# huzi96/gaussian-pcloud-render

Measured on AMD Instinct MI355X. Metric: rendered frames/sec at 1080p (fwd+bwd), THuman-800K, higher is better.
Workload: dtype f32

## Files before the change

### gaussian-pcloud-render_amd/csrc/api.hip

```cpp
#include <algorithm>
#include <cstdarg>
#include <cstdio>
#include <cstring>
#include <string>
#include <vector>

#include "common.hpp"
#include <atomic>
#include <map>
#include <mutex>

namespace gsr {

static thread_local char g_err[512] = "";

static int fail(int code, const char* fmt, ...)
{
    va_list ap;
    va_start(ap, fmt);
    vsnprintf(g_err, sizeof(g_err), fmt, ap);
    va_end(ap);
    return code;
}

int check_launch(const Launch& L, const char* what)
{
    hipError_t e = hipGetLastError();
    if (e == hipSuccess && L.debug) e = hipStreamSynchronize(L.stream);
    if (e != hipSuccess) return fail(GSR_ERR_HIP, "[gsr] %s: %s", what, hipGetErrorString(e));
    return GSR_OK;
}

struct ProfEntry {
    const char* name;
    int a, b;
};
struct ProfTables {
    std::vector<hipEvent_t> pool;
    size_t used = 0;
    std::vector<ProfEntry> rec;
    int event()
    {
        if (used == pool.size()) {
            hipEvent_t e;
            if (hipEventCreateWithFlags(&e, hipEventDisableSystemFence) != hipSuccess) (void)hipEventCreate(&e);
            pool.push_back(e);
        }
        return (int)used++;
    }
};
static std::atomic<int> g_prof_on{0};
static std::mutex g_prof_mu;
static std::map<hipStream_t, ProfTables> g_prof;

struct ProfScope {
    hipStream_t s;
    bool on;
    ProfEntry e;
    ProfScope(const char* name, hipStream_t stream) : s(stream), on(false)
    {
        const int mode = g_prof_on;
        on = mode == 1 || (mode == 2 && strncmp(name, "render_", 7) == 0);
        if (!on) return;
        e.name = name;
        hipEvent_t ea;
        {
            std::lock_guard<std::mutex> lk(g_prof_mu);
            ProfTables& t = g_prof[s];
            e.a = t.event();
            e.b = t.event();
            ea = t.pool[e.a];
        }
        (void)hipEventRecord(ea, s);
    }
    ~ProfScope()
    {
        if (!on) return;
        std::lock_guard<std::mutex> lk(g_prof_mu);
        ProfTables& t = g_prof[s];
        (void)hipEventRecord(t.pool[e.b], s);
        t.rec.push_back(e);
    }
};

constexpr int MAX_VIEWS = 256;
struct HostLanding {
    uint64_t* pinned = nullptr;
    uint64_t* mapped = nullptr;
    hipEvent_t ev = nullptr;
};
static thread_local std::map<int, HostLanding> t_lands;
static int landing(HostLanding** out)
{
    int dev = 0;
    if (hipGetDevice(&dev) != hipSuccess) return fail(GSR_ERR_HIP, "[gsr] hipGetDevice: %s", hipGetErrorString(hipGetLastError()));
    HostLanding& h = t_lands[dev];
    if (!h.pinned) {
        if (hipHostMalloc((void**)&h.pinned, MAX_VIEWS * 4 * sizeof(uint64_t), hipHostMallocMapped | hipHostMallocCoherent) != hipSuccess ||
            hipHostGetDevicePointer((void**)&h.mapped, h.pinned, 0) != hipSuccess ||
            hipEventCreateWithFlags(&h.ev, hipEventDisableTiming) != hipSuccess) {
            h.pinned = nullptr;
            return fail(GSR_ERR_HIP, "[gsr] pinned host buffer: %s", hipGetErrorString(hipGetLastError()));
        }
    }
    *out = &h;
    return GSR_OK;
}

static thread_local std::vector<int64_t> t_list_pairs;

static std::atomic<long long> g_d2h_count{0};

static std::atomic<int> g_tickets{[] { const char* e = getenv("GSR_TICKETS"); return e && atoi(e) == 0 ? 0 : 1; }()};
int block_tickets(int set)
{
    if (set >= 0) g_tickets = set != 0;
    return g_tickets;
}

static int tile_count(const gsr_params* p) { return ((p->W + TILE_X - 1) / TILE_X) * ((p->H + TILE_Y - 1) / TILE_Y); }

static int check_params(const gsr_params* p, int V = 1)
{
    if (!p) return fail(GSR_ERR_INVALID, "[gsr] params is NULL");
    if (p->P < 0 || p->W <= 0 || p->H <= 0) return fail(GSR_ERR_INVALID, "[gsr] bad sizes P=%d W=%d H=%d", p->P, p->W, p->H);
    if (V < 1 || V > MAX_VIEWS) return fail(GSR_ERR_INVALID, "[gsr] view count %d outside 1..%d", V, MAX_VIEWS);
    if (p->P == 0) return GSR_OK;
    if (!p->means3D || !p->opacities || !p->bg || !p->viewmatrix || !p->projmatrix || !p->campos)
        return fail(GSR_ERR_INVALID, "[gsr] a required input pointer is NULL");
    if ((p->shs == nullptr) == (p->colors_precomp == nullptr))
        return fail(GSR_ERR_INVALID, "Please provide excatly one of either SHs or precomputed colors!");
    if (((p->scales == nullptr || p->rotations == nullptr) && p->cov3D_precomp == nullptr) ||
        ((p->scales != nullptr || p->rotations != nullptr) && p->cov3D_precomp != nullptr))
        return fail(GSR_ERR_INVALID, "Please provide exactly one of either scale/rotation pair or precomputed 3D covariance!");
    if (p->shs) {
        if (p->D < 0 || p->D > 3) return fail(GSR_ERR_INVALID, "[gsr] SH degree %d outside 0..3", p->D);
        if ((p->D + 1) * (p->D + 1) > p->M) return fail(GSR_ERR_INVALID, "[gsr] SH degree %d needs %d coefficients, M=%d", p->D, (p->D + 1) * (p->D + 1), p->M);
    }
    const int64_t gx = (p->W + TILE_X - 1) / TILE_X, gy = (p->H + TILE_Y - 1) / TILE_Y;
    if (gx > 65535 || gy > 65535) return fail(GSR_ERR_INVALID, "[gsr] image too large for 16-bit tile coordinates");
    if (gx * gy > (1ll << BWD_TILE_BITS) || (gx * gy / 8 + 1) * 64 * V > 0x7FFFFFFFll)
        return fail(GSR_ERR_INVALID, "[gsr] %lld tiles x %d views: too many for one launch", (long long)(gx * gy), V);
    return GSR_OK;
}

static int tile_bits(int T) { return (int)higher_msb((uint32_t)T); }
static int sorted_buffer(int T) { return ((tile_bits(T) + RADIX_BITS - 1) / RADIX_BITS) & 1; }

static inline void* align256(void* p) { return (void*)(((uintptr_t)p + 255) & ~(uintptr_t)255); }

static int make_batch(const gsr_params* p, int V, void* geom, size_t geom_bytes, void* image, size_t image_bytes, void* binning,
                      size_t binning_bytes, bool with_grad, Batch& B)
{
    B.V = V;
    const size_t G = geom_view(nullptr, p->P).bytes, I = image_view(nullptr, p->W, p->H).bytes;
    const size_t GR = with_grad ? grad_rec_bytes(p->P) : 0;
    if (!geom || geom_bytes < (size_t)V * (G + GR) + 256)
        return fail(GSR_ERR_CAPACITY, "[gsr] geom arena too small (%zu < %zu%s)", geom_bytes, (size_t)V * (G + GR) + 256,
                    with_grad ? ", need_backward" : "");
    if (!image || image_bytes < (size_t)V * I + 256)
        return fail(GSR_ERR_CAPACITY, "[gsr] image arena too small (%zu < %zu)", image_bytes, (size_t)V * I + 256);
    B.g = geom_view(align256(geom), p->P);
    B.g_stride = G;
    B.grad_rec = with_grad ? reinterpret_cast<float*>(reinterpret_cast<char*>(align256(geom)) + (size_t)V * G) : nullptr;
    B.gr_stride = GR;
    B.iv = image_view(align256(image), p->W, p->H);
    B.iv_stride = I;
    if (binning) {
        if (binning_bytes < 256 + 256 * (size_t)V) return fail(GSR_ERR_CAPACITY, "[gsr] binning arena too small");
        const size_t per_view = ((binning_bytes - 256) / (size_t)V) / 256 * 256;
        const int64_t cap = bin_capacity_from_bytes(per_view);
        if (cap < 1) return fail(GSR_ERR_CAPACITY, "[gsr] binning arena too small (%zu bytes for %d views)", binning_bytes, V);
        B.b = bin_view(align256(binning), cap > 0xFFFFFFFFll ? 0xFFFFFFFFll : cap);
        B.b_stride = per_view;
    } else {
        B.b = bin_view(nullptr, 1);
        B.b.cap = 0;
        B.b_stride = 0;
    }
    return GSR_OK;
}

struct FrameRecord {
    int kind = 0;
    int need_backward = 0;
    int nx = 0, layout = 0;
    int V = 0, P = 0, W = 0, H = 0;
    const void* xstate = nullptr;
    size_t xstate_bytes = 0;
    int fwd_need_backward = -1;
    int64_t list_pairs = -1;
    FrameRecord() = default;
    FrameRecord(int kind_, const gsr_params* p, int V_) : kind(kind_), need_backward(p->need_backward != 0), V(V_), P(p->P), W(p->W), H(p->H) {}
};
static std::mutex g_frames_mu;
static std::map<const void*, FrameRecord> g_frames;
static void note_frame(const void* geom, const FrameRecord& r)
{
    std::lock_guard<std::mutex> lk(g_frames_mu);
    if (g_frames.size() > 4096 && !g_frames.count(geom)) g_frames.clear();
    g_frames[geom] = r;
}
static bool find_frame(const void* geom, FrameRecord& r)
{
    std::lock_guard<std::mutex> lk(g_frames_mu);
    const auto it = g_frames.find(geom);
    if (it == g_frames.end()) return false;
    r = it->second;
    return true;
}
static size_t xstate_view_bytes(int W, int H, int64_t cap, int nx) { return align_up(xstate_view(nullptr, W, H, cap, nx).bytes, 256); }

static int memset_views(hipStream_t s, void* base, size_t stride, size_t bytes, int V)
{
    if (bytes == 0) return GSR_OK;
    hipError_t e = V == 1 ? hipMemsetAsync(base, 0, bytes, s) : hipMemset2DAsync(base, stride, 0, bytes, (size_t)V, s);
    return e == hipSuccess ? GSR_OK : fail(GSR_ERR_HIP, "[gsr] memset failed: %s", hipGetErrorString(e));
}

static int forward_impl(const gsr_params* p, int V, void* geom, size_t geom_bytes, void* image, size_t image_bytes, void* binning,
                        size_t binning_bytes, int* radii, float* out_color, int64_t* num_rendered, int mode, hipStream_t stream,
                        const ExtraChannels* X = nullptr)
{
    if (int e = check_params(p, V)) return e;
    if (!num_rendered) return fail(GSR_ERR_INVALID, "[gsr] num_rendered is NULL");
    for (int v = 0; v < V; v++) num_rendered[v] = 0;
    if (p->P == 0) return GSR_OK;
    if (mode != 1 && !radii) return fail(GSR_ERR_INVALID, "[gsr] radii is NULL");
    if (mode != 2 && !out_color) return fail(GSR_ERR_INVALID, "[gsr] out_color is NULL");
    if (mode != 2 && !binning) return fail(GSR_ERR_INVALID, "[gsr] binning arena is NULL");
    Batch B;
    if (int e = make_batch(p, V, geom, geom_bytes, image, image_bytes, mode == 2 ? nullptr : binning, binning_bytes,
                           p->need_backward != 0, B))
        return e;
    ExtraChannels Xs;
    const void* xraw = X != nullptr ? (const void*)X->state.accum : nullptr;
    if (X != nullptr && X->state.accum != nullptr) {
        Xs = *X;
        const size_t need = (size_t)V * xstate_view_bytes(p->W, p->H, B.b.cap, X->nx) + 256;
        if (X->state.bytes < need)
            return fail(GSR_ERR_CAPACITY, "[gsr] extra-state block too small (%zu < %zu: V * gsr_extra_state_bytes(W, H, n, nx) for a binning "
                        "arena of V * gsr_binning_bytes(n))", X->state.bytes, need);
        Xs.state = xstate_view(align256(const_cast<float*>(X->state.accum)), p->W, p->H, B.b.cap, X->nx);
        Xs.state_stride = xstate_view_bytes(p->W, p->H, B.b.cap, X->nx);
        if (!p->need_backward) Xs.state = XStateView{nullptr, nullptr, 0};
        X = &Xs;
    }
    {
        FrameRecord r(X ? 1 : 0, p, V);
        r.fwd_need_backward = r.need_backward;
        if (X) {
            r.nx = X->nx;
            r.layout = X->values_hi ? 2 : X->view_stride ? 1 : 0;
            if (X->state.accum) { r.xstate = xraw; r.xstate_bytes = X->state.bytes; }
        }
        note_frame(geom, r);
    }
    HostLanding* landp = nullptr;
    if (int e = landing(&landp)) return e;
    HostLanding& t_land = *landp;
    const Launch L{stream, p->debug};
    const int T = tile_count(p);
    const int gridx = (p->W + TILE_X - 1) / TILE_X;
    const bool key16 = tile_keys16(T);
    memset(t_land.pinned, 0, (size_t)V * 4 * sizeof(uint64_t));

    if (mode == 1) {
        if (int e = memset_views(L.stream, B.g.zero_begin, B.g_stride, B.g.zero_bytes, V)) return e;
        if (int e = memset_views(L.stream, B.iv.zero_begin, B.iv_stride, B.iv.zero_bytes, V)) return e;
    } else {
        if (p->prefiltered)
            if (int e = memset_views(L.stream, B.g.counters, B.g_stride, 8 * sizeof(uint64_t), V)) return e;
        {
            ProfScope ps("preprocess", L.stream);
            if (int e = launch_preprocess(L, *p, B, radii)) return e;
        }
        {
            ProfScope ps("depth_sort", L.stream);
            SortJob job{{B.g.dkey[0], B.g.dkey[1]}, {B.g.dval[0], B.g.dval[1]}, B.g.hist, B.g.totals, B.g_stride, nullptr, 0, p->P, V};
            job.blk_minmax = B.g.blk_minmax;
            job.sortctl = B.g.sortctl;
            job.small_blocks = div_up(p->P, RS_TILE) * V < 4096;
            int res = 0;
            if (int e = launch_radix_sort_pairs(L, job, true, 32, &res)) return e;
        }
    }
    const auto rest = [&]() -> int {
        {
            ProfScope ps("duplicate", L.stream);
            if (int e = launch_duplicate(L, p->P, B, gridx, key16, t_land.mapped)) return e;
        }
        {
            g_d2h_count++;
            const hipError_t e = hipEventRecord(t_land.ev, L.stream);
            if (e != hipSuccess) return fail(GSR_ERR_HIP, "[gsr] num_rendered read-back: %s", hipGetErrorString(e));
        }
        if (mode != 2) {
            const int res = sorted_buffer(T);
            {
                ProfScope ps("tile_sort", L.stream);
                SortJob job{{B.b.key[0], B.b.key[1]}, {B.b.val[0], B.b.val[1]}, B.b.hist, B.b.totals, B.b_stride,
                            B.g.counters + CNT_NUM_RENDERED, B.g_stride, B.b.cap, V};
                int r2 = 0;
                if (int e = launch_radix_sort_pairs(L, job, false, tile_bits(T), &r2, key16)) return e;
            }
            {
                ProfScope ps("tile_ranges", L.stream);
                if (int e = launch_tile_ranges(L, B, B.b.key[res], T, key16)) return e;
                if (int e = launch_tile_order(L, B, T)) return e;
            }
            {
                ProfScope ps("render_forward", L.stream);
                if (int e = launch_render_forward(L, *p, B, B.b.val[res], out_color, p->need_backward != 0, X)) return e;
            }
        }
        return GSR_OK;
    };
    if (int e = rest()) {
        (void)hipStreamSynchronize(L.stream);
        return e;
    }
    if (hipEventSynchronize(t_land.ev) != hipSuccess)
        return fail(GSR_ERR_HIP, "[gsr] num_rendered read-back failed: %s", hipGetErrorString(hipGetLastError()));
    bool retry = false;
    t_list_pairs.assign((size_t)V, 0);
    for (int v = 0; v < V; v++) {
        const uint64_t R = t_land.pinned[4 * v + LAND_NUM_REFERENCE], Lp = t_land.pinned[4 * v + CNT_NUM_RENDERED];
        if (t_land.pinned[4 * v + CNT_STALL])
            return fail(GSR_ERR_HIP, "[gsr] pair emission: a workgroup's pair count never arrived (view %d)", v);
        if (p->prefiltered && t_land.pinned[4 * v + CNT_TRAP])
            return fail(GSR_ERR_TRAP, "Point is filtered although prefiltered is set. This shouldn't happen!");
        if (R > 0x7FFFFFFFull)
            return fail(GSR_ERR_CAPACITY, "[gsr] num_rendered = %llu tile pairs does not fit the reference's int (scales too large?)",
                        (unsigned long long)R);
        num_rendered[v] = (int64_t)R;
        t_list_pairs[(size_t)v] = (int64_t)Lp;
        if (mode != 2 && (int64_t)Lp > B.b.cap) retry = true;
    }
    {
        FrameRecord r;
        if (find_frame(geom, r)) {
            r.list_pairs = *std::max_element(t_list_pairs.begin(), t_list_pairs.end());
            note_frame(geom, r);
        }
    }
    if (retry) {
        fail(GSR_RETRY, "[gsr] binning arena holds %lld pairs per view, the frame needs more (num_rendered is enough; gsr_last_list_pairs is exact): repeat with resume = 1",
             (long long)B.b.cap);
        return GSR_RETRY;
    }
    return GSR_OK;
}

}

using namespace gsr;

extern "C" {

size_t gsr_geom_bytes(int P) { return geom_view(nullptr, P).bytes + grad_rec_bytes(P) + 256; }
size_t gsr_geom_bytes_inference(int P) { return geom_view(nullptr, P).bytes + 256; }
size_t gsr_image_bytes(int W, int H) { return image_view(nullptr, W, H).bytes + 256; }
size_t gsr_binning_bytes(int64_t R) { return bin_view(nullptr, R).bytes + 256; }

int gsr_forward_batch(const gsr_params* p, int V, void* geom, size_t geom_bytes, void* image, size_t image_bytes, void* binning,
                      size_t binning_bytes, int* radii, float* out_color, int64_t* num_rendered, int resume, gsr_stream_t stream)
{
    return forward_impl(p, V, geom, geom_bytes, image, image_bytes, binning, binning_bytes, radii, out_color, num_rendered,
                        resume ? 1 : 0, (hipStream_t)stream);
}

static int extra_channels(const gsr_params* p, int nx, int extra_per_view, const float* extra, const float* extra_view_scale,
                          const float* bg_extra, float* out_extra, ExtraChannels& X)
{
    if (!p) return fail(GSR_ERR_INVALID, "[gsr] params is NULL");
    if (nx != 4 && nx != 8) return fail(GSR_ERR_INVALID, "[gsr] extra channels come in 4 or 8 (got %d): pad with zeros", nx);
    if (!extra || !bg_extra || !out_extra) return fail(GSR_ERR_INVALID, "[gsr] an extra-channel pointer is NULL");
    if (extra_per_view < 0 || extra_per_view > 2 || (extra_per_view == 2 && nx != 8))
        return fail(GSR_ERR_INVALID, "[gsr] extra_per_view is 0, 1 or (with 8 channels) 2");
    X = ExtraChannels{nx, extra, extra_view_scale, bg_extra, out_extra, extra_per_view == 1 ? (size_t)p->P * (size_t)nx : (size_t)0};
    if (extra_per_view == 2) {
        X.values_hi = extra + (size_t)p->P * 4;
        X.hi_view_stride = (size_t)p->P * 4;
    }
    return GSR_OK;
}

int gsr_forward_batch_channels(const gsr_params* p, int V, void* geom, size_t geom_bytes, void* image, size_t image_bytes,
                               void* binning, size_t binning_bytes, int* radii, float* out_color, int64_t* num_rendered, int resume,
                               int nx, int extra_per_view, const float* extra, const float* extra_view_scale, const float* bg_extra,
                               float* out_extra, gsr_stream_t stream)
{
    ExtraChannels X;
    if (int e = extra_channels(p, nx, extra_per_view, extra, extra_view_scale, bg_extra, out_extra, X)) return e;
    return forward_impl(p, V, geom, geom_bytes, image, image_bytes, binning, binning_bytes, radii, out_color, num_rendered,
                        resume ? 1 : 0, (hipStream_t)stream, &X);
}

size_t gsr_extra_state_bytes(int W, int H, int64_t num_rendered, int nx)
{
    if (W <= 0 || H <= 0 || (nx != 4 && nx != 8)) return 0;
    return xstate_view_bytes(W, H, bin_capacity_from_bytes(bin_view(nullptr, num_rendered).bytes), nx);
}

int gsr_forward_batch_channels_train(const gsr_params* p, int V, void* geom, size_t geom_bytes, void* image, size_t image_bytes,
                                     void* binning, size_t binning_bytes, int* radii, float* out_color, int64_t* num_rendered,
                                     int resume, int nx, int extra_per_view, const float* extra, const float* extra_view_scale,
                                     const float* bg_extra, float* out_extra, void* extra_state, size_t extra_state_bytes,
                                     gsr_stream_t stream)
{
    ExtraChannels X;
    if (int e = extra_channels(p, nx, extra_per_view, extra, extra_view_scale, bg_extra, out_extra, X)) return e;
    if (!extra_state) return fail(GSR_ERR_INVALID, "[gsr] extra_state is NULL");
    X.state = XStateView{reinterpret_cast<float*>(extra_state), nullptr, extra_state_bytes};
    return forward_impl(p, V, geom, geom_bytes, image, image_bytes, binning, binning_bytes, radii, out_color, num_rendered,
                        resume ? 1 : 0, (hipStream_t)stream, &X);
}

int gsr_forward_stage1(const gsr_params* p, void* geom, size_t geom_bytes, void* image, size_t image_bytes, int* radii,
                       int64_t* num_rendered_out, gsr_stream_t stream)
{
    if (!num_rendered_out) return fail(GSR_ERR_INVALID, "[gsr] num_rendered_out is NULL");
    return forward_impl(p, 1, geom, geom_bytes, image, image_bytes, nullptr, 0, radii, nullptr, num_rendered_out, 2, (hipStream_t)stream);
}

int gsr_forward_stage2(const gsr_params* p, void* geom, size_t geom_bytes, void* binning, size_t binning_bytes, void* image,
                       size_t image_bytes, int64_t R, float* out_color, gsr_stream_t stream)
{
    if (R < 0 || R > 0x7FFFFFFFll) return fail(GSR_ERR_INVALID, "[gsr] num_rendered out of range");
    if (p && p->P > 0 && (!binning || binning_bytes < gsr_binning_bytes(R)))
        return fail(GSR_ERR_CAPACITY, "[gsr] binning arena too small (%zu < %zu)", binning_bytes, gsr_binning_bytes(R));
    int64_t got = 0;
    const int rc = forward_impl(p, 1, geom, geom_bytes, image, image_bytes, binning, binning_bytes, nullptr, out_color, &got, 1,
                                (hipStream_t)stream);
    if (rc == GSR_OK && p && p->P > 0 && got != R) return fail(GSR_ERR_INVALID, "[gsr] stage 2 found %lld pairs, stage 1 reported %lld", (long long)got, (long long)R);
    return rc;
}

int gsr_forward_recolor(const gsr_params* p, int V, int colors_per_view, void* geom, size_t geom_bytes, const void* binning,
                        size_t binning_bytes, void* image, size_t image_bytes, float* out_color, gsr_stream_t stream)
{
    if (!p) return fail(GSR_ERR_INVALID, "[gsr] params is NULL");
    if (V < 1 || V > MAX_VIEWS) return fail(GSR_ERR_INVALID, "[gsr] view count %d outside 1..%d", V, MAX_VIEWS);
    if (p->P <= 0) return GSR_OK;
    if ((p->shs == nullptr) == (p->colors_precomp == nullptr))
        return fail(GSR_ERR_INVALID, "Please provide excatly one of either SHs or precomputed colors!");
    if (p->shs && (!p->means3D || !p->campos || p->D < 0 || p->D > 3 || (p->D + 1) * (p->D + 1) > p->M))
        return fail(GSR_ERR_INVALID, "[gsr] recolor: bad SH arguments");
    if (!out_color || !p->bg || !binning) return fail(GSR_ERR_INVALID, "[gsr] recolor: NULL pointer");
    Batch B;
    if (int e = make_batch(p, V, geom, geom_bytes, image, image_bytes, const_cast<void*>(binning), binning_bytes, false, B)) return e;
    {
        FrameRecord prev, r(2, p, V);
        if (find_frame(geom, prev)) {
            r.fwd_need_backward = prev.fwd_need_backward;
            r.list_pairs = prev.list_pairs;
        }
        note_frame(geom, r);
    }
    const Launch L{(hipStream_t)stream, p->debug};
    const int res = sorted_buffer(tile_count(p));
    {
        ProfScope ps("recolor", L.stream);
        if (int e = launch_recolor(L, *p, B, (colors_per_view && p->colors_precomp) ? (size_t)p->P * 3 : 0)) return e;
        if (int e = memset_views(L.stream, B.iv.tile_need, B.iv_stride, (size_t)tile_count(p) * sizeof(uint32_t), V)) return e;
    }
    {
        ProfScope ps("render_forward", L.stream);
        if (int e = launch_render_forward(L, *p, B, B.b.val[res], out_color, p->need_backward != 0)) return e;
    }
    return GSR_OK;
}

static size_t det_view_bytes(int W, int H, int64_t pairs)
{
    const int T = ((W + TILE_X - 1) / TILE_X) * ((H + TILE_Y - 1) / TILE_Y);
    return align_up(det_view(nullptr, T, pairs).bytes, 256);
}

size_t gsr_backward_det_bytes(int V, int P, int W, int H, int64_t pairs)
{
    (void)P;
    if (V < 1 || W <= 0 || H <= 0) return 0;
    if (pairs > 0xFFFFFFFFll) pairs = 0xFFFFFFFFll;
    return (size_t)V * det_view_bytes(W, H, pairs) + 256;
}

struct BwdGrads {
    const float* dL_dpix;
    float *dL_dmean2D, *dL_dopacity, *dL_dcolor, *dL_dmean3D, *dL_dcov3D, *dL_dsh, *dL_dscale, *dL_drot;
};
struct BwdDet { void* scratch; size_t bytes; };
struct BwdExtra {
    ExtraChannels X;
    ExtraGrads XG;
    int layout;
    const void* state;
    size_t state_bytes;
};

static int check_bwd_pointers(const gsr_params* p, const int* radii, const void* binning, const BwdGrads& G)
{
    if (!radii || !G.dL_dpix || !G.dL_dmean2D || !G.dL_dopacity || !G.dL_dcolor || !G.dL_dmean3D || !G.dL_dcov3D)
        return fail(GSR_ERR_INVALID, "[gsr] a required backward pointer is NULL");
    if (p->shs && !G.dL_dsh) return fail(GSR_ERR_INVALID, "[gsr] dL_dsh is NULL");
    if (p->scales && (!G.dL_dscale || !G.dL_drot)) return fail(GSR_ERR_INVALID, "[gsr] dL_dscale/dL_drot is NULL");
    if (p->scales && ((uintptr_t)G.dL_drot & 15u)) return fail(GSR_ERR_INVALID, "[gsr] dL_drot must be 16-byte aligned (it is written one float4 per Gaussian)");
    if (!binning) return fail(GSR_ERR_INVALID, "[gsr] binning arena is NULL");
    return GSR_OK;
}

static int check_bwd_frame(const void* geom, const gsr_params* p, int V, const BwdExtra* x, int64_t* list_pairs)
{
    FrameRecord r;
    *list_pairs = -1;
    if (!find_frame(geom, r))
        return x ? fail(GSR_ERR_INVALID, "[gsr] backward_channels: no forward on this geometry arena (run gsr_forward_batch_channels_train first)")
                 : GSR_OK;
    *list_pairs = r.list_pairs;
    const bool same = r.V == V && r.P == p->P && r.W == p->W && r.H == p->H;
    if (x) {
        if (r.kind == 2)
            return fail(GSR_ERR_INVALID, "[gsr] backward_channels after gsr_forward_recolor is not supported: the recolor replaced the saves "
                        "of the channels forward (run gsr_forward_batch_channels_train again)");
        if (r.kind != 1 || !r.need_backward || r.xstate == nullptr)
            return fail(GSR_ERR_INVALID, "[gsr] backward_channels: the forward on this arena saved no extra channels (it needs "
                        "gsr_forward_batch_channels_train with need_backward = 1)");
        if (r.nx != x->X.nx || r.layout != x->layout)
            return fail(GSR_ERR_INVALID, "[gsr] backward_channels: nx = %d, extra_per_view = %d, but the forward had nx = %d, extra_per_view = %d",
                        x->X.nx, x->layout, r.nx, r.layout);
        if (!same) return fail(GSR_ERR_INVALID, "[gsr] backward_channels: views / sizes differ from the forward's");
        if (r.xstate != x->state || x->state_bytes < r.xstate_bytes)
            return fail(GSR_ERR_INVALID, "[gsr] backward_channels: extra_state is not the block the forward saved into");
        return GSR_OK;
    }
    if (!r.need_backward)
        return fail(GSR_ERR_INVALID, "[gsr] backward: the last %s on this geometry arena had need_backward = 0 and saved nothing for "
                    "it", r.kind == 2 ? "gsr_forward_recolor" : "forward");
    if (r.fwd_need_backward == 0)
        return fail(GSR_ERR_INVALID, "[gsr] backward: the recolor's forward on this geometry arena had need_backward = 0 (a "
                    "need_backward recolor needs the arenas of a need_backward forward)");
    if (!same)
        return fail(GSR_ERR_INVALID, "[gsr] backward: V = %d, P = %d, %d x %d, but the last forward or recolor on this geometry "
                    "arena had V = %d, P = %d, %d x %d", V, p->P, p->W, p->H, r.V, r.P, r.W, r.H);
    return GSR_OK;
}

static int backward_impl(const gsr_params* p, int V, const int* radii, const void* geom, size_t geom_bytes, const void* binning,
                         size_t binning_bytes, const void* image, size_t image_bytes, const BwdGrads& G, const BwdDet* det, BwdExtra* x,
                         gsr_stream_t stream)
{
    if (det && x) return fail(GSR_ERR_INVALID, "[gsr] backward: no deterministic backward of the extra channels");
    if (int e = check_params(p, V)) return e;
    if (p->P == 0) return GSR_OK;
    int64_t list_pairs = -1;
    if (!x)
        if (int e = check_bwd_pointers(p, radii, binning, G)) return e;
    if (int e = check_bwd_frame(geom, p, V, x, &list_pairs)) return e;
    if (x)
        if (int e = check_bwd_pointers(p, radii, binning, G)) return e;
    Batch B;
    if (int e = make_batch(p, V, const_cast<void*>(geom), geom_bytes, const_cast<void*>(image), image_bytes,
                           const_cast<void*>(binning), binning_bytes, true, B))
        return e;
    const Launch L{(hipStream_t)stream, p->debug};
    const int T = tile_count(p), res = sorted_buffer(T);
    DetView D{};
    size_t d_stride = 0;
    if (det) {
        int64_t n = list_pairs >= 0 ? list_pairs : B.b.cap;
        if (n > B.b.cap) n = B.b.cap;
        if (n < 1) n = 1;
        const size_t need = gsr_backward_det_bytes(V, p->P, p->W, p->H, n);
        if (!det->scratch || det->bytes < need)
            return fail(GSR_ERR_CAPACITY, "[gsr] backward_det: scratch block too small (%zu < %zu = gsr_backward_det_bytes(%d, %d, %d, %d, %lld): "
                        "the forward's lists hold up to %lld pairs per view)", det->bytes, need, V, p->P, p->W, p->H, (long long)n,
                        (long long)n);
        D = det_view(align256(det->scratch), T, n);
        d_stride = det_view_bytes(p->W, p->H, n);
    }
    if (x) {
        const int nx = x->X.nx;
        x->X.state = xstate_view(align256(const_cast<void*>(x->state)), p->W, p->H, B.b.cap, nx);
        x->X.state_stride = xstate_view_bytes(p->W, p->H, B.b.cap, nx);
        if (x->state_bytes < (size_t)V * x->X.state_stride + 256)
            return fail(GSR_ERR_CAPACITY, "[gsr] extra-state block too small for this binning arena");
    }
    {
        ProfScope ps("bwd_items", L.stream);
        const size_t n_out = !x ? 0 : (size_t)p->P * (x->layout == 0 ? x->X.nx : x->layout == 1 ? V * x->X.nx : (1 + V) * 4);
        if (x && hipMemsetAsync(x->XG.grad, 0, n_out * sizeof(float), L.stream) != hipSuccess)
            return fail(GSR_ERR_HIP, "[gsr] memset failed: %s", hipGetErrorString(hipGetLastError()));
        if (int e = launch_bwd_items(L, B, T, p->P)) return e;
    }
    int dres = 0;
    if (det) {
        {
            ProfScope ps("det_prepare", L.stream);
            if (int e = launch_det_prepare(L, B, D, d_stride, B.b.val[res], T)) return e;
        }
        {
            ProfScope ps("det_sort", L.stream);
            if (int e = launch_det_sort(L, B, D, d_stride, p->P, &dres)) return e;
        }
    }
    {
        ProfScope ps("render_backward", L.stream);
        const RenderBwdDet d{D.part, D.flags, D.slot_base, d_stride, (uint32_t)D.cap};
        if (int e = launch_render_backward(L, *p, B, B.b.val[res], G.dL_dpix, x ? &x->X : nullptr, x ? &x->XG : nullptr, det ? &d : nullptr))
            return e;
    }
    if (det) {
        ProfScope ps("det_reduce", L.stream);
        if (int e = launch_det_reduce(L, B, D, d_stride, dres)) return e;
    }
    {
        ProfScope ps("preprocess_backward", L.stream);
        if (int e = launch_preprocess_backward(L, *p, B, radii, G.dL_dmean2D, G.dL_dopacity, G.dL_dcolor, G.dL_dmean3D, G.dL_dcov3D,
                                               G.dL_dsh, G.dL_dscale, G.dL_drot))
            return e;
    }
    return GSR_OK;
}

int gsr_backward_batch(const gsr_params* p, int V, const int* radii, const void* geom, size_t geom_bytes, const void* binning,
                       size_t binning_bytes, const void* image, size_t image_bytes, const float* dL_dpix, float* dL_dmean2D,
                       float* dL_dopacity, float* dL_dcolor, float* dL_dmean3D, float* dL_dcov3D, float* dL_dsh, float* dL_dscale,
                       float* dL_drot, gsr_stream_t stream)
{
    const BwdGrads G{dL_dpix, dL_dmean2D, dL_dopacity, dL_dcolor, dL_dmean3D, dL_dcov3D, dL_dsh, dL_dscale, dL_drot};
    return backward_impl(p, V, radii, geom, geom_bytes, binning, binning_bytes, image, image_bytes, G, nullptr, nullptr, stream);
}

int gsr_backward_batch_det(const gsr_params* p, int V, const int* radii, const void* geom, size_t geom_bytes, const void* binning,
                           size_t binning_bytes, const void* image, size_t image_bytes, const float* dL_dpix, float* dL_dmean2D,
                           float* dL_dopacity, float* dL_dcolor, float* dL_dmean3D, float* dL_dcov3D, float* dL_dsh, float* dL_dscale,
                           float* dL_drot, void* det_scratch, size_t det_scratch_bytes, gsr_stream_t stream)
{
    const BwdGrads G{dL_dpix, dL_dmean2D, dL_dopacity, dL_dcolor, dL_dmean3D, dL_dcov3D, dL_dsh, dL_dscale, dL_drot};
    const BwdDet det{det_scratch, det_scratch_bytes};
    return backward_impl(p, V, radii, geom, geom_bytes, binning, binning_bytes, image, image_bytes, G, &det, nullptr, stream);
}

int gsr_backward_batch_channels(const gsr_params* p, int V, const int* radii, const void* geom, size_t geom_bytes, const void* binning,
                                size_t binning_bytes, const void* image, size_t image_bytes, const float* dL_dpix, float* dL_dmean2D,
                                float* dL_dopacity, float* dL_dcolor, float* dL_dmean3D, float* dL_dcov3D, float* dL_dsh,
                                float* dL_dscale, float* dL_drot, int nx, int extra_per_view, const float* extra,
                                const float* extra_view_scale, const float* bg_extra, const void* extra_state, size_t extra_state_bytes,
                                const float* dL_dextra, float* dL_dextra_values, gsr_stream_t stream)
{
    BwdExtra x{{}, {}, extra_per_view, extra_state, extra_state_bytes};
    if (int e = extra_channels(p, nx, extra_per_view, extra, extra_view_scale, bg_extra, dL_dextra_values, x.X)) return e;
    if (!dL_dextra || !extra_state) return fail(GSR_ERR_INVALID, "[gsr] dL_dextra / extra_state is NULL");
    x.XG = ExtraGrads{dL_dextra, dL_dextra_values, extra_per_view == 2 ? dL_dextra_values + (size_t)p->P * 4 : nullptr};
    const BwdGrads G{dL_dpix, dL_dmean2D, dL_dopacity, dL_dcolor, dL_dmean3D, dL_dcov3D, dL_dsh, dL_dscale, dL_drot};
    return backward_impl(p, V, radii, geom, geom_bytes, binning, binning_bytes, image, image_bytes, G, nullptr, &x, stream);
}

int gsr_backward(const gsr_params* p, const int* radii, int64_t R, const void* geom, size_t geom_bytes, const void* binning,
                 size_t binning_bytes, const void* image, size_t image_bytes, const float* dL_dpix, float* dL_dmean2D,
                 float* dL_dopacity, float* dL_dcolor, float* dL_dmean3D, float* dL_dcov3D, float* dL_dsh,
                 float* dL_dscale, float* dL_drot, gsr_stream_t stream)
{
    (void)R;
    return gsr_backward_batch(p, 1, radii, geom, geom_bytes, binning, binning_bytes, image, image_bytes, dL_dpix, dL_dmean2D,
                              dL_dopacity, dL_dcolor, dL_dmean3D, dL_dcov3D, dL_dsh, dL_dscale, dL_drot, stream);
}

int gsr_mark_visible(int P, const float* means3D, const float* viewmatrix, const float* projmatrix, uint8_t* present,
                     gsr_stream_t stream)
{
    (void)projmatrix;
    if (P < 0) return fail(GSR_ERR_INVALID, "[gsr] P < 0");
    if (P == 0) return GSR_OK;
    if (!means3D || !viewmatrix || !present) return fail(GSR_ERR_INVALID, "[gsr] NULL pointer");
    const Launch L{(hipStream_t)stream, 0};
    return launch_mark_visible(L, P, means3D, viewmatrix, present);
}

namespace {
__global__ void k_clock_probe(unsigned long long* out, int iters)
{
    const unsigned long long s0 = clock64(), w0 = wall_clock64();
    float x = (float)threadIdx.x * 1e-3f;
    for (int i = 0; i < iters; i++) {
#pragma unroll
        for (int k = 0; k < 64; k++) x = __builtin_fmaf(x, 0.999f, 1e-3f);
    }
    const unsigned long long s1 = clock64(), w1 = wall_clock64();
    if (threadIdx.x == 0) {
        out[0] = s1 - s0;
        out[1] = w1 - w0;
    }
    if (x == 12345.678f) out[1] = 0;
}
__global__ void k_query(int what, int64_t n, const Splat* __restrict__ sp, const uint8_t* __restrict__ clamped,
                        const uint32_t* __restrict__ k, int key16, const uint32_t* __restrict__ v, void* __restrict__ dst)
{
    const int64_t i = (int64_t)blockIdx.x * 256 + threadIdx.x;
    if (i >= n) return;
    float* d = (float*)dst;
    switch (what) {
    case GSR_Q_DEPTHS: d[i] = sp[i].q2.y; break;
    case GSR_Q_MEANS2D: d[2 * i] = sp[i].q0.x; d[2 * i + 1] = sp[i].q0.y; break;
    case GSR_Q_CONIC_OPACITY:
        d[4 * i] = sp[i].q0.z; d[4 * i + 1] = sp[i].q0.w; d[4 * i + 2] = sp[i].q1.x; d[4 * i + 3] = sp[i].q1.y;
        break;
    case GSR_Q_RGB: d[3 * i] = sp[i].q1.z; d[3 * i + 1] = sp[i].q1.w; d[3 * i + 2] = sp[i].q2.x; break;
    case GSR_Q_POINT_LIST_KEYS:
        ((uint64_t*)dst)[i] = ((uint64_t)(key16 ? (uint32_t)((const uint16_t*)k)[i] : k[i]) << 32) | (uint64_t)__float_as_uint(sp[v[i]].q2.y);
        break;
    case GSR_Q_LIST_PAIRS: {
        const uint64_t* c = (const uint64_t*)k;
        if (i == 0) { ((uint64_t*)dst)[0] = c[CNT_NUM_RENDERED]; ((uint64_t*)dst)[1] = c[CNT_NUM_REFERENCE]; }
        break;
    }
    case GSR_Q_DEPTH_SORT: {
        uint32_t* o = (uint32_t*)dst;
        if (i == 0) { o[0] = k[SORTCTL_BASE]; o[1] = k[SORTCTL_BITS]; o[2] = depth_sort_passes(k[SORTCTL_BITS]); o[3] = 0u; }
        break;
    }
    case GSR_Q_CLAMPED: {
        uint8_t* c = (uint8_t*)dst;
        c[3 * i] = clamped[i] & 1; c[3 * i + 1] = (clamped[i] >> 1) & 1; c[3 * i + 2] = (clamped[i] >> 2) & 1;
        break;
    }
    default: break;
    }
}
}

int gsr_query(const gsr_params* p, int what, const void* geom, const void* binning, size_t binning_bytes, const void* image,
              int64_t R, void* dst, size_t dst_bytes, gsr_stream_t stream)
{
    if (!p || !dst) return fail(GSR_ERR_INVALID, "[gsr] query: NULL");
    hipStream_t s = (hipStream_t)stream;
    const int P = p->P, T = tile_count(p);
    const int64_t N = (int64_t)p->W * p->H;
    const GeomView g = geom_view(align256(const_cast<void*>(geom)), P);
    if (binning && binning_bytes < 512) return fail(GSR_ERR_CAPACITY, "[gsr] query: binning arena too small");
    const int64_t cap = binning ? bin_capacity_from_bytes(((binning_bytes - 256)) / 256 * 256) : 0;
    if (binning && R > cap && (what == GSR_Q_POINT_LIST || what == GSR_Q_POINT_LIST_KEYS))
        return fail(GSR_ERR_CAPACITY, "[gsr] query: arena holds %lld pairs, asked for %lld (the lists hold GSR_Q_LIST_PAIRS pairs)", (long long)cap, (long long)R);
    const BinView b = bin_view(align256(const_cast<void*>(binning)), cap > 0 ? cap : 1);
    const ImageView iv = image_view(align256(const_cast<void*>(image)), p->W, p->H);
    const int res = sorted_buffer(T);
    int64_t n = 0;
    size_t bytes = 0;
    const void* src = nullptr;
    switch (what) {
    case GSR_Q_DEPTHS: n = P; bytes = (size_t)P * 4; break;
    case GSR_Q_MEANS2D: n = P; bytes = (size_t)P * 8; break;
    case GSR_Q_CONIC_OPACITY: n = P; bytes = (size_t)P * 16; break;
    case GSR_Q_RGB: n = P; bytes = (size_t)P * 12; break;
    case GSR_Q_CLAMPED: n = P; bytes = (size_t)P * 3; break;
    case GSR_Q_POINT_LIST_KEYS: n = R; bytes = (size_t)R * 8; break;
    case GSR_Q_TILES_TOUCHED: src = g.tiles_touched; bytes = (size_t)P * 4; break;
    case GSR_Q_POINT_LIST: src = b.val[res]; bytes = (size_t)R * 4; break;
    case GSR_Q_RANGES: src = iv.ranges; bytes = (size_t)T * 8; break;
    case GSR_Q_FINAL_T: src = iv.final_T; bytes = (size_t)N * 4; break;
    case GSR_Q_N_CONTRIB: src = iv.n_contrib; bytes = (size_t)N * 4; break;
    case GSR_Q_TILE_NEED: src = iv.tile_need; bytes = (size_t)T * 4; break;
    case GSR_Q_DEPTH_SORT: n = 1; bytes = 16; break;
    case GSR_Q_LIST_PAIRS: n = 1; bytes = 16; break;
    default: return fail(GSR_ERR_INVALID, "[gsr] query: unknown item %d", what);
    }
    if (dst_bytes < bytes) return fail(GSR_ERR_CAPACITY, "[gsr] query %d: destination too small", what);
    if (bytes == 0) return GSR_OK;
    if (src) {
        if (hipMemcpyAsync(dst, src, bytes, hipMemcpyDeviceToDevice, s) != hipSuccess) return fail(GSR_ERR_HIP, "[gsr] query copy failed");
    } else {
        hipLaunchKernelGGL(k_query, dim3((unsigned)div_up(n, 256)), dim3(256), 0, s, what, n, g.splat, g.clamped,
                           what == GSR_Q_DEPTH_SORT ? (const uint32_t*)g.sortctl
                           : what == GSR_Q_LIST_PAIRS ? (const uint32_t*)g.counters : (const uint32_t*)b.key[res],
                           (int)tile_keys16(T), b.val[res], dst);
        if (hipGetLastError() != hipSuccess) return fail(GSR_ERR_HIP, "[gsr] query kernel failed");
    }
    return GSR_OK;
}

int gsr_selftest(gsr_stream_t stream)
{
    hipStream_t s = (hipStream_t)stream;
    float* d = nullptr;
    if (hipMalloc(&d, 256 * sizeof(float)) != hipSuccess) return fail(GSR_ERR_HIP, "[gsr] selftest: hipMalloc failed");
    const int rm = selftest_mm(s, d);
    (void)hipFree(d);
    if (rm != 0) return fail(GSR_ERR_HIP, "[gsr] selftest: matrix-core pixel contraction wrong at check %d", rm);
    const int rd = selftest_det_reduce(s);
    if (rd != 0) return fail(GSR_ERR_HIP, "[gsr] selftest: ordered reduction of the deterministic backward differs from the host sum at check %d", rd);

    const int64_t n = 100003;
    std::vector<uint32_t> hk(n), hv(n), order(n);
    uint32_t x = 12345u;
    for (int64_t i = 0; i < n; i++) {
        x = x * 1664525u + 1013904223u;
        hk[i] = (x >> 8) % 3001u;
        hv[i] = (uint32_t)i;
        order[i] = (uint32_t)i;
    }
    std::stable_sort(order.begin(), order.end(), [&](uint32_t a, uint32_t b) { return hk[a] < hk[b]; });
    uint32_t *k0, *k1, *v0, *v1, *hist, *tot;
    const size_t nb = (size_t)sort_hist_stride(n);
    if (hipMalloc(&k0, n * 4) != hipSuccess || hipMalloc(&k1, n * 4) != hipSuccess || hipMalloc(&v0, n * 4) != hipSuccess ||
        hipMalloc(&v1, n * 4) != hipSuccess || hipMalloc(&hist, RADIX * nb * 4) != hipSuccess || hipMalloc(&tot, RADIX * 4) != hipSuccess)
        return fail(GSR_ERR_HIP, "[gsr] selftest: hipMalloc failed");
    (void)hipMemcpyAsync(k0, hk.data(), n * 4, hipMemcpyHostToDevice, s);
    uint32_t* key[2] = {k0, k1};
    uint32_t* val[2] = {v0, v1};
    int res = 0;
    const Launch L{s, 1};
    const SortJob job{{k0, k1}, {v0, v1}, hist, tot, 0, nullptr, 0, n, 1};
    int rc = launch_radix_sort_pairs(L, job, true, 12, &res);
    std::vector<uint32_t> gk(n), gv(n);
    if (rc == 0) {
        (void)hipMemcpyAsync(gk.data(), key[res], n * 4, hipMemcpyDeviceToHost, s);
        (void)hipMemcpyAsync(gv.data(), val[res], n * 4, hipMemcpyDeviceToHost, s);
        if (hipStreamSynchronize(s) != hipSuccess) rc = GSR_ERR_HIP;
    }
    (void)hipFree(k0); (void)hipFree(k1); (void)hipFree(v0); (void)hipFree(v1); (void)hipFree(hist); (void)hipFree(tot);
    if (rc != 0) return rc;
    for (int64_t i = 0; i < n; i++)
        if (gv[i] != order[i] || gk[i] != hk[order[i]]) return fail(GSR_ERR_HIP, "[gsr] selftest: radix sort differs from std::stable_sort at %lld", (long long)i);
    return GSR_OK;
}

int gsr_clock_probe_launch(void* dst16, int iters, gsr_stream_t stream)
{
    if (!dst16 || iters < 1) return fail(GSR_ERR_INVALID, "[gsr] clock probe: bad argument");
    hipLaunchKernelGGL(k_clock_probe, dim3(1), dim3(64), 0, (hipStream_t)stream, (unsigned long long*)dst16, iters);
    if (hipGetLastError() != hipSuccess) return fail(GSR_ERR_HIP, "[gsr] clock probe launch failed");
    return GSR_OK;
}

int gsr_wall_clock_khz(void)
{
    int dev = 0, khz = 0;
    if (hipGetDevice(&dev) != hipSuccess || hipDeviceGetAttribute(&khz, hipDeviceAttributeWallClockRate, dev) != hipSuccess) return 0;
    return khz;
}

void gsr_set_profiling(int on)
{
    std::lock_guard<std::mutex> lk(g_prof_mu);
    g_prof_on = on < 0 ? 0 : on > 2 ? 1 : on;
    for (auto& kv : g_prof) { kv.second.rec.clear(); kv.second.used = 0; }
}

int gsr_get_profile(const char** names, float* ms, int cap)
{
    std::lock_guard<std::mutex> lk(g_prof_mu);
    int n = 0;
    for (auto& kv : g_prof) {
        ProfTables& t = kv.second;
        for (auto& e : t.rec) {
            if (n >= cap) break;
            (void)hipEventSynchronize(t.pool[e.b]);
            float d = 0;
            (void)hipEventElapsedTime(&d, t.pool[e.a], t.pool[e.b]);
            names[n] = e.name;
            ms[n] = d;
            n++;
        }
        t.rec.clear();
        t.used = 0;
    }
    return n;
}

#ifdef GSR_STATS
__attribute__((visibility("default"))) int gsr_debug_bwd_stats(unsigned long long* out8, int reset) { return gsr::debug_bwd_stats(out8, reset); }
__attribute__((visibility("default"))) int gsr_debug_scatter_times(unsigned long long* out8, int reset) { return gsr::debug_scatter_times(out8, reset); }
__attribute__((visibility("default"))) int gsr_debug_fwd_times(unsigned long long* out8, int reset) { return gsr::debug_fwd_times(out8, reset); }
__attribute__((visibility("default"))) int gsr_debug_fwd_records(unsigned* out, int n) { return gsr::debug_fwd_records(out, n); }
__attribute__((visibility("default"))) int gsr_debug_bwd_times(unsigned long long* out8, int reset) { return gsr::debug_bwd_times(out8, reset); }
__attribute__((visibility("default"))) int gsr_debug_bwd_records(unsigned* out, int n) { return gsr::debug_bwd_records(out, n); }
__attribute__((visibility("default"))) int gsr_debug_dup_times(unsigned long long* out8, int reset) { return gsr::debug_dup_times(out8, reset); }
#endif

long long gsr_d2h_count(void) { return gsr::g_d2h_count.load(); }
int gsr_set_forward_half_views(int views) { return gsr::forward_half_views(views); }
int gsr_set_backward_moments(int mode) { return gsr::backward_subquadrant_moments(mode); }

int gsr_last_list_pairs(int64_t* out, int V)
{
    if (!out || V < 0) return fail(GSR_ERR_INVALID, "[gsr] gsr_last_list_pairs: bad argument");
    for (int v = 0; v < V; v++) out[v] = (size_t)v < gsr::t_list_pairs.size() ? gsr::t_list_pairs[(size_t)v] : 0;
    return GSR_OK;
}

const char* gsr_last_error(void) { return gsr::g_err; }
const char* gsr_version(void) { return "gsr-hip 0.3 (gfx950)"; }

}
```

### gaussian-pcloud-render_amd/csrc/binning.hip

```cpp
#include "common.hpp"
#include "tile_cull.hpp"

namespace gsr {

__device__ __forceinline__ uint64_t agent_load(const uint64_t* p)
{
    return __hip_atomic_load(p, __ATOMIC_RELAXED, __HIP_MEMORY_SCOPE_AGENT);
}
__device__ __forceinline__ void agent_store(uint64_t* p, uint64_t v)
{
    __hip_atomic_store(p, v, __ATOMIC_RELAXED, __HIP_MEMORY_SCOPE_AGENT);
}

#ifdef GSR_STATS
constexpr int DUP_REC = 65536;
__device__ unsigned g_dup_rec[DUP_REC][4];
#define DUP_T(var) const unsigned long long var = wall_clock64()
#define DUP_ADD(i, v) do { if (threadIdx.x == 0) { const unsigned r_ = blockIdx.y * gridDim.x + s_ticket; if (r_ < DUP_REC) g_dup_rec[r_][i] = (unsigned)(v); } } while (0)
int debug_dup_times(unsigned long long* out8, int reset)
{
    static unsigned host[DUP_REC][4];
    if (hipMemcpyFromSymbol(host, HIP_SYMBOL(g_dup_rec), sizeof(host)) != hipSuccess) return -1;
    for (int i = 0; i < 8; i++) out8[i] = 0;
    for (int r = 0; r < DUP_REC; r++) {
        if (host[r][0] == 0 && host[r][1] == 0) continue;
        for (int i = 0; i < 4; i++) out8[i] += host[r][i];
        out8[4]++;
    }
    if (reset) {
        for (int r = 0; r < DUP_REC; r++) for (int i = 0; i < 4; i++) host[r][i] = 0;
        if (hipMemcpyToSymbol(HIP_SYMBOL(g_dup_rec), host, sizeof(host)) != hipSuccess) return -1;
    }
    return 0;
}
#else
#define DUP_T(var) do { } while (0)
#define DUP_ADD(i, v) do { } while (0)
#endif

struct DupArgs {
    int P;
    uint32_t gridx;
    const uint32_t* order[2];
    const uint32_t* sortctl;
    const Splat* splat;
    uint64_t* dup_status;
    uint64_t* counters;
    size_t g_stride;
    void* keys;
    uint32_t* vals;
    size_t b_stride;
    int64_t cap;
    uint64_t* host_land;
    int tickets;
};

template <typename KeyT>
__global__ __launch_bounds__(DUP_THREADS) void k_duplicate(DupArgs a)
{
    __shared__ uint32_t s_off[4][64];
    __shared__ uint32_t s_id[4][64];
    __shared__ uint2 s_rect[4][64];
    __shared__ uint32_t s_sp2[4][64];
    __shared__ uint2 s_pre[4][64];
    __shared__ uint32_t s_flag[4][64];
    __shared__ uint64_t s_wave[4];
    __shared__ uint64_t s_ref[4];
    __shared__ uint64_t s_base;
    __shared__ uint32_t s_ticket;
    const uint32_t view = blockIdx.y;
    const uint32_t lane = threadIdx.x & 63, w = threadIdx.x >> 6;
    uint64_t* status = at_view(a.dup_status, a.g_stride, view);
    const uint32_t nblk = gridDim.x;
    DUP_T(t0);
    if (threadIdx.x == 0) s_ticket = a.tickets ? (uint32_t)atomicAdd((unsigned long long*)&status[DUP_COPIES * nblk], 1ull) : blockIdx.x;
    __syncthreads();
    DUP_T(t1);
    DUP_ADD(0, t1 - t0);
    const uint32_t blk = s_ticket;
    const uint32_t npass = depth_sort_passes(at_view(a.sortctl, a.g_stride, view)[SORTCTL_BITS]);
    const uint32_t* order = at_view((npass & 1u) ? a.order[1] : a.order[0], a.g_stride, view);
    const Splat* splat = at_view(a.splat, a.g_stride, view);

    uint32_t cnt[DUP_G], id[DUP_G], sp2[DUP_G];
    uint2 rc[DUP_G];
    uint64_t ref_cnt = 0;
    const int slot0 = (int)(blk * DUP_BLOCK + w * (64 * DUP_G) + lane);
#pragma unroll
    for (int g = 0; g < DUP_G; g++) {
        const int slot = slot0 + g * 64;
        id[g] = slot < a.P ? order[slot] : 0u;
    }
#pragma unroll
    for (int g = 0; g < DUP_G; g++) {
        cnt[g] = 0;
        rc[g] = make_uint2(0, 0);
        sp2[g] = 0;
        if (slot0 + g * 64 < a.P) {
            const float4 q3 = splat[id[g]].q3;
            const uint32_t w3 = __float_as_uint(q3.w);
            rc[g] = make_uint2(__float_as_uint(q3.x), __float_as_uint(q3.y));
            sp2[g] = __float_as_uint(q3.z);
            if (w3 & SPANS_FLAG) {
                const uint32_t a4 = (rc[g].y >> 4) & 0x0F0F0F0Fu, b4 = (sp2[g] >> 4) & 0x0F0F0F0Fu;
                const uint32_t pa = a4 * 0x01010101u;
                const uint32_t pb = b4 * 0x01010101u + (pa >> 24) * 0x01010101u;
                cnt[g] = pb >> 24;
                id[g] |= SPANS_FLAG;
            } else {
                cnt[g] = sp2[g];
            }
            ref_cnt += w3 & ~SPANS_FLAG;
        }
    }
    uint64_t excl[DUP_G];
    uint64_t run = 0;
#pragma unroll
    for (int g = 0; g < DUP_G; g++) {
        uint64_t inc64 = cnt[g];
#pragma unroll
        for (int d = 1; d < 64; d <<= 1) {
            const uint64_t n = (uint64_t)__shfl_up((unsigned long long)inc64, d, 64);
            if (lane >= (uint32_t)d) inc64 += n;
        }
        excl[g] = run + inc64 - cnt[g];
        run += (uint64_t)__shfl((unsigned long long)inc64, 63, 64);
    }
#pragma unroll
    for (int d = 32; d >= 1; d >>= 1) ref_cnt += (uint64_t)__shfl_xor((unsigned long long)ref_cnt, d, 64);
    if (lane == 63) { s_wave[w] = run; s_ref[w] = ref_cnt; }
    __syncthreads();
    uint64_t wave_base = 0;
#pragma unroll
    for (int i = 0; i < 4; i++)
        if ((uint32_t)i < w) wave_base += s_wave[i];
    const uint64_t block_total = s_wave[0] + s_wave[1] + s_wave[2] + s_wave[3];
    const uint64_t block_ref = s_ref[0] + s_ref[1] + s_ref[2] + s_ref[3];
    const uint64_t sat = 0xFFFFFFFEull;
    const uint64_t word = ((block_total < sat ? block_total : sat) + 1ull) | ((block_ref < 0xFFFFFFFFull ? block_ref : 0xFFFFFFFFull) << 32);
    if (threadIdx.x < DUP_COPIES) agent_store(&status[threadIdx.x * nblk + blk], word);
    DUP_T(t2);
    DUP_ADD(1, t2 - t1);
    uint64_t part = 0, part_ref = 0;
    constexpr uint32_t LB = 4;
    const uint64_t* mine = status + (size_t)(blk % DUP_COPIES) * nblk;
    for (uint32_t b0 = threadIdx.x; b0 < blk; b0 += DUP_THREADS * LB) {
        uint64_t v[LB];
#pragma unroll
        for (uint32_t k = 0; k < LB; k++) {
            const uint32_t b = b0 + k * DUP_THREADS;
            v[k] = b < blk ? agent_load(&mine[b]) : 1ull;
        }
#pragma unroll
        for (uint32_t k = 0; k < LB; k++) {
            uint32_t spins = 0;
            while ((uint32_t)v[k] == 0u) {
                v[k] = agent_load(&mine[b0 + k * DUP_THREADS]);
                if ((uint32_t)v[k] == 0u && ++spins > (1u << 24)) {
                    at_view(a.counters, a.g_stride, view)[CNT_STALL] = 1;
                    a.host_land[4 * view + CNT_STALL] = 1;
                    v[k] = 1;
                }
            }
            part += (v[k] & 0xFFFFFFFFull) - 1;
            part_ref += v[k] >> 32;
        }
    }
#pragma unroll
    for (int d = 32; d >= 1; d >>= 1) {
        part += (uint64_t)__shfl_xor((unsigned long long)part, d, 64);
        part_ref += (uint64_t)__shfl_xor((unsigned long long)part_ref, d, 64);
    }
    __syncthreads();
    if (lane == 0) { s_wave[w] = part; s_ref[w] = part_ref; }
    __syncthreads();
    if (threadIdx.x == 0) {
        const uint64_t base = s_wave[0] + s_wave[1] + s_wave[2] + s_wave[3];
        s_base = base;
        if (blk == nblk - 1) {
            uint64_t* cnt = at_view(a.counters, a.g_stride, view);
            const uint64_t ref_total = s_ref[0] + s_ref[1] + s_ref[2] + s_ref[3] + block_ref;
            cnt[CNT_NUM_RENDERED] = base + block_total;
            cnt[CNT_NUM_REFERENCE] = ref_total;
            a.host_land[4 * view + CNT_NUM_RENDERED] = base + block_total;
            a.host_land[4 * view + CNT_TRAP] = cnt[CNT_TRAP];
            a.host_land[4 * view + LAND_NUM_REFERENCE] = ref_total;
            __threadfence_system();
        }
    }
    __syncthreads();
    DUP_T(t3);
    DUP_ADD(2, t3 - t2);
    if (a.keys == nullptr) return;
    KeyT* keys = at_view((KeyT*)a.keys, a.b_stride, view);
    uint32_t* vals = at_view(a.vals, a.b_stride, view);
    const uint64_t wave_off = s_base + wave_base;

#pragma unroll 1
    for (int g = 0; g < DUP_G; g++) {
        uint32_t cnt_g = cnt[0], id_g = id[0], sp2_g = sp2[0];
        uint2 rc_g = rc[0];
        uint64_t ex_g = excl[0];
#pragma unroll
        for (int k = 1; k < DUP_G; k++)
            if (g == k) { cnt_g = cnt[k]; id_g = id[k]; rc_g = rc[k]; ex_g = excl[k]; sp2_g = sp2[k]; }
        const uint64_t off64 = wave_off + ex_g;
        const uint64_t grp_begin64 = (uint64_t)__shfl((unsigned long long)off64, 0, 64);
        const uint64_t grp_end64 = (uint64_t)__shfl((unsigned long long)(off64 + cnt_g), 63, 64);
        if (grp_begin64 >= (uint64_t)a.cap) break;
        const uint32_t grp_begin = (uint32_t)grp_begin64;
        const uint32_t grp_end = grp_end64 < (uint64_t)a.cap ? (uint32_t)grp_end64 : (uint32_t)a.cap;
        const uint64_t nzb = __ballot(cnt_g != 0);
        const uint32_t n_nz = (uint32_t)__popcll(nzb);
        const uint32_t jslot = __builtin_amdgcn_mbcnt_hi((uint32_t)(nzb >> 32), __builtin_amdgcn_mbcnt_lo((uint32_t)nzb, 0u));
        __builtin_amdgcn_wave_barrier();
        if (cnt_g != 0) {
            s_off[w][jslot] = (uint32_t)(off64 - grp_begin64);
            s_id[w][jslot] = id_g;
            s_rect[w][jslot] = rc_g;
            s_sp2[w][jslot] = sp2_g;
            if (id_g & SPANS_FLAG) {
                const uint32_t a4 = (rc_g.y >> 4) & 0x0F0F0F0Fu, b4 = (sp2_g >> 4) & 0x0F0F0F0Fu;
                const uint32_t pa = a4 * 0x01010101u;
                s_pre[w][jslot] = make_uint2(pa, b4 * 0x01010101u + (pa >> 24) * 0x01010101u);
            }
        }
        __builtin_amdgcn_wave_barrier();
        const uint32_t my_start = lane < n_nz ? s_off[w][lane] : 0xFFFFFFFFu;
        const uint32_t range = grp_end - grp_begin;
        uint32_t before = 0;
        for (uint32_t c = 0; c < range; c += 64) {
            s_flag[w][lane] = 0u;
            const uint32_t d = my_start - c;
            if (d < 64u) s_flag[w][d] = 1u;
            __builtin_amdgcn_wave_barrier();
            const uint32_t mine = s_flag[w][lane];
            const uint64_t starts = __ballot(mine != 0u);
            const uint32_t owner = before + mine - 1u +
                                   __builtin_amdgcn_mbcnt_hi((uint32_t)(starts >> 32), __builtin_amdgcn_mbcnt_lo((uint32_t)starts, 0u));
            before += (uint32_t)__popcll(starts);
            __builtin_amdgcn_wave_barrier();
            const uint32_t rel = c + lane;
            if (rel < range) {
                const uint2 r = s_rect[w][owner];
                const uint32_t oid = s_id[w][owner];
                const uint32_t minx = r.x & 0xFFFFu, miny = r.x >> 16;
                const uint32_t t = rel - s_off[w][owner];
                uint32_t row, col;
                if (oid & SPANS_FLAG) {
                    const uint2 pre = s_pre[w][owner];
                    const uint32_t tt = (127u - t) * 0x01010101u;
                    const uint32_t xa = (pre.x + tt) & 0x80808080u, xb = (pre.y + tt) & 0x80808080u;
                    row = 8u - (uint32_t)__popc(xa) - (uint32_t)__popc(xb);
                    const uint32_t rp = row - 1u;
                    const uint32_t before = row == 0u ? 0u : (((rp < 4u ? pre.x : pre.y) >> (8u * (rp & 3u))) & 0xFFu);
                    const uint32_t byte = ((row < 4u ? r.y : s_sp2[w][owner]) >> (8u * (row & 3u))) & 0xFFu;
                    col = (byte & 15u) + (t - before);
                } else {
                    const uint32_t width = (r.y & 0xFFFFu) - minx;
                    row = t / width;
                    col = t - row * width;
                }
                const uint32_t p = grp_begin + rel;
                keys[p] = (KeyT)((miny + row) * a.gridx + (minx + col));
                vals[p] = oid & ~SPANS_FLAG;
            }
        }
    }
#ifdef GSR_STATS
    if (w == 0) { DUP_T(t4); DUP_ADD(3, t4 - t3); }
#endif
}

int launch_duplicate(const Launch& L, int P, const Batch& B, int gridx, bool key16, uint64_t* host_land)
{
    DupArgs a;
    a.P = P;
    a.gridx = (uint32_t)gridx;
    a.order[0] = B.g.dval[0];
    a.order[1] = B.g.dval[1];
    a.sortctl = B.g.sortctl;
    a.splat = B.g.splat;
    a.dup_status = B.g.dup_status;
    a.counters = B.g.counters;
    a.g_stride = B.g_stride;
    a.keys = B.b.key[0];
    a.vals = B.b.val[0];
    a.b_stride = B.b_stride;
    a.cap = B.b.key[0] ? B.b.cap : 0;
    a.host_land = host_land;
    a.tickets = block_tickets(-1);
    const dim3 grid((unsigned)div_up(P, DUP_BLOCK), B.V);
    if (key16)
        hipLaunchKernelGGL(k_duplicate<uint16_t>, grid, dim3(DUP_THREADS), 0, L.stream, a);
    else
        hipLaunchKernelGGL(k_duplicate<uint32_t>, grid, dim3(DUP_THREADS), 0, L.stream, a);
    return check_launch(L, "duplicate");
}

constexpr int RANGE_SAMPLE = 4096;
constexpr int RANGE_MAX_SAMPLES = 8192;

template <typename KeyT>
__device__ __forceinline__ uint32_t lower_bound_keys(const KeyT* __restrict__ keys, uint32_t n, const uint32_t* __restrict__ samples,
                                                     uint32_t ns, uint32_t t)
{
    uint32_t lo = 0, hi = n;
    if (ns != 0) {
        uint32_t a = 0, b = ns;
        while (a < b) {
            const uint32_t m = (a + b) >> 1;
            if (samples[m] < t) a = m + 1; else b = m;
        }
        if (a == 0) return 0;
        lo = (a - 1) * RANGE_SAMPLE + 1;
        hi = a < ns ? a * RANGE_SAMPLE : n;
    }
    while (lo < hi) {
        const uint32_t m = (lo + hi) >> 1;
        if ((uint32_t)keys[m] < t) lo = m + 1; else hi = m;
    }
    return lo;
}

constexpr int RANGE_TILES_PER_WG = 255;
template <typename KeyT>
__global__ __launch_bounds__(256) void k_tile_ranges(const uint64_t* __restrict__ counters, size_t g_stride, int64_t cap,
                                                     const KeyT* __restrict__ keys, size_t b_stride, uint2* __restrict__ ranges,
                                                     size_t iv_stride, int T)
{
    __shared__ uint32_t samples[RANGE_MAX_SAMPLES];
    __shared__ uint32_t bound[256];
    const uint32_t view = blockIdx.y;
    const uint64_t n64 = at_view(counters, g_stride, view)[CNT_NUM_RENDERED];
    const uint32_t n = (uint32_t)(n64 < (uint64_t)cap ? n64 : (uint64_t)cap);
    keys = at_view(keys, b_stride, view);
    ranges = at_view(ranges, iv_stride, view);
    uint32_t ns = (n + RANGE_SAMPLE - 1) / RANGE_SAMPLE;
    if (ns > RANGE_MAX_SAMPLES) ns = 0;
    for (uint32_t j = threadIdx.x; j < ns; j += 256) samples[j] = (uint32_t)keys[(size_t)j * RANGE_SAMPLE];
    __syncthreads();
    const int t = blockIdx.x * RANGE_TILES_PER_WG + threadIdx.x;
    bound[threadIdx.x] = (t < T && n != 0) ? lower_bound_keys(keys, n, samples, ns, (uint32_t)t) : n;
    __syncthreads();
    if (threadIdx.x >= RANGE_TILES_PER_WG || t >= T) return;
    const uint32_t first = bound[threadIdx.x], last = bound[threadIdx.x + 1];
    ranges[t] = first < last ? make_uint2(first, last) : make_uint2(0u, 0u);
}

int launch_tile_ranges(const Launch& L, const Batch& B, const uint32_t* sorted_keys, int T, bool key16)
{
    const dim3 grid((unsigned)div_up(T, RANGE_TILES_PER_WG), B.V);
    if (key16)
        hipLaunchKernelGGL(k_tile_ranges<uint16_t>, grid, dim3(256), 0, L.stream, B.g.counters, B.g_stride, B.b.cap,
                           (const uint16_t*)sorted_keys, B.b_stride, B.iv.ranges, B.iv_stride, T);
    else
        hipLaunchKernelGGL(k_tile_ranges<uint32_t>, grid, dim3(256), 0, L.stream, B.g.counters, B.g_stride, B.b.cap, sorted_keys,
                           B.b_stride, B.iv.ranges, B.iv_stride, T);
    return check_launch(L, "tile_ranges");
}

constexpr int ORD_BUCKETS = 128;

__device__ __forceinline__ uint32_t work_bucket(uint32_t len)
{
    if (len == 0) return ORD_BUCKETS - 1;
    const uint32_t msb = 31u - (uint32_t)__builtin_clz(len);
    const uint32_t frac = msb >= 2 ? (len >> (msb - 2)) & 3u : 0u;
    const uint32_t rank = msb * 4u + frac;
    return (ORD_BUCKETS - 2) - (rank < ORD_BUCKETS - 2 ? rank : ORD_BUCKETS - 2);
}

__device__ __forceinline__ uint32_t work_estimate(uint32_t len, float knee, float expo)
{
    if (knee <= 0.f || (float)len <= knee) return len;
    return (uint32_t)(knee * __builtin_amdgcn_exp2f(expo * __builtin_amdgcn_logf(knee / (float)len)));
}

__global__ __launch_bounds__(1024) void k_tile_order(int T, const uint2* __restrict__ ranges, uint32_t* __restrict__ tile_order,
                                                     size_t iv_stride, float knee, float expo)
{
    ranges = at_view(ranges, iv_stride, blockIdx.x);
    tile_order = at_view(tile_order, iv_stride, blockIdx.x);
    __shared__ uint32_t cnt[ORD_BUCKETS];
    __shared__ uint32_t cur[ORD_BUCKETS];
    const uint32_t lane = threadIdx.x & 63;
    const uint64_t lt_mask = (1ull << lane) - 1ull;
    if (threadIdx.x < ORD_BUCKETS) cnt[threadIdx.x] = 0;
    __syncthreads();
    const int T_pad = (T + 1023) / 1024 * 1024;
    for (int pass = 0; pass < 2; pass++) {
        for (int t = threadIdx.x; t < T_pad; t += 1024) {
            const bool ok = t < T;
            uint32_t b = 0;
            if (ok) b = work_bucket(work_estimate(ranges[t].y - ranges[t].x, knee, expo));
            const bool empty = ok && b == ORD_BUCKETS - 1;
            const uint64_t em = __ballot(empty);
            uint32_t slot = 0;
            if (pass == 0) {
                if (empty) { if ((em & lt_mask) == 0) atomicAdd(&cnt[b], (uint32_t)__popcll(em)); }
                else if (ok) atomicAdd(&cnt[b], 1u);
            } else {
                uint32_t basev = 0;
                const int leader = em ? (int)__builtin_ctzll(em) : 0;
                if (empty && (int)lane == leader) basev = atomicAdd(&cur[b], (uint32_t)__popcll(em));
                basev = __shfl(basev, leader, 64);
                if (empty) slot = basev + (uint32_t)__popcll(em & lt_mask);
                else if (ok) slot = atomicAdd(&cur[b], 1u);
                if (ok) tile_order[slot] = (uint32_t)t;
            }
        }
        __syncthreads();
        if (pass == 0) {
            if (threadIdx.x < 64) {
                const uint32_t a0 = cnt[2 * lane], a1 = cnt[2 * lane + 1];
                uint32_t inc = a0 + a1;
#pragma unroll
                for (int d = 1; d < 64; d <<= 1) {
                    const uint32_t n = __shfl_up(inc, d, 64);
                    if (lane >= (uint32_t)d) inc += n;
                }
                cur[2 * lane] = inc - a0 - a1;
                cur[2 * lane + 1] = inc - a1;
            }
            __syncthreads();
        }
    }
}

static void order_params(float& knee, float& expo)
{
    static const float k = [] { const char* e = getenv("GSR_ORDER_KNEE"); return e ? (float)atof(e) : 2048.f; }();
    static const float x = [] { const char* e = getenv("GSR_ORDER_EXP"); return e ? (float)atof(e) : 0.3f; }();
    knee = k;
    expo = x;
}

int launch_tile_order(const Launch& L, const Batch& B, int T)
{
    float knee, expo;
    order_params(knee, expo);
    hipLaunchKernelGGL(k_tile_order, dim3(B.V), dim3(1024), 0, L.stream, T, B.iv.ranges, B.iv.tile_order, B.iv_stride, knee, expo);
    return check_launch(L, "tile_order");
}

constexpr int BWD_CLEAR_BLOCKS = 64;
__global__ __launch_bounds__(1024) void k_bwd_items(int T, int chunk_shift, const uint32_t* __restrict__ need, uint32_t* __restrict__ items,
                                                    uint32_t* __restrict__ count, size_t iv_stride, const uint64_t* __restrict__ counters,
                                                    size_t g_stride, float* __restrict__ grad_rec, size_t gr_stride, size_t gr_bytes)
{
    if (blockIdx.y != 0) {
        if (at_view(counters, g_stride, blockIdx.x)[CNT_BWD_DIRTY] == 0) return;
        zero_region(reinterpret_cast<char*>(at_view(grad_rec, gr_stride, blockIdx.x)), gr_bytes,
                    (size_t)(blockIdx.y - 1) * 1024 + threadIdx.x, (size_t)BWD_CLEAR_BLOCKS * 1024);
        return;
    }
    need = at_view(need, iv_stride, blockIdx.x);
    items = at_view(items, iv_stride, blockIdx.x);
    count = at_view(count, iv_stride, blockIdx.x);
    if (threadIdx.x < 8) count[BWD_QUEUE_WORD + threadIdx.x] = 0;
    __shared__ uint32_t cnt[ORD_BUCKETS];
    __shared__ uint32_t cur[ORD_BUCKETS];
    const uint32_t lane = threadIdx.x & 63;
    if (threadIdx.x < ORD_BUCKETS) cnt[threadIdx.x] = 0;
    __syncthreads();
    const uint32_t full_bucket = work_bucket(1u << chunk_shift);
    for (int pass = 0; pass < 2; pass++) {
        for (int t = threadIdx.x; t < T; t += 1024) {
            const uint32_t n = need[t];
            if (n == 0) continue;
            uint32_t n_full = n >> chunk_shift;
            if (n_full > BWD_MAX_CHUNKS - 1) n_full = BWD_MAX_CHUNKS - 1;
            const uint32_t rest = n - (n_full << chunk_shift);
            if (pass == 0) {
                if (n_full) atomicAdd(&cnt[full_bucket], n_full);
                if (rest) atomicAdd(&cnt[work_bucket(rest)], 1u);
            } else {
                if (n_full) {
                    const uint32_t slot = atomicAdd(&cur[full_bucket], n_full);
                    for (uint32_t c = 0; c < n_full; c++) items[slot + c] = (uint32_t)t | (c << BWD_TILE_BITS);
                }
                if (rest) items[atomicAdd(&cur[work_bucket(rest)], 1u)] = (uint32_t)t | (n_full << BWD_TILE_BITS);
            }
        }
        __syncthreads();
        if (pass == 0) {
            if (threadIdx.x < 64) {
                const uint32_t a0 = cnt[2 * lane], a1 = cnt[2 * lane + 1];
                uint32_t inc = a0 + a1;
#pragma unroll
                for (int d = 1; d < 64; d <<= 1) {
                    const uint32_t n = __shfl_up(inc, d, 64);
                    if (lane >= (uint32_t)d) inc += n;
                }
                cur[2 * lane] = inc - a0 - a1;
                cur[2 * lane + 1] = inc - a1;
                if (lane == 63) count[0] = inc;
            }
            __syncthreads();
        }
    }
}

int launch_bwd_items(const Launch& L, const Batch& B, int T, int P)
{
    hipLaunchKernelGGL(k_bwd_items, dim3(B.V, 1 + BWD_CLEAR_BLOCKS), dim3(1024), 0, L.stream, T, B.chunk_shift(), B.iv.tile_need, B.iv.bwd_items,
                       B.iv.bwd_count, B.iv_stride, B.g.counters, B.g_stride, B.grad_rec, B.gr_stride, grad_rec_bytes(P));
    return check_launch(L, "bwd_items");
}

}
```

### gaussian-pcloud-render_amd/csrc/common.hpp

```cpp
#pragma once
#include <hip/hip_runtime.h>
#include <stdint.h>

#include <type_traits>

#include "../../include/gsr.h"

#if defined(__HIP_DEVICE_COMPILE__) && !defined(__gfx950__)
#error "libgsr_hip is written for gfx950 (MI355X) only: build with --offload-arch=gfx950"
#endif

namespace gsr {

constexpr int TILE_X = 16;
constexpr int TILE_Y = 16;
constexpr int TILE_PIX = TILE_X * TILE_Y;

constexpr int RS_THREADS = 256;
constexpr int RS_WAVES = RS_THREADS / 64;
#ifndef GSR_RS_ITEMS
#define GSR_RS_ITEMS 16
#endif
constexpr int RS_ITEMS = GSR_RS_ITEMS;
constexpr int RS_TILE = RS_THREADS * RS_ITEMS;
constexpr int RADIX_BITS = 8;
constexpr int RADIX = 1 << RADIX_BITS;

constexpr int RS_ITEMS_SMALL = 8;
constexpr int RS_TILE_SMALL = RS_THREADS * RS_ITEMS_SMALL;
inline int sort_hist_stride(int64_t n, int tile = RS_TILE) { return (int)(((n + tile - 1) / tile + 15) / 16 * 16); }

constexpr int DUP_THREADS = 256;
#ifndef GSR_DUP_G
#define GSR_DUP_G 4
#endif
constexpr int DUP_G = GSR_DUP_G;
constexpr int DUP_BLOCK = DUP_THREADS * DUP_G;
#ifndef GSR_DUP_COPIES
#define GSR_DUP_COPIES 8
#endif
constexpr int DUP_COPIES = GSR_DUP_COPIES;

inline size_t align_up(size_t v, size_t a) { return (v + a - 1) / a * a; }
inline int64_t div_up(int64_t a, int64_t b) { return (a + b - 1) / b; }

template <typename T>
__host__ __device__ __forceinline__ T* at_view(T* p, size_t stride_bytes, uint32_t view)
{
    using B = typename std::conditional<std::is_const<T>::value, const char, char>::type;
    return (T*)((B*)p + stride_bytes * view);
}

struct __attribute__((aligned(64))) Splat {
    float4 q0, q1, q2, q3;
};

constexpr int GRAD_REC_WORDS = 16;
inline size_t grad_rec_bytes(int P) { return ((size_t)(P > 0 ? P : 1) * GRAD_REC_WORDS * sizeof(float) + 255) / 256 * 256; }

constexpr int CNT_NUM_RENDERED = 0;
constexpr int CNT_TRAP = 1;
constexpr int CNT_STALL = 2;
constexpr int CNT_NUM_REFERENCE = 4;
constexpr int LAND_NUM_REFERENCE = 3;
constexpr int CNT_BWD_DIRTY = 3;

struct GeomView {
    Splat* splat;
    uint32_t* tiles_touched;
    uint8_t* clamped;
    uint32_t* dkey[2];
    uint32_t* dval[2];
    uint32_t* hist;
    uint32_t* totals;
    uint32_t* blk_minmax;
    uint32_t* sortctl;
    uint64_t* dup_status;
    uint64_t* counters;
    char* zero_begin;
    size_t zero_bytes;
    size_t bytes;
};

constexpr int BWD_CHUNK_SHIFT_MIN = 9;
#ifndef GSR_CHUNK_V
#define GSR_CHUNK_V 2
#endif
__host__ __device__ inline int bwd_chunk_shift(int V) { return V >= GSR_CHUNK_V ? 10 : 9; }
constexpr int BWD_MAX_CHUNKS = 32;
constexpr int BWD_QUEUE_WORD = 8;
constexpr int BWD_TILE_BITS = 27;

struct BinView {
    uint32_t* key[2];
    uint32_t* val[2];
    uint32_t* hist;
    uint32_t* totals;
    float4* ckpt;
    int64_t cap;
    size_t bytes;
};

struct ImageView {
    uint32_t* tile_need;
    uint32_t* bwd_count;
    uint2* ranges;
    float* final_T;
    uint32_t* n_contrib;
    uint32_t* tile_order;
    float* accum;
    uint32_t* bwd_items;
    char* zero_begin;
    size_t zero_bytes;
    size_t bytes;
};

template <typename T>
inline void carve(char*& cur, T*& ptr, size_t count)
{
    ptr = reinterpret_cast<T*>(cur);
    cur += align_up(count * sizeof(T), 256);
}

inline GeomView geom_view(void* base, int P)
{
    GeomView g;
    char* cur = reinterpret_cast<char*>(base);
    const size_t p = (size_t)(P > 0 ? P : 1);
    const size_t nblk = (size_t)sort_hist_stride((int64_t)p, RS_TILE_SMALL);
    carve(cur, g.splat, p);
    carve(cur, g.tiles_touched, p);
    carve(cur, g.clamped, p);
    carve(cur, g.dkey[0], p);
    carve(cur, g.dkey[1], p);
    carve(cur, g.dval[0], p);
    carve(cur, g.dval[1], p);
    carve(cur, g.hist, RADIX * nblk);
    carve(cur, g.totals, (size_t)RADIX);
    carve(cur, g.blk_minmax, 2 * nblk);
    carve(cur, g.sortctl, (size_t)4);
    g.zero_begin = cur;
    carve(cur, g.dup_status, (size_t)DUP_COPIES * (size_t)div_up((int64_t)p, DUP_BLOCK) + 1);
    g.zero_bytes = (size_t)(cur - g.zero_begin);
    carve(cur, g.counters, (size_t)8);
    g.bytes = (size_t)(cur - reinterpret_cast<char*>(base));
    return g;
}

inline BinView bin_view(void* base, int64_t cap)
{
    BinView b;
    char* cur = reinterpret_cast<char*>(base);
    const size_t r = (size_t)(cap > 0 ? cap : 1);
    const size_t nblk = (size_t)sort_hist_stride((int64_t)r);
    carve(cur, b.key[0], r);
    carve(cur, b.key[1], r);
    carve(cur, b.val[0], r);
    carve(cur, b.val[1], r);
    carve(cur, b.hist, RADIX * nblk);
    carve(cur, b.totals, (size_t)RADIX);
    carve(cur, b.ckpt, ((r >> BWD_CHUNK_SHIFT_MIN) + 2) * 256);
    b.cap = (int64_t)r;
    b.bytes = (size_t)(cur - reinterpret_cast<char*>(base));
    return b;
}

inline int64_t bin_capacity_from_bytes(size_t bytes)
{
    if (bin_view(nullptr, 1).bytes > bytes) return 0;
    int64_t lo = 1, hi = (int64_t)(bytes / 16) + 1;
    while (lo < hi) {
        const int64_t mid = lo + (hi - lo + 1) / 2;
        if (bin_view(nullptr, mid).bytes <= bytes) lo = mid; else hi = mid - 1;
    }
    return lo;
}

struct XStateView {
    float* accum;
    float4* ckpt;
    size_t bytes;
};
inline XStateView xstate_view(void* base, int W, int H, int64_t cap, int nx)
{
    XStateView x;
    char* cur = reinterpret_cast<char*>(base);
    const size_t N = (size_t)W * (size_t)H, r = (size_t)(cap > 0 ? cap : 1);
    carve(cur, x.accum, (size_t)nx * (N ? N : 1));
    carve(cur, x.ckpt, ((r >> BWD_CHUNK_SHIFT_MIN) + 2) * (size_t)(nx / 4) * 256);
    x.bytes = (size_t)(cur - reinterpret_cast<char*>(base));
    return x;
}

inline ImageView image_view(void* base, int W, int H)
{
    ImageView v;
    char* cur = reinterpret_cast<char*>(base);
    const size_t N = (size_t)W * (size_t)H;
    const size_t T = (size_t)((W + TILE_X - 1) / TILE_X) * (size_t)((H + TILE_Y - 1) / TILE_Y);
    v.zero_begin = cur;
    carve(cur, v.tile_need, T ? T : 1);
    carve(cur, v.bwd_count, (size_t)16);
    v.zero_bytes = (size_t)(cur - v.zero_begin);
    carve(cur, v.ranges, T ? T : 1);
    carve(cur, v.final_T, N ? N : 1);
    carve(cur, v.n_contrib, N ? N : 1);
    carve(cur, v.tile_order, T ? T : 1);
    carve(cur, v.accum, 3 * (N ? N : 1));
    carve(cur, v.bwd_items, (size_t)BWD_MAX_CHUNKS * (T ? T : 1));
    v.bytes = (size_t)(cur - reinterpret_cast<char*>(base));
    return v;
}

inline uint32_t higher_msb(uint32_t n)
{
    uint32_t msb = sizeof(n) * 4;
    uint32_t step = msb;
    while (step > 1) {
        step /= 2;
        if (n >> msb) msb += step; else msb -= step;
    }
    if (n >> msb) msb++;
    return msb;
}

constexpr int DET_SLOT_WORDS = 16;
struct DetView {
    uint32_t* key[2];
    uint32_t* val[2];
    uint32_t* hist;
    uint32_t* totals;
    uint32_t* slot_base;
    uint64_t* count;
    uint32_t* flags;
    float* part;
    int64_t cap;
    size_t bytes;
};
inline DetView det_view(void* base, int T, int64_t cap)
{
    DetView d;
    char* cur = reinterpret_cast<char*>(base);
    const size_t r = (size_t)(cap > 0 ? cap : 1);
    carve(cur, d.key[0], r);
    carve(cur, d.key[1], r);
    carve(cur, d.val[0], r);
    carve(cur, d.val[1], r);
    carve(cur, d.hist, (size_t)RADIX * (size_t)sort_hist_stride((int64_t)r));
    carve(cur, d.totals, (size_t)RADIX);
    carve(cur, d.slot_base, (size_t)(T > 0 ? T : 1) + 1);
    carve(cur, d.count, (size_t)2);
    carve(cur, d.flags, r);
    carve(cur, d.part, r * 4 * DET_SLOT_WORDS);
    d.cap = (int64_t)r;
    d.bytes = (size_t)(cur - reinterpret_cast<char*>(base));
    return d;
}
struct RenderBwdDet {
    float* part;
    uint32_t* flags;
    const uint32_t* slot_base;
    size_t stride;
    uint32_t cap;
};

struct Launch {
    hipStream_t stream;
    int debug;
};

struct Batch {
    int V;
    int chunk_shift() const { return bwd_chunk_shift(V); }
    GeomView g;
    size_t g_stride;
    ImageView iv;
    size_t iv_stride;
    BinView b;
    size_t b_stride;
    float* grad_rec;
    size_t gr_stride;
};

int check_launch(const Launch& L, const char* what);

int launch_preprocess(const Launch& L, const gsr_params& p, const Batch& B, int* radii);
int launch_recolor(const Launch& L, const gsr_params& p, const Batch& B, size_t colors_view_stride);
int launch_mark_visible(const Launch& L, int P, const float* means3D, const float* view, uint8_t* present);
struct SortJob {
    uint32_t* key[2];
    uint32_t* val[2];
    uint32_t* hist;
    uint32_t* totals;
    size_t stride;
    const uint64_t* n_dev;
    size_t n_stride;
    int64_t cap;
    int V;
    uint32_t* blk_minmax = nullptr;
    uint32_t* sortctl = nullptr;
    bool small_blocks = false;
};
constexpr int SORTCTL_BASE = 0;
constexpr int SORTCTL_BITS = 1;
constexpr uint32_t CULLED_KEY = 0xFFFFFFFFu;
__host__ __device__ inline uint32_t depth_sort_passes(uint32_t bits) { return (bits + RADIX_BITS - 1) / RADIX_BITS; }
int launch_radix_sort_pairs(const Launch& L, const SortJob& job, bool iota_vals, int end_bit, int* result_buffer, bool key16 = false);
int block_tickets(int set);
inline bool tile_keys16(int T) { return T <= 65536; }
int launch_duplicate(const Launch& L, int P, const Batch& B, int gridx, bool key16, uint64_t* host_land);
int launch_tile_ranges(const Launch& L, const Batch& B, const uint32_t* sorted_keys, int T, bool key16);
int launch_tile_order(const Launch& L, const Batch& B, int T);
int launch_bwd_items(const Launch& L, const Batch& B, int T, int P);
struct ExtraChannels {
    int nx;
    const float* values;
    const float* view_scale;
    const float* bg;
    float* out;
    size_t view_stride;
    const float* values_hi = nullptr;
    size_t hi_view_stride = 0;
    XStateView state{nullptr, nullptr, 0};
    size_t state_stride = 0;
};
struct ExtraGrads {
    const float* dL_dextra;
    float* grad;
    float* grad_hi;
};
int launch_render_forward(const Launch& L, const gsr_params& p, const Batch& B, const uint32_t* point_list, float* out_color,
                          bool with_ckpt, const ExtraChannels* X = nullptr);
int launch_render_backward(const Launch& L, const gsr_params& p, const Batch& B, const uint32_t* point_list, const float* dL_dpix,
                           const ExtraChannels* X = nullptr, const ExtraGrads* XG = nullptr, const RenderBwdDet* D = nullptr);
int backward_subquadrant_moments(int set);
int forward_half_views(int set);
int selftest_mm(hipStream_t stream, float* d_scratch256);
int launch_det_prepare(const Launch& L, const Batch& B, const DetView& D, size_t d_stride, const uint32_t* point_list, int T);
int launch_det_sort(const Launch& L, const Batch& B, const DetView& D, size_t d_stride, int P, int* result_buffer);
int launch_det_reduce(const Launch& L, const Batch& B, const DetView& D, size_t d_stride, int sorted_buffer);
int selftest_det_reduce(hipStream_t stream);
#ifdef GSR_STATS
int debug_bwd_stats(unsigned long long* out8, int reset);
int debug_dup_times(unsigned long long* out8, int reset);
int debug_scatter_times(unsigned long long* out8, int reset);
int debug_fwd_times(unsigned long long* out8, int reset);
int debug_fwd_records(unsigned* out, int n);
int debug_bwd_times(unsigned long long* out8, int reset);
int debug_bwd_records(unsigned* out, int n);
#endif
int launch_preprocess_backward(const Launch& L, const gsr_params& p, const Batch& B, const int* radii, float* dL_dmean2D,
                               float* dL_dopacity, float* dL_dcolor, float* dL_dmean3D, float* dL_dcov3D, float* dL_dsh,
                               float* dL_dscale, float* dL_drot);

__device__ __forceinline__ void zero_region(char* p, size_t bytes, size_t gtid, size_t nthreads)
{
    uint4* q = reinterpret_cast<uint4*>(p);
    const size_t n = bytes / 16;
    for (size_t i = gtid; i < n; i += nthreads) q[i] = make_uint4(0u, 0u, 0u, 0u);
}

}
```

### gaussian-pcloud-render_amd/csrc/preprocess.hip

```cpp
#include "common.hpp"
#include "splat_math.hpp"
#include "tile_cull.hpp"

namespace gsr {

template <int deg>
__device__ __forceinline__ V3 sh_to_rgb_t(V3 pos, V3 campos, const float* sh, uint32_t* clamp_mask)
{
    V3 dir = pos - campos;
    const float len = sqrtf(dot3(dir, dir));
    dir = v3(dir.x / len, dir.y / len, dir.z / len);
#define SHV(k) v3(sh[3 * (k)], sh[3 * (k) + 1], sh[3 * (k) + 2])
    V3 result = kSH_C0 * SHV(0);
    if constexpr (deg > 0) {
        const float x = dir.x, y = dir.y, z = dir.z;
        result = ((result - (kSH_C1 * y) * SHV(1)) + (kSH_C1 * z) * SHV(2)) - (kSH_C1 * x) * SHV(3);
        if constexpr (deg > 1) {
            const float xx = x * x, yy = y * y, zz = z * z;
            const float xy = x * y, yz = y * z, xz = x * z;
            result = result + (kSH_C2[0] * xy) * SHV(4);
            result = result + (kSH_C2[1] * yz) * SHV(5);
            result = result + (kSH_C2[2] * (2.0f * zz - xx - yy)) * SHV(6);
            result = result + (kSH_C2[3] * xz) * SHV(7);
            result = result + (kSH_C2[4] * (xx - yy)) * SHV(8);
            if constexpr (deg > 2) {
                result = result + (kSH_C3[0] * y * (3.0f * xx - yy)) * SHV(9);
                result = result + (kSH_C3[1] * xy * z) * SHV(10);
                result = result + (kSH_C3[2] * y * (4.0f * zz - xx - yy)) * SHV(11);
                result = result + (kSH_C3[3] * z * (2.0f * zz - 3.0f * xx - 3.0f * yy)) * SHV(12);
                result = result + (kSH_C3[4] * x * (4.0f * zz - xx - yy)) * SHV(13);
                result = result + (kSH_C3[5] * z * (xx - yy)) * SHV(14);
                result = result + (kSH_C3[6] * x * (xx - 3.0f * yy)) * SHV(15);
            }
        }
    }
#undef SHV
    result.x += 0.5f;
    result.y += 0.5f;
    result.z += 0.5f;
    *clamp_mask = (result.x < 0 ? 1u : 0u) | (result.y < 0 ? 2u : 0u) | (result.z < 0 ? 4u : 0u);
    return v3(fmax_(result.x, 0.0f), fmax_(result.y, 0.0f), fmax_(result.z, 0.0f));
}

__device__ __forceinline__ V3 sh_to_rgb(int deg, V3 pos, V3 campos, const float* __restrict__ sh, uint32_t* clamp_mask)
{
    switch (deg) {
    case 0: return sh_to_rgb_t<0>(pos, campos, sh, clamp_mask);
    case 1: return sh_to_rgb_t<1>(pos, campos, sh, clamp_mask);
    case 2: return sh_to_rgb_t<2>(pos, campos, sh, clamp_mask);
    default: return sh_to_rgb_t<3>(pos, campos, sh, clamp_mask);
    }
}

__device__ __forceinline__ float ndc_to_pix(float v, int S) { return (float)((((double)v + 1.0) * (double)S - 1.0) * 0.5); }

__device__ __forceinline__ uint32_t clamp_tile(float f, uint32_t grid)
{
    int v = (int)f;
    v = v > 0 ? v : 0;
    return grid < (uint32_t)v ? grid : (uint32_t)v;
}

struct PreArgs {
    int P, D, M, W, H, V, vpt;
    float tanfovx, tanfovy, focal_x, focal_y, scale_modifier;
    int prefiltered, need_backward, reference_lists;
    uint32_t gridx, gridy;
    const float *means3D, *shs, *colors_precomp, *opacities, *scales, *rotations, *cov3D_precomp;
    const float *view, *proj, *campos;
    Splat* splat;
    uint32_t* tiles_touched;
    uint8_t* clamped;
    uint32_t* dkey;
    float* grad_rec;
    uint64_t* counters;
    char* g_zero;
    size_t g_zero_bytes, g_stride, gr_stride;
    char* iv_zero;
    size_t iv_zero_bytes, iv_stride;
    int* radii;
};

template <int DEG>
__global__ __launch_bounds__(256) void k_preprocess(PreArgs a)
{
    const int v_first = blockIdx.y * a.vpt, v_last = v_first + a.vpt < a.V ? v_first + a.vpt : a.V;
    const int idx_raw = blockIdx.x * 256 + threadIdx.x;
    {
        const size_t gtid = (size_t)blockIdx.x * 256 + threadIdx.x, nthr = (size_t)gridDim.x * 256;
        for (int vw = v_first; vw < v_last; vw++) {
            if (gtid == 0) {
                at_view(a.counters, a.g_stride, vw)[CNT_STALL] = 0;
                at_view(a.counters, a.g_stride, vw)[CNT_BWD_DIRTY] = 0;
            }
            zero_region(a.g_zero + a.g_stride * vw, a.g_zero_bytes, gtid, nthr);
            zero_region(a.iv_zero + a.iv_stride * vw, a.iv_zero_bytes, gtid, nthr);
        }
    }
    const bool valid = idx_raw < a.P;
    const int idx = valid ? idx_raw : a.P - 1;
    __shared__ float4 xpose[4][256];

    const V3 p_orig = v3(a.means3D[3 * idx], a.means3D[3 * idx + 1], a.means3D[3 * idx + 2]);
    float cov6[6];
    if (a.cov3D_precomp) {
#pragma unroll
        for (int i = 0; i < 6; i++) cov6[i] = a.cov3D_precomp[6 * (size_t)idx + i];
    } else {
        const V3 sc = v3(a.scales[3 * idx], a.scales[3 * idx + 1], a.scales[3 * idx + 2]);
        const float4 q = *reinterpret_cast<const float4*>(a.rotations + 4 * (size_t)idx);
        cov3d_from_scale_rot(sc, a.scale_modifier, q, cov6, nullptr);
    }
    const float opacity = a.opacities[idx];
    V3 rgb_pre = v3(0, 0, 0);
    constexpr int NSH = 3 * (DEG + 1) * (DEG + 1);
    float shv[NSH];
    if (a.colors_precomp) {
        rgb_pre = v3(a.colors_precomp[3 * idx], a.colors_precomp[3 * idx + 1], a.colors_precomp[3 * idx + 2]);
    } else {
        const float* shp = a.shs + (size_t)idx * a.M * 3;
#pragma unroll
        for (int i = 0; i < NSH; i++) shv[i] = shp[i];
    }

    for (int vw = v_first; vw < v_last; vw++) {
        float view[16], proj[16];
#pragma unroll
        for (int i = 0; i < 16; i++) {
            view[i] = a.view[16 * vw + i];
            proj[i] = a.proj[16 * vw + i];
        }

        int radius_out = 0;
        uint32_t tiles = 0, etiles = 0, key = 0xFFFFFFFFu, cmask = 0;
        uint2 rect = make_uint2(0, 0), spans = make_uint2(0, 0);
        bool spans_valid = false;
        Splat s;
        s.q0 = make_float4(0, 0, 0, 0);
        s.q1 = make_float4(0, 0, 0, 0);
        s.q2 = make_float4(0, 0, 0, 0);

        const V3 p_view = xform_point_4x3(p_orig, view);
        if (p_view.z <= 0.2f) {
            if (a.prefiltered && valid) at_view(a.counters, a.g_stride, vw)[CNT_TRAP] = 1;
        } else {
            const float hx = ((proj[0] * p_orig.x + proj[4] * p_orig.y) + proj[8] * p_orig.z) + proj[12];
            const float hy = ((proj[1] * p_orig.x + proj[5] * p_orig.y) + proj[9] * p_orig.z) + proj[13];
            const float hw = ((proj[3] * p_orig.x + proj[7] * p_orig.y) + proj[11] * p_orig.z) + proj[15];
            const float p_w = 1.0f / (hw + 0.0000001f);
            const float proj_x = hx * p_w, proj_y = hy * p_w;

            const Cov2D c = cov2d_project(p_orig, a.focal_x, a.focal_y, a.tanfovx, a.tanfovy, cov6, view);
            const float cov_x = c.cov.m[0][0] + 0.3f;
            const float cov_y = c.cov.m[0][1];
            const float cov_z = c.cov.m[1][1] + 0.3f;

            const float det = (cov_x * cov_z - cov_y * cov_y);
            if (det != 0.0f) {
                const float det_inv = 1.f / det;
                const float conic_x = cov_z * det_inv, conic_y = -cov_y * det_inv, conic_z = cov_x * det_inv;

                const float mid = 0.5f * (cov_x + cov_z);
                const float lambda1 = mid + sqrtf(fmax_(0.1f, mid * mid - det));
                const float lambda2 = mid - sqrtf(fmax_(0.1f, mid * mid - det));
                const float my_radius = ceilf(3.f * sqrtf(fmax_(lambda1, lambda2)));
                const float px = ndc_to_pix(proj_x, a.W), py = ndc_to_pix(proj_y, a.H);

                const float r = (float)(int)my_radius;
                const uint32_t minx = clamp_tile((px - r) / (float)TILE_X, a.gridx);
                const uint32_t miny = clamp_tile((py - r) / (float)TILE_Y, a.gridy);
                const uint32_t maxx = clamp_tile((((px + r) + (float)TILE_X) - 1.0f) / (float)TILE_X, a.gridx);
                const uint32_t maxy = clamp_tile((((py + r) + (float)TILE_Y) - 1.0f) / (float)TILE_Y, a.gridy);
                const uint32_t ntiles = (maxx - minx) * (maxy - miny);
                if (ntiles != 0) {
                    V3 rgb = rgb_pre;
                    if (!a.colors_precomp) {
                        const V3 cam = v3(a.campos[3 * vw], a.campos[3 * vw + 1], a.campos[3 * vw + 2]);
                        rgb = sh_to_rgb_t<DEG>(p_orig, cam, shv, &cmask);
                    }
                    radius_out = (int)my_radius;
                    tiles = ntiles;
                    key = __float_as_uint(p_view.z);
                    rect = make_uint2(minx | (miny << 16), maxx | (maxy << 16));
                    etiles = a.reference_lists ? ntiles
                                               : clip_rect_to_footprint(px, py, cov_x, cov_y, cov_z, det, conic_x, conic_y, conic_z,
#ifdef GSR_NO_SPANS
                                                                        opacity, r, rect, a.gridx, a.gridy);
#else
                                                                        opacity, r, rect, a.gridx, a.gridy, &spans, &spans_valid);
#endif
                    s.q0 = make_float4(px, py, conic_x, conic_y);
                    s.q1 = make_float4(conic_z, opacity, rgb.x, rgb.y);
                    s.q2 = make_float4(rgb.z, p_view.z, 0.f, 0.f);
                }
            }
        }

        if (valid) {
            a.radii[(size_t)vw * a.P + idx] = radius_out;
            at_view(a.tiles_touched, a.g_stride, vw)[idx] = tiles;
            at_view(a.dkey, a.g_stride, vw)[idx] = key;
        }
        const float4 q3 = spans_valid ? make_float4(__uint_as_float(rect.x), __uint_as_float(spans.x), __uint_as_float(spans.y),
                                                    __uint_as_float(tiles | SPANS_FLAG))
                                      : make_float4(__uint_as_float(rect.x), __uint_as_float(rect.y), __uint_as_float(etiles),
                                                    __uint_as_float(tiles));
        const int wave_first = idx_raw - (int)(threadIdx.x & 63);
        const bool full_wave = wave_first + 64 <= a.P;
        if (full_wave) {
            float4* mine = xpose[threadIdx.x >> 6] + 4 * (threadIdx.x & 63);
            mine[0] = s.q0; mine[1] = s.q1; mine[2] = s.q2; mine[3] = q3;
            __builtin_amdgcn_wave_barrier();
            const float4* rd = xpose[threadIdx.x >> 6] + (threadIdx.x & 63);
            float4* out = reinterpret_cast<float4*>(at_view(a.splat, a.g_stride, vw) + wave_first) + (threadIdx.x & 63);
            const float4 t0 = rd[0], t1 = rd[64], t2 = rd[128], t3 = rd[192];
            out[0] = t0; out[64] = t1; out[128] = t2; out[192] = t3;
            __builtin_amdgcn_wave_barrier();
        } else if (valid) {
            Splat* sp = at_view(a.splat, a.g_stride, vw) + idx;
            sp->q0 = s.q0;
            sp->q1 = s.q1;
            sp->q2 = s.q2;
            sp->q3 = q3;
        }
        if (a.need_backward && valid) {
            at_view(a.clamped, a.g_stride, vw)[idx] = (uint8_t)cmask;
            const float4 z = make_float4(0.f, 0.f, 0.f, 0.f);
            if (full_wave) {
                float4* recw = reinterpret_cast<float4*>(at_view(a.grad_rec, a.gr_stride, vw) + (size_t)wave_first * GRAD_REC_WORDS) + (threadIdx.x & 63);
                recw[0] = z; recw[64] = z; recw[128] = z; recw[192] = z;
            } else {
                float4* rec = reinterpret_cast<float4*>(at_view(a.grad_rec, a.gr_stride, vw) + (size_t)idx * GRAD_REC_WORDS);
                rec[0] = z; rec[1] = z; rec[2] = z; rec[3] = z;
            }
        }
    }
}

int launch_preprocess(const Launch& L, const gsr_params& p, const Batch& B, int* radii)
{
    const GeomView& g = B.g;
    PreArgs a;
    a.P = p.P; a.D = p.D; a.M = p.M; a.W = p.W; a.H = p.H;
    a.tanfovx = p.tanfovx; a.tanfovy = p.tanfovy;
    a.focal_y = p.H / (2.0f * p.tanfovy);
    a.focal_x = p.W / (2.0f * p.tanfovx);
    a.scale_modifier = p.scale_modifier;
    a.prefiltered = p.prefiltered;
    a.need_backward = p.need_backward;
    a.reference_lists = p.reference_lists;
    a.gridx = (uint32_t)((p.W + TILE_X - 1) / TILE_X);
    a.gridy = (uint32_t)((p.H + TILE_Y - 1) / TILE_Y);
    a.means3D = p.means3D; a.shs = p.shs; a.colors_precomp = p.colors_precomp; a.opacities = p.opacities;
    a.scales = p.scales; a.rotations = p.rotations; a.cov3D_precomp = p.cov3D_precomp;
    a.view = p.viewmatrix; a.proj = p.projmatrix; a.campos = p.campos;
    a.splat = g.splat; a.tiles_touched = g.tiles_touched; a.clamped = g.clamped;
    a.dkey = g.dkey[0]; a.radii = radii; a.counters = g.counters; a.grad_rec = B.grad_rec; a.gr_stride = B.gr_stride;
    a.g_zero = g.zero_begin; a.g_zero_bytes = g.zero_bytes; a.g_stride = B.g_stride;
    a.iv_zero = B.iv.zero_begin; a.iv_zero_bytes = B.iv.zero_bytes; a.iv_stride = B.iv_stride;
    const int blocks = (p.P + 255) / 256;
    a.V = B.V;
    a.vpt = 1;
    while (a.vpt < B.V && (int64_t)blocks * div_up(B.V, a.vpt * 2) >= 2048) a.vpt *= 2;
    if (a.vpt > B.V) a.vpt = B.V;
    const dim3 grid(blocks, (unsigned)div_up(B.V, a.vpt));
    switch (p.shs ? p.D : 0) {
    case 0: hipLaunchKernelGGL(k_preprocess<0>, grid, dim3(256), 0, L.stream, a); break;
    case 1: hipLaunchKernelGGL(k_preprocess<1>, grid, dim3(256), 0, L.stream, a); break;
    case 2: hipLaunchKernelGGL(k_preprocess<2>, grid, dim3(256), 0, L.stream, a); break;
    default: hipLaunchKernelGGL(k_preprocess<3>, grid, dim3(256), 0, L.stream, a); break;
    }
    return check_launch(L, "preprocess");
}

__global__ __launch_bounds__(256) void k_recolor(int P, int D, int M, const float* __restrict__ means3D,
                                                 const float* __restrict__ shs, const float* __restrict__ colors_precomp,
                                                 const float* __restrict__ campos, const uint32_t* __restrict__ tiles_touched,
                                                 Splat* __restrict__ splat, uint8_t* __restrict__ clamped, size_t g_stride,
                                                 size_t colors_view_stride)
{
    const uint32_t vw = blockIdx.y;
    if (colors_precomp) colors_precomp += colors_view_stride * vw;
    tiles_touched = at_view(tiles_touched, g_stride, vw);
    splat = at_view(splat, g_stride, vw);
    if (campos) campos += 3 * vw;
    const int idx = blockIdx.x * 256 + threadIdx.x;
    if (idx >= P || tiles_touched[idx] == 0) return;
    V3 rgb;
    uint32_t cmask = 0;
    if (colors_precomp) {
        rgb = v3(colors_precomp[3 * idx], colors_precomp[3 * idx + 1], colors_precomp[3 * idx + 2]);
    } else {
        const V3 pos = v3(means3D[3 * idx], means3D[3 * idx + 1], means3D[3 * idx + 2]);
        rgb = sh_to_rgb(D, pos, v3(campos[0], campos[1], campos[2]), shs + (size_t)idx * M * 3, &cmask);
    }
    float* rec = reinterpret_cast<float*>(splat + idx);
    rec[6] = rgb.x;
    rec[7] = rgb.y;
    rec[8] = rgb.z;
    if (clamped) at_view(clamped, g_stride, vw)[idx] = (uint8_t)cmask;
}

int launch_recolor(const Launch& L, const gsr_params& p, const Batch& B, size_t colors_view_stride)
{
    hipLaunchKernelGGL(k_recolor, dim3((p.P + 255) / 256, B.V), dim3(256), 0, L.stream, p.P, p.D, p.M, p.means3D, p.shs,
                       p.colors_precomp, p.campos, B.g.tiles_touched, B.g.splat, p.need_backward ? B.g.clamped : nullptr, B.g_stride,
                       colors_view_stride);
    return check_launch(L, "recolor");
}

__global__ __launch_bounds__(256) void k_mark_visible(int P, const float* __restrict__ means3D,
                                                      const float* __restrict__ view, uint8_t* __restrict__ present)
{
    const int idx = blockIdx.x * 256 + threadIdx.x;
    if (idx >= P) return;
    const V3 p = v3(means3D[3 * idx], means3D[3 * idx + 1], means3D[3 * idx + 2]);
    const float z = ((view[2] * p.x + view[6] * p.y) + view[10] * p.z) + view[14];
    present[idx] = !(z <= 0.2f);
}

int launch_mark_visible(const Launch& L, int P, const float* means3D, const float* view, uint8_t* present)
{
    hipLaunchKernelGGL(k_mark_visible, dim3((P + 255) / 256), dim3(256), 0, L.stream, P, means3D, view, present);
    return check_launch(L, "mark_visible");
}

}
```

### gaussian-pcloud-render_amd/csrc/sort.hip

```cpp
#include "common.hpp"

namespace gsr {

__device__ __forceinline__ uint32_t lane_id() { return __builtin_amdgcn_mbcnt_hi(~0u, __builtin_amdgcn_mbcnt_lo(~0u, 0u)); }

__device__ __forceinline__ uint32_t wave_inclusive_scan(uint32_t v, uint32_t lane)
{
#pragma unroll
    for (int d = 1; d < 64; d <<= 1) {
        const uint32_t n = __shfl_up(v, d, 64);
        if (lane >= (uint32_t)d) v += n;
    }
    return v;
}

__device__ __forceinline__ uint32_t block_exclusive_scan_256(uint32_t v, uint32_t* tmp, uint32_t* total)
{
    const uint32_t lane = threadIdx.x & 63, w = threadIdx.x >> 6;
    const uint32_t inc = wave_inclusive_scan(v, lane);
    if (lane == 63) tmp[w] = inc;
    __syncthreads();
    uint32_t base = 0;
#pragma unroll
    for (int i = 0; i < 4; i++)
        if ((uint32_t)i < w) base += tmp[i];
    if (total) *total = tmp[0] + tmp[1] + tmp[2] + tmp[3];
    __syncthreads();
    return base + inc - v;
}

struct SortView {
    size_t stride;
    const uint64_t* n_dev;
    size_t n_stride;
    int64_t cap;
    const uint32_t* ctl;
};
__device__ __forceinline__ bool pass_control(const SortView& sv, uint32_t view, int shift, uint32_t& base)
{
    base = 0u;
    if (sv.ctl == nullptr) return true;
    const uint32_t* c = at_view(sv.ctl, sv.stride, view);
    base = c[SORTCTL_BASE];
    return (uint32_t)shift < c[SORTCTL_BITS];
}
__device__ __forceinline__ int64_t view_count(const SortView& sv, uint32_t view)
{
    if (sv.n_dev == nullptr) return sv.cap;
    const uint64_t n = *at_view(sv.n_dev, sv.n_stride, view);
    return n < (uint64_t)sv.cap ? (int64_t)n : sv.cap;
}

constexpr int HIST_GROUP = 16;

template <typename KeyT, int RS_ITEMS>
__global__ __launch_bounds__(RS_THREADS) void k_radix_hist(const KeyT* __restrict__ keys, SortView sv, int shift,
                                                           uint32_t mask, uint32_t* __restrict__ hist, int nblk_pad,
                                                           uint32_t* __restrict__ minmax)
{
    constexpr int RS_TILE = RS_THREADS * RS_ITEMS;
    const uint32_t view = blockIdx.y;
    uint32_t kbase;
    if (!pass_control(sv, view, shift, kbase)) return;
    const int64_t n = view_count(sv, view);
    keys = at_view(keys, sv.stride, view);
    hist = at_view(hist, sv.stride, view);
    if (minmax) minmax = at_view(minmax, sv.stride, view);
    const uint32_t d = threadIdx.x;
    if ((int64_t)blockIdx.x * RS_TILE >= n) {
        if (d <= mask) hist[(size_t)d * nblk_pad + blockIdx.x] = 0;
        if (minmax && d == 0) { minmax[blockIdx.x] = 0xFFFFFFFFu; minmax[nblk_pad + blockIdx.x] = 0u; }
        return;
    }
    constexpr int HIST_COPIES = 4 * RS_WAVES;
    __shared__ __attribute__((aligned(16))) uint32_t h[HIST_COPIES][RADIX];
    __shared__ uint32_t s_min, s_max;
    for (int i = threadIdx.x; i < HIST_COPIES * RADIX / 4; i += RS_THREADS) reinterpret_cast<uint4*>(&h[0][0])[i] = make_uint4(0, 0, 0, 0);
    if (threadIdx.x == 0) { s_min = 0xFFFFFFFFu; s_max = 0u; }
    __syncthreads();
    uint32_t kmin = 0xFFFFFFFFu, kmax = 0u;
    const int64_t base = (int64_t)blockIdx.x * RS_TILE;
    const uint32_t w = (threadIdx.x >> 6) * 4u + (threadIdx.x & 3u);
    if (sizeof(KeyT) == 2 && RS_ITEMS % 8 == 0 && base + RS_TILE <= n) {
        const uint4* k4 = reinterpret_cast<const uint4*>(keys + base) + threadIdx.x * (RS_ITEMS / 8);
#pragma unroll
        for (int v = 0; v < RS_ITEMS / 8; v++) {
            const uint4 q = k4[v];
            const uint32_t wds[4] = {q.x, q.y, q.z, q.w};
#pragma unroll
            for (int j = 0; j < 4; j++) {
                atomicAdd(&h[w][((wds[j] & 0xFFFFu) >> shift) & mask], 1u);
                atomicAdd(&h[w][((wds[j] >> 16) >> shift) & mask], 1u);
            }
        }
    } else {
#pragma unroll
        for (int i = 0; i < RS_ITEMS; i++) {
            const int64_t idx = base + i * RS_THREADS + threadIdx.x;
            if (idx < n) {
                const uint32_t key = (uint32_t)keys[idx];
                atomicAdd(&h[w][((key - kbase) >> shift) & mask], 1u);
                if (key != CULLED_KEY) { kmin = key < kmin ? key : kmin; kmax = key > kmax ? key : kmax; }
            }
        }
    }
    if (minmax) {
#pragma unroll
        for (int dd = 32; dd >= 1; dd >>= 1) {
            const uint32_t a = __shfl_xor(kmin, dd, 64), b = __shfl_xor(kmax, dd, 64);
            kmin = a < kmin ? a : kmin;
            kmax = b > kmax ? b : kmax;
        }
        if ((threadIdx.x & 63) == 0) { atomicMin(&s_min, kmin); atomicMax(&s_max, kmax); }
    }
    __syncthreads();
    if (minmax && d == 0) { minmax[blockIdx.x] = s_min; minmax[nblk_pad + blockIdx.x] = s_max; }
    if (d <= mask) {
        uint32_t c = 0;
#pragma unroll
        for (int i = 0; i < HIST_COPIES; i++) c += h[i][d];
        hist[(size_t)d * nblk_pad + blockIdx.x] = c;
    }
}

__global__ __launch_bounds__(256) void k_radix_rowscan(uint32_t* __restrict__ hist, uint32_t* __restrict__ totals, int nblk_pad,
                                                       size_t stride, const uint32_t* __restrict__ ctl, int shift,
                                                       const uint32_t* __restrict__ minmax, uint32_t* __restrict__ ctl_out,
                                                       uint32_t nrows)
{
    __shared__ uint32_t tmp[4];
    if (blockIdx.x == nrows) {
        minmax = at_view(minmax, stride, blockIdx.y);
        uint32_t kmin = 0xFFFFFFFFu, kmax = 0u;
        for (int b = threadIdx.x; b < nblk_pad; b += 256) {
            const uint32_t a = minmax[b], c = minmax[nblk_pad + b];
            kmin = a < kmin ? a : kmin;
            kmax = c > kmax ? c : kmax;
        }
        __shared__ uint32_t s_min, s_max;
        if (threadIdx.x == 0) { s_min = 0xFFFFFFFFu; s_max = 0u; }
        __syncthreads();
        atomicMin(&s_min, kmin);
        atomicMax(&s_max, kmax);
        __syncthreads();
        if (threadIdx.x == 0) {
            uint32_t* c = at_view(ctl_out, stride, blockIdx.y);
            const uint32_t base = s_min <= s_max ? (s_min & ~(uint32_t)(RADIX - 1)) : 0u;
            const uint32_t span = s_min <= s_max ? s_max - base : 0u;
            const uint32_t bits = span ? 32u - (uint32_t)__builtin_clz(span) : 0u;
            c[SORTCTL_BASE] = base;
            c[SORTCTL_BITS] = bits < (uint32_t)RADIX_BITS ? (uint32_t)RADIX_BITS : bits;
        }
        return;
    }
    if (ctl != nullptr && (uint32_t)shift >= at_view(ctl, stride, blockIdx.y)[SORTCTL_BITS]) return;
    hist = at_view(hist, stride, blockIdx.y);
    totals = at_view(totals, stride, blockIdx.y);
    uint32_t* row = hist + (size_t)blockIdx.x * nblk_pad;
    uint32_t carry = 0;
    for (int b0 = 0; b0 < nblk_pad; b0 += 256) {
        const int b = b0 + threadIdx.x;
        const uint32_t v = b < nblk_pad ? row[b] : 0u;
        uint32_t tot;
        const uint32_t ex = block_exclusive_scan_256(v, tmp, &tot);
        if (b < nblk_pad) row[b] = carry + ex;
        carry += tot;
    }
    if (threadIdx.x == 0) totals[blockIdx.x] = carry;
}

#ifdef GSR_STATS
constexpr int SC_REC = 65536;
__device__ unsigned g_sc_rec[SC_REC][5];
#define SC_T(var) const unsigned long long var = wall_clock64()
#define SC_PUT(i, v) do { if (threadIdx.x == 0) { const unsigned r_ = blockIdx.y * gridDim.x + blockIdx.x; if (r_ < SC_REC) g_sc_rec[r_][i] = (unsigned)(v); } } while (0)
int debug_scatter_times(unsigned long long* out8, int reset)
{
    static unsigned host[SC_REC][5];
    if (hipMemcpyFromSymbol(host, HIP_SYMBOL(g_sc_rec), sizeof(host)) != hipSuccess) return -1;
    for (int i = 0; i < 8; i++) out8[i] = 0;
    for (int r = 0; r < SC_REC; r++) {
        if (host[r][1] == 0) continue;
        for (int i = 0; i < 5; i++) out8[i] += host[r][i];
        out8[5]++;
    }
    if (reset) {
        for (int r = 0; r < SC_REC; r++) for (int i = 0; i < 5; i++) host[r][i] = 0;
        if (hipMemcpyToSymbol(HIP_SYMBOL(g_sc_rec), host, sizeof(host)) != hipSuccess) return -1;
    }
    return 0;
}
#else
#define SC_T(var) do { } while (0)
#define SC_PUT(i, v) do { } while (0)
#endif

template <int BITS, typename KeyT, int RS_ITEMS>
__global__ __launch_bounds__(RS_THREADS) void k_radix_scatter(const KeyT* __restrict__ keys_in,
                                                              const uint32_t* __restrict__ vals_in,
                                                              KeyT* __restrict__ keys_out,
                                                              uint32_t* __restrict__ vals_out, SortView sv, int shift,
                                                              uint32_t mask, const uint32_t* __restrict__ hist,
                                                              const uint32_t* __restrict__ totals, int nblk_pad)
{
    constexpr int RS_TILE = RS_THREADS * RS_ITEMS;
    const uint32_t view = blockIdx.y;
    uint32_t kbase;
    if (!pass_control(sv, view, shift, kbase)) return;
    const int64_t n = view_count(sv, view);
    const uint32_t wg = blockIdx.x, xcd = wg & 7u, r = wg >> 3;
    const uint32_t blk = ((r / HIST_GROUP) * 8u + xcd) * HIST_GROUP + (r % HIST_GROUP);
    hist = at_view(hist, sv.stride, view);
    totals = at_view(totals, sv.stride, view);
    if ((int64_t)blk * RS_TILE >= n) return;
    keys_in = at_view(keys_in, sv.stride, view);
    if (vals_in) vals_in = at_view(vals_in, sv.stride, view);
    keys_out = at_view(keys_out, sv.stride, view);
    vals_out = at_view(vals_out, sv.stride, view);
    __shared__ uint32_t s_key[RS_TILE];
    __shared__ uint32_t s_val[RS_TILE];
    __shared__ uint32_t wave_cnt[RS_WAVES][RADIX];
    __shared__ uint32_t local_base[RADIX];
    __shared__ uint32_t global_base[RADIX];
    __shared__ uint32_t tmp[4];

    const uint32_t tid = threadIdx.x, lane = tid & 63, w = tid >> 6;
    const int64_t blk_base = (int64_t)blk * RS_TILE;
    const int64_t seg_base = blk_base + (int64_t)w * (RS_TILE / RS_WAVES);

    for (int i = lane; i < RADIX; i += 64) wave_cnt[w][i] = 0;
    SC_T(t0);

    const uint32_t tot_d = tid <= mask ? totals[tid] : 0u;
    const uint32_t hist_d = tid <= mask ? hist[(size_t)tid * nblk_pad + blk] : 0u;

    uint32_t k[RS_ITEMS], v[RS_ITEMS], rank[RS_ITEMS];
    const bool full = blk_base + RS_TILE <= n;
    {
        const KeyT* kp = keys_in + seg_base + lane;
        const uint32_t* vp = vals_in ? vals_in + seg_base + lane : nullptr;
        if (full) {
#pragma unroll
            for (int j = 0; j < RS_ITEMS; j++) k[j] = (uint32_t)kp[j * 64] - kbase;
            if (vp) {
#pragma unroll
                for (int j = 0; j < RS_ITEMS; j++) v[j] = vp[j * 64];
            } else {
#pragma unroll
                for (int j = 0; j < RS_ITEMS; j++) v[j] = (uint32_t)(seg_base + j * 64 + lane);
            }
        } else {
#pragma unroll
            for (int j = 0; j < RS_ITEMS; j++) {
                const int64_t idx = seg_base + j * 64 + lane;
                const bool ok = idx < n;
                k[j] = ok ? (uint32_t)kp[j * 64] - kbase : 0xFFFFFFFFu;
                v[j] = ok ? (vp ? vp[j * 64] : (uint32_t)idx) : 0u;
            }
        }
    }
    uint32_t gbase_d = block_exclusive_scan_256(tot_d, tmp, nullptr) + hist_d;
    __builtin_amdgcn_wave_barrier();
#ifdef GSR_STATS
    asm volatile("s_waitcnt vmcnt(0)" ::: "memory");
#endif
    SC_T(t1);
    SC_PUT(0, t1 - t0);

#pragma unroll
    for (int j = 0; j < RS_ITEMS; j++) {
        const bool ok = full || seg_base + j * 64 + lane < n;
        const uint32_t d = (k[j] >> shift) & mask;
        const uint64_t okb = full ? ~0ull : __ballot(ok);
        uint32_t plo = (uint32_t)okb, phi = (uint32_t)(okb >> 32);
#pragma unroll
        for (int b = 0; b < BITS; b++) {
            const uint32_t m = (uint32_t)__builtin_amdgcn_sbfe((int32_t)k[j], (uint32_t)(shift + b), 1u);
            const uint64_t bal = __ballot(m != 0u);
            plo = __builtin_amdgcn_bitop3_b32(plo, (uint32_t)bal, m, 0x90);
            phi = __builtin_amdgcn_bitop3_b32(phi, (uint32_t)(bal >> 32), m, 0x90);
        }
        const uint32_t before = wave_cnt[w][d];
        const uint32_t below = __builtin_amdgcn_mbcnt_hi(phi, __builtin_amdgcn_mbcnt_lo(plo, 0u));
        rank[j] = before + below;
        __builtin_amdgcn_wave_barrier();
        if (ok && below == 0) wave_cnt[w][d] = before + (uint32_t)__popc(plo) + (uint32_t)__popc(phi);
        __builtin_amdgcn_wave_barrier();
    }
    __syncthreads();
    SC_T(t2);
    SC_PUT(1, t2 - t1);

    {
        const uint32_t d = tid;
        uint32_t c[RS_WAVES], run = 0;
#pragma unroll
        for (int i = 0; i < RS_WAVES; i++) {
            c[i] = wave_cnt[i][d];
            wave_cnt[i][d] = run;
            run += c[i];
        }
        const uint32_t lbase = block_exclusive_scan_256(run, tmp, nullptr);
        local_base[d] = lbase;
        global_base[d] = gbase_d;
    }
    __syncthreads();
    SC_T(t3);
    SC_PUT(2, t3 - t2);

#pragma unroll
    for (int j = 0; j < RS_ITEMS; j++) {
        if (full || seg_base + j * 64 + lane < n) {
            const uint32_t d = (k[j] >> shift) & mask;
            const uint32_t pos = local_base[d] + wave_cnt[w][d] + rank[j];
            s_key[pos] = k[j];
            s_val[pos] = v[j];
        }
    }
    __syncthreads();
    SC_T(t4);
    SC_PUT(3, t4 - t3);

    const int64_t rem = n - blk_base;
    const uint32_t count = rem < RS_TILE ? (uint32_t)rem : (uint32_t)RS_TILE;
#pragma unroll
    for (int i = 0; i < RS_ITEMS; i++) {
        const uint32_t p = i * RS_THREADS + tid;
        if (p < count) {
            const uint32_t key = s_key[p];
            const uint32_t d = (key >> shift) & mask;
            const size_t g = (size_t)global_base[d] + (p - local_base[d]);
            keys_out[g] = (KeyT)(key + kbase);
            vals_out[g] = s_val[p];
        }
    }
#ifdef GSR_STATS
    { SC_T(t5); SC_PUT(4, t5 - t4); }
#endif
}

int launch_radix_sort_pairs(const Launch& L, const SortJob& job, bool iota_vals, int end_bit, int* result_buffer, bool key16)
{
    int cur = 0;
    if (job.cap > 0 && job.V > 0) {
        const bool small = job.small_blocks && !key16 && end_bit % RADIX_BITS == 0;
        const int tile = small ? RS_TILE_SMALL : RS_TILE;
        const int nblk = (int)div_up(job.cap, tile);
        const int nblk_pad = sort_hist_stride(job.cap, tile);
        SortView sv{job.stride, job.n_dev, job.n_stride, job.cap, nullptr};
        const dim3 grid_hist(nblk_pad, job.V);
        const dim3 grid((unsigned)div_up(nblk, 8 * HIST_GROUP) * 8 * HIST_GROUP, job.V);
        bool first = true;
        const int npass = (end_bit + RADIX_BITS - 1) / RADIX_BITS;
        int shift = 0;
        for (int pass = 0; pass < npass; pass++) {
            const int bits = (end_bit - shift + (npass - pass) - 1) / (npass - pass);
            const uint32_t mask = (1u << bits) - 1u;
            const bool make_ctl = job.sortctl != nullptr && pass == 0;
            sv.ctl = (job.sortctl != nullptr && pass > 0) ? job.sortctl : nullptr;
            uint32_t* minmax = make_ctl ? job.blk_minmax : nullptr;
            if (key16)
                hipLaunchKernelGGL((k_radix_hist<uint16_t, RS_ITEMS>), grid_hist, dim3(RS_THREADS), 0, L.stream, (const uint16_t*)job.key[cur], sv,
                                   shift, mask, job.hist, nblk_pad, minmax);
            else if (small)
                hipLaunchKernelGGL((k_radix_hist<uint32_t, RS_ITEMS_SMALL>), grid_hist, dim3(RS_THREADS), 0, L.stream, (const uint32_t*)job.key[cur], sv,
                                   shift, mask, job.hist, nblk_pad, minmax);
            else
                hipLaunchKernelGGL((k_radix_hist<uint32_t, RS_ITEMS>), grid_hist, dim3(RS_THREADS), 0, L.stream, (const uint32_t*)job.key[cur], sv,
                                   shift, mask, job.hist, nblk_pad, minmax);
            if (int e = check_launch(L, "radix_hist")) return e;
            hipLaunchKernelGGL(k_radix_rowscan, dim3(mask + 1u + (make_ctl ? 1u : 0u), job.V), dim3(256), 0, L.stream, job.hist,
                               job.totals, nblk_pad, job.stride, sv.ctl, shift, (const uint32_t*)minmax, job.sortctl, mask + 1u);
            if (int e = check_launch(L, "radix_rowscan")) return e;
            const uint32_t* vin = (first && iota_vals) ? (const uint32_t*)nullptr : (const uint32_t*)job.val[cur];
#define GSR_SCATTER(B)                                                                                                        \
    case B:                                                                                                                   \
        if (key16)                                                                                                            \
            hipLaunchKernelGGL((k_radix_scatter<B, uint16_t, RS_ITEMS>), grid, dim3(RS_THREADS), 0, L.stream,                 \
                               (const uint16_t*)job.key[cur], vin, (uint16_t*)job.key[cur ^ 1], job.val[cur ^ 1], sv, shift,  \
                               mask, job.hist, job.totals, nblk_pad);                                                         \
        else                                                                                                                  \
            hipLaunchKernelGGL((k_radix_scatter<B, uint32_t, RS_ITEMS>), grid, dim3(RS_THREADS), 0, L.stream,                 \
                               (const uint32_t*)job.key[cur], vin, job.key[cur ^ 1], job.val[cur ^ 1], sv, shift, mask,       \
                               job.hist, job.totals, nblk_pad);                                                               \
        break;
            if (small)
                hipLaunchKernelGGL((k_radix_scatter<RADIX_BITS, uint32_t, RS_ITEMS_SMALL>), grid, dim3(RS_THREADS), 0, L.stream,
                                   (const uint32_t*)job.key[cur], vin, job.key[cur ^ 1], job.val[cur ^ 1], sv, shift, mask, job.hist,
                                   job.totals, nblk_pad);
            else switch (bits) {
                GSR_SCATTER(1) GSR_SCATTER(2) GSR_SCATTER(3) GSR_SCATTER(4) GSR_SCATTER(5) GSR_SCATTER(6) GSR_SCATTER(7)
                GSR_SCATTER(8)
            }
#undef GSR_SCATTER
            if (int e = check_launch(L, "radix_scatter")) return e;
            cur ^= 1;
            first = false;
            shift += bits;
        }
    } else {
        cur = ((end_bit + RADIX_BITS - 1) / RADIX_BITS) & 1;
    }
    *result_buffer = cur;
    return GSR_OK;
}

}
```

### gaussian-pcloud-render_amd/diff_gaussian_rasterization/_native.py

```python
import ctypes as C
import os
import threading
import weakref as _weakref

import torch

_HERE = os.path.dirname(os.path.abspath(__file__))
LIB_PATH = os.environ.get("GSR_LIB") or os.path.join(_HERE, "libgsr_hip.so")

_fp = C.c_void_p


class GsrParams(C.Structure):
    _fields_ = [
        ("P", C.c_int), ("D", C.c_int), ("M", C.c_int), ("W", C.c_int), ("H", C.c_int),
        ("tanfovx", C.c_float), ("tanfovy", C.c_float), ("scale_modifier", C.c_float),
        ("prefiltered", C.c_int), ("debug", C.c_int), ("need_backward", C.c_int), ("reference_lists", C.c_int),
        ("bg", _fp), ("means3D", _fp), ("shs", _fp), ("colors_precomp", _fp), ("opacities", _fp),
        ("scales", _fp), ("rotations", _fp), ("cov3D_precomp", _fp),
        ("viewmatrix", _fp), ("projmatrix", _fp), ("campos", _fp),
    ]


GSR_RETRY = 1

Q = dict(DEPTHS=1, MEANS2D=2, CONIC_OPACITY=3, RGB=4, TILES_TOUCHED=5, POINT_LIST=6, POINT_LIST_KEYS=7, RANGES=8,
         FINAL_T=9, N_CONTRIB=10, CLAMPED=11, TILE_NEED=12, DEPTH_SORT=13, LIST_PAIRS=14)

_int, _i64, _size, _pp = C.c_int, C.c_int64, C.c_size_t, C.POINTER(GsrParams)
_ARENAS = [_fp, _size, _fp, _size, _fp, _size]
_FWD = [_pp, _int] + _ARENAS + [_fp, _fp, C.POINTER(_i64), _int]
_FWD_X = _FWD + [_int, _int, _fp, _fp, _fp, _fp]
_BWD = [_pp, _int, _fp] + _ARENAS + [_fp] * 9
_DECL = {
    "gsr_geom_bytes": (_size, [_int]),
    "gsr_geom_bytes_inference": (_size, [_int]),
    "gsr_image_bytes": (_size, [_int, _int]),
    "gsr_binning_bytes": (_size, [_i64]),
    "gsr_extra_state_bytes": (_size, [_int, _int, _i64, _int]),
    "gsr_backward_det_bytes": (_size, [_int, _int, _int, _int, _i64]),
    "gsr_forward_batch": (_int, _FWD + [_fp]),
    "gsr_forward_batch_channels": (_int, _FWD_X + [_fp]),
    "gsr_forward_batch_channels_train": (_int, _FWD_X + [_fp, _size, _fp]),
    "gsr_forward_stage1": (_int, [_pp, _fp, _size, _fp, _size, _fp, C.POINTER(_i64), _fp]),
    "gsr_forward_stage2": (_int, [_pp] + _ARENAS + [_i64, _fp, _fp]),
    "gsr_forward_recolor": (_int, [_pp, _int, _int] + _ARENAS + [_fp, _fp]),
    "gsr_backward_batch": (_int, _BWD + [_fp]),
    "gsr_backward_batch_det": (_int, _BWD + [_fp, _size, _fp]),
    "gsr_backward_batch_channels": (_int, _BWD + [_int, _int, _fp, _fp, _fp, _fp, _size, _fp, _fp, _fp]),
    "gsr_backward": (_int, [_pp, _fp, _i64] + _ARENAS + [_fp] * 9 + [_fp]),
    "gsr_mark_visible": (_int, [_int, _fp, _fp, _fp, _fp, _fp]),
    "gsr_query": (_int, [_pp, _int, _fp, _fp, _size, _fp, _i64, _fp, _size, _fp]),
    "gsr_set_profiling": (None, [_int]),
    "gsr_set_forward_half_views": (_int, [_int]),
    "gsr_set_backward_moments": (_int, [_int]),
    "gsr_get_profile": (_int, [C.POINTER(C.c_char_p), C.POINTER(C.c_float), _int]),
    "gsr_selftest": (_int, [_fp]),
    "gsr_d2h_count": (C.c_longlong, []),
    "gsr_clock_probe_launch": (_int, [_fp, _int, _fp]),
    "gsr_wall_clock_khz": (_int, []),
    "gsr_last_list_pairs": (_int, [C.POINTER(_i64), _int]),
}
_RESTYPE_ONLY = {"gsr_last_error": C.c_char_p, "gsr_version": C.c_char_p}
SYMBOLS = tuple(_DECL) + tuple(_RESTYPE_ONLY)


def _load():
    if not os.path.exists(LIB_PATH):
        raise ImportError(
            "diff_gaussian_rasterization: %s not found - build it with "
            "`python gaussian-pcloud-render_amd/build.py` (hipcc, gfx950). There is no CPU fallback." % LIB_PATH)
    lib = C.CDLL(LIB_PATH)
    for name, (restype, argtypes) in _DECL.items():
        getattr(lib, name).restype, getattr(lib, name).argtypes = restype, argtypes
    for name, restype in _RESTYPE_ONLY.items():
        getattr(lib, name).restype = restype
    return lib


lib = _load()


def _ptr(t):
    if t is None or t.numel() == 0:
        return None
    return t.data_ptr()


def _check(rc):
    if rc != 0:
        raise RuntimeError(lib.gsr_last_error().decode("utf-8", "replace"))


def _f32c(t, device, name):
    if t.numel() == 0:
        return t
    if t.dtype != torch.float32:
        raise RuntimeError("expected scalar type Float but found %s for %s" % (t.dtype, name))
    if t.device == device and t.is_contiguous():
        return t
    return t.to(device).contiguous()


_raw_stream = getattr(torch._C, "_cuda_getCurrentRawStream", None)


def _stream_handle(device):
    if _raw_stream is not None and device.index is not None:
        return _raw_stream(device.index)
    return torch.cuda.current_stream(device).cuda_stream


class _NoContext:
    def __enter__(self):
        return self

    def __exit__(self, *exc):
        return False

    @staticmethod
    def give(*tensors):
        return tensors[0] if len(tensors) == 1 else tensors


_NO_CONTEXT = _NoContext()


def _on_device(device):
    if device.index is None or device.index == torch.cuda.current_device():
        return _NO_CONTEXT
    return torch.cuda.device(device)


def _require_hip(device):
    if device.type != "cuda":
        raise RuntimeError(
            "diff_gaussian_rasterization (MI355X build) needs tensors on a HIP device (torch device 'cuda'); got %s. "
            "There is no CPU path." % device)


def _params(bg, means3D, colors, opacity, scales, rotations, scale_modifier, cov3D_precomp, viewmatrix, projmatrix,
            tan_fovx, tan_fovy, H, W, sh, degree, campos, prefiltered, debug, need_backward):
    device = means3D.device
    keep = (_f32c(bg, device, "bg"), _f32c(means3D, device, "means3D"), _f32c(sh, device, "sh"),
            _f32c(colors, device, "colors_precomp"), _f32c(opacity, device, "opacities"), _f32c(scales, device, "scales"),
            _f32c(rotations, device, "rotations"), _f32c(cov3D_precomp, device, "cov3D_precomp"),
            _f32c(viewmatrix, device, "viewmatrix"), _f32c(projmatrix, device, "projmatrix"), _f32c(campos, device, "campos"))
    M = int(sh.shape[1]) if sh.numel() != 0 and sh.shape[0] != 0 else 0
    p = GsrParams(means3D.shape[0], int(degree), M, int(W), int(H), float(tan_fovx), float(tan_fovy), float(scale_modifier),
                  int(bool(prefiltered)), int(bool(debug)), int(bool(need_backward)), int(reference_lists()),
                  *[_ptr(t) for t in keep])
    return p, keep


_REFERENCE_LISTS = [os.environ.get("GSR_REFERENCE_LISTS", "0") not in ("", "0")]
_TLS = threading.local()


def reference_lists():
    return getattr(_TLS, "reference_lists", _REFERENCE_LISTS[0])


def set_reference_lists(on):
    old = getattr(_TLS, "reference_lists", None)
    if on is None:
        if hasattr(_TLS, "reference_lists"):
            del _TLS.reference_lists
    else:
        _TLS.reference_lists = bool(on)
    return old


_DETERMINISTIC = [{"0": False, "1": True}.get(os.environ.get("GSR_DETERMINISTIC", "").strip())]
CALLS = dict(backward=0, backward_det=0)


def set_deterministic(flag):
    _DETERMINISTIC[0] = None if flag is None else bool(flag)


def get_deterministic():
    return _DETERMINISTIC[0]


def deterministic_active():
    f = _DETERMINISTIC[0]
    return bool(torch.are_deterministic_algorithms_enabled()) if f is None else f


def last_list_pairs(V):
    pairs = (C.c_int64 * V)()
    _check(lib.gsr_last_list_pairs(pairs, V))
    return int(max(pairs))


def det_scratch(V, P, W, H, pairs, binning_bytes, device):
    if pairs is None:
        pairs = max(1, int(binning_bytes) // max(1, V) // 16)
    return torch.empty((int(lib.gsr_backward_det_bytes(V, P, W, H, int(pairs))),), dtype=torch.uint8, device=device)


_CAP_HINT = {}
CAP_SLACK = 1.25


def _cap_key(device, P, W, H):
    return (device.index if device.index is not None else torch.cuda.current_device(), int(P), int(W), int(H))


def _note_counts(key, counts):
    old = _CAP_HINT.get(key, 0)
    _CAP_HINT[key] = max(max(counts), int(old * 0.98))


def reset_capacity_hints():
    _CAP_HINT.clear()


_ARENA_BYTES, _IMAGE_BYTES = {}, {}


def _arena_bytes(P, need_backward):
    k = (P, bool(need_backward))
    b = _ARENA_BYTES.get(k)
    if b is None:
        if len(_ARENA_BYTES) > 256:
            _ARENA_BYTES.clear()
        b = _ARENA_BYTES[k] = int(lib.gsr_geom_bytes(P) if need_backward else lib.gsr_geom_bytes_inference(P))
    return b


def _image_bytes(W, H):
    k = (W, H)
    b = _IMAGE_BYTES.get(k)
    if b is None:
        if len(_IMAGE_BYTES) > 256:
            _IMAGE_BYTES.clear()
        b = _IMAGE_BYTES[k] = int(lib.gsr_image_bytes(W, H))
    return b



if os.environ.get("GSR_SET_HW_QUEUES", "0") == "1" and not torch.cuda.is_initialized():
    os.environ.setdefault("GPU_MAX_HW_QUEUES", "8")

_OVERLAP_ON = os.environ.get("GSR_OVERLAP", "0") == "1"
_OVERLAP_STREAMS = int(os.environ.get("GSR_OVERLAP_STREAMS", "3"))
_OVERLAP_PRIORITY = int(os.environ.get("GSR_OVERLAP_PRIORITY", "-1"))
OVERLAP_MAX_VIEWS = 3
_OVERLAP = {}
OVERLAP_STATS = dict(calls=0, overlapped=0)


def set_overlap(on):
    global _OVERLAP_ON
    _OVERLAP_ON = bool(on)


class _OverlapState:
    def __init__(self, device, cur):
        self.streams = [torch.cuda.Stream(device=device, priority=_OVERLAP_PRIORITY) for _ in range(_OVERLAP_STREAMS)]
        self.turn = 0
        self.seen = {}
        self.seq = 0

    @staticmethod
    def _where(t):
        return (t.data_ptr(), t.storage_offset(), tuple(t.shape), tuple(t.stride()), t.dtype)

    def input_event(self, tensors, cur):
        self.seq += 1
        newest, missing = None, []
        for t in tensors:
            try:
                ver = t._version
            except RuntimeError:
                return self._now(cur, []), False
            rec = self.seen.get(id(t))
            if rec is not None and rec[0]() is t and rec[1] == ver and rec[4] == self._where(t):
                if newest is None or rec[3] > newest[3]:
                    newest = rec
            else:
                missing.append((t, ver))
        if missing or newest is None:
            return self._now(cur, missing), False
        return newest[2], True

    def _now(self, cur, missing):
        ev = torch.cuda.Event()
        ev.record(cur)
        if len(self.seen) > 512:
            self.seen = {k: r for k, r in self.seen.items() if r[0]() is not None}
            if len(self.seen) > 512:
                self.seen.clear()
        for t, ver in missing:
            self.seen[id(t)] = (_weakref.ref(t), ver, ev, self.seq, self._where(t))
        return ev

    def next_stream(self):
        self.turn = (self.turn + 1) % len(self.streams)
        return self.streams[self.turn]


class _OnSideStream:

    def __init__(self, device, tensors):
        self.device, self.active, self.out = device, False, []
        if device.type != "cuda":
            return
        self.cur = torch.cuda.current_stream(device)
        key = (device.index if device.index is not None else torch.cuda.current_device(), self.cur.cuda_stream)
        st = _OVERLAP.get(key)
        if st is None:
            st = _OVERLAP[key] = _OverlapState(device, self.cur)
        live = [t for t in tensors if isinstance(t, torch.Tensor) and t.numel() != 0 and t.device.type == "cuda"]
        ev, early = st.input_event(live, self.cur)
        OVERLAP_STATS["calls"] += 1
        OVERLAP_STATS["overlapped"] += int(early)
        self.side = st.next_stream()
        self.side.wait_event(ev)
        self.active = True

    def give(self, *tensors):
        self.out += [t for t in tensors if isinstance(t, torch.Tensor) and t.numel() != 0]
        return tensors[0] if len(tensors) == 1 else tensors

    def __enter__(self):
        if self.active:
            self.ctx = torch.cuda.stream(self.side)
            self.ctx.__enter__()
        return self

    def __exit__(self, *exc):
        if self.active:
            self.ctx.__exit__(*exc)
            done = torch.cuda.Event()
            done.record(self.side)
            self.cur.wait_event(done)
            for t in self.out:
                t.record_stream(self.cur)
        return False


def _extra_layout(extra, P, V, device):
    xv, xs, xb = extra
    if isinstance(xv, (tuple, list)):
        lo, hi = xv
        if tuple(lo.shape) != (P, 4) or tuple(hi.shape) != (V, P, 4):
            raise RuntimeError("split extra channels must have shapes (num_points, 4) and (num_views, num_points, 4)")
        xv = torch.cat([_f32c(lo, device, "extra").reshape(-1), _f32c(hi, device, "extra").reshape(-1)])
        x_per_view, nx = 2, 8
    else:
        x_per_view = int(xv.dim() == 3)
        nx = int(xv.shape[-1]) if xv.dim() in (2, 3) else -1
        if nx not in (4, 8) or xv.shape[-2] != P or (x_per_view and xv.shape[0] != V):
            raise RuntimeError("extra channels must have shape (num_points, 4 or 8) or (num_views, num_points, 4 or 8)")
    if xb.numel() != nx or (xs is not None and tuple(xs.shape) != (V, nx)):
        raise RuntimeError("bg_extra must have nx entries and view_scale shape (V, nx)")
    return nx, x_per_view, xv, xs, xb
# ... 422 lines not shown
```

### include/gsr.h

```cpp
#ifndef GSR_H
#define GSR_H

#include <stddef.h>
#include <stdint.h>

#ifdef __cplusplus
extern "C" {
#endif

#define GSR_OK 0
#define GSR_ERR_INVALID (-1)
#define GSR_ERR_HIP (-2)
#define GSR_ERR_CAPACITY (-3)
#define GSR_ERR_TRAP (-4)
#define GSR_RETRY 1

typedef void* gsr_stream_t;

typedef struct gsr_params {
    int P;
    int D;
    int M;
    int W, H;
    float tanfovx, tanfovy;
    float scale_modifier;
    int prefiltered;
    int debug;
    int need_backward;
    int reference_lists;
    const float* bg;
    const float* means3D;
    const float* shs;
    const float* colors_precomp;
    const float* opacities;
    const float* scales;
    const float* rotations;
    const float* cov3D_precomp;
    const float* viewmatrix;
    const float* projmatrix;
    const float* campos;
} gsr_params;

size_t gsr_geom_bytes(int P);
size_t gsr_geom_bytes_inference(int P);
size_t gsr_image_bytes(int W, int H);
size_t gsr_binning_bytes(int64_t num_rendered);

int gsr_forward_batch(const gsr_params* p, int V, void* geom, size_t geom_bytes, void* image, size_t image_bytes,
                      void* binning, size_t binning_bytes, int* radii, float* out_color, int64_t* num_rendered,
                      int resume, gsr_stream_t stream);

int gsr_forward_batch_channels(const gsr_params* p, int V, void* geom, size_t geom_bytes, void* image, size_t image_bytes,
                               void* binning, size_t binning_bytes, int* radii, float* out_color, int64_t* num_rendered, int resume,
                               int nx, int extra_per_view, const float* extra, const float* extra_view_scale, const float* bg_extra,
                               float* out_extra, gsr_stream_t stream);

size_t gsr_extra_state_bytes(int W, int H, int64_t num_rendered, int nx);
int gsr_forward_batch_channels_train(const gsr_params* p, int V, void* geom, size_t geom_bytes, void* image, size_t image_bytes,
                                     void* binning, size_t binning_bytes, int* radii, float* out_color, int64_t* num_rendered,
                                     int resume, int nx, int extra_per_view, const float* extra, const float* extra_view_scale,
                                     const float* bg_extra, float* out_extra, void* extra_state, size_t extra_state_bytes,
                                     gsr_stream_t stream);

int gsr_forward_stage1(const gsr_params* p, void* geom, size_t geom_bytes, void* image, size_t image_bytes,
                       int* radii, int64_t* num_rendered_out, gsr_stream_t stream);

int gsr_forward_stage2(const gsr_params* p, void* geom, size_t geom_bytes, void* binning, size_t binning_bytes,
                       void* image, size_t image_bytes, int64_t num_rendered, float* out_color, gsr_stream_t stream);

int gsr_forward_recolor(const gsr_params* p, int V, int colors_per_view, void* geom, size_t geom_bytes, const void* binning,
                        size_t binning_bytes, void* image, size_t image_bytes, float* out_color, gsr_stream_t stream);

int gsr_backward_batch(const gsr_params* p, int V, const int* radii, const void* geom, size_t geom_bytes, const void* binning,
                       size_t binning_bytes, const void* image, size_t image_bytes, const float* dL_dpix, float* dL_dmean2D,
                       float* dL_dopacity, float* dL_dcolor, float* dL_dmean3D, float* dL_dcov3D, float* dL_dsh,
                       float* dL_dscale, float* dL_drot, gsr_stream_t stream);

size_t gsr_backward_det_bytes(int V, int P, int W, int H, int64_t pairs);
int gsr_backward_batch_det(const gsr_params* p, int V, const int* radii, const void* geom, size_t geom_bytes, const void* binning,
                           size_t binning_bytes, const void* image, size_t image_bytes, const float* dL_dpix, float* dL_dmean2D,
                           float* dL_dopacity, float* dL_dcolor, float* dL_dmean3D, float* dL_dcov3D, float* dL_dsh,
                           float* dL_dscale, float* dL_drot, void* det_scratch, size_t det_scratch_bytes, gsr_stream_t stream);

int gsr_backward_batch_channels(const gsr_params* p, int V, const int* radii, const void* geom, size_t geom_bytes, const void* binning,
                                size_t binning_bytes, const void* image, size_t image_bytes, const float* dL_dpix, float* dL_dmean2D,
                                float* dL_dopacity, float* dL_dcolor, float* dL_dmean3D, float* dL_dcov3D, float* dL_dsh,
                                float* dL_dscale, float* dL_drot, int nx, int extra_per_view, const float* extra,
                                const float* extra_view_scale, const float* bg_extra, const void* extra_state, size_t extra_state_bytes,
                                const float* dL_dextra, float* dL_dextra_values, gsr_stream_t stream);

int gsr_backward(const gsr_params* p, const int* radii, int64_t num_rendered, const void* geom, size_t geom_bytes,
                 const void* binning, size_t binning_bytes, const void* image, size_t image_bytes,
                 const float* dL_dpix , float* dL_dmean2D, float* dL_dopacity,
                 float* dL_dcolor, float* dL_dmean3D, float* dL_dcov3D, float* dL_dsh, float* dL_dscale,
                 float* dL_drot, gsr_stream_t stream);

int gsr_last_list_pairs(int64_t* out, int V);

int gsr_mark_visible(int P, const float* means3D, const float* viewmatrix, const float* projmatrix,
                     uint8_t* present, gsr_stream_t stream);

#define GSR_Q_DEPTHS 1
#define GSR_Q_MEANS2D 2
#define GSR_Q_CONIC_OPACITY 3
#define GSR_Q_RGB 4
#define GSR_Q_TILES_TOUCHED 5
#define GSR_Q_POINT_LIST 6
#define GSR_Q_POINT_LIST_KEYS 7
#define GSR_Q_RANGES 8
#define GSR_Q_FINAL_T 9
#define GSR_Q_N_CONTRIB 10
#define GSR_Q_TILE_NEED 12
#define GSR_Q_CLAMPED 11
#define GSR_Q_LIST_PAIRS 14
#define GSR_Q_DEPTH_SORT 13
int gsr_query(const gsr_params* p, int what, const void* geom, const void* binning, size_t binning_bytes, const void* image,
              int64_t num_rendered, void* dst, size_t dst_bytes, gsr_stream_t stream);

void gsr_set_profiling(int on);
int gsr_get_profile(const char** names, float* ms, int cap);

int gsr_clock_probe_launch(void* dst16, int iters, gsr_stream_t stream);
int gsr_wall_clock_khz(void);

int gsr_selftest(gsr_stream_t stream);

long long gsr_d2h_count(void);

int gsr_set_forward_half_views(int views);

int gsr_set_backward_moments(int mode);

const char* gsr_last_error(void);
const char* gsr_version(void);

#ifdef __cplusplus
}
#endif
#endif
```

Before: 2132.

## Fuse tile-key pair emission with first radix pass via digit-counting duplicate

Replaces the single-pass decoupled-lookback duplicate kernel (ticketed blocks spinning on status words) with three steps. A count kernel builds per-block histograms of the low tile-key digit using LDS difference arrays. A rowscan produces pair offsets, totals and host landing values. The duplicate kernel then scatters pairs directly into first-radix-pass order, so the tile sort skips its first pass. This removes inter-block spin-waiting and one full sort pass, at the cost of an extra launch and a second read of splat rectangles.

```diff
diff --git a/gaussian-pcloud-render_amd/csrc/api.hip b/gaussian-pcloud-render_amd/csrc/api.hip
--- a/gaussian-pcloud-render_amd/csrc/api.hip
+++ b/gaussian-pcloud-render_amd/csrc/api.hip
@@ -110,13 +110,6 @@
 static thread_local std::vector<int64_t> t_list_pairs;
 
 static std::atomic<long long> g_d2h_count{0};
-
-static std::atomic<int> g_tickets{[] { const char* e = getenv("GSR_TICKETS"); return e && atoi(e) == 0 ? 0 : 1; }()};
-int block_tickets(int set)
-{
-    if (set >= 0) g_tickets = set != 0;
-    return g_tickets;
-}
 
 static int tile_count(const gsr_params* p) { return ((p->W + TILE_X - 1) / TILE_X) * ((p->H + TILE_Y - 1) / TILE_Y); }
 
@@ -144,7 +137,6 @@
     return GSR_OK;
 }
 
-static int tile_bits(int T) { return (int)higher_msb((uint32_t)T); }
 static int sorted_buffer(int T) { return ((tile_bits(T) + RADIX_BITS - 1) / RADIX_BITS) & 1; }
 
 static inline void* align256(void* p) { return (void*)(((uintptr_t)p + 255) & ~(uintptr_t)255); }
@@ -266,7 +258,6 @@
     memset(t_land.pinned, 0, (size_t)V * 4 * sizeof(uint64_t));
 
     if (mode == 1) {
-        if (int e = memset_views(L.stream, B.g.zero_begin, B.g_stride, B.g.zero_bytes, V)) return e;
         if (int e = memset_views(L.stream, B.iv.zero_begin, B.iv_stride, B.iv.zero_bytes, V)) return e;
     } else {
         if (p->prefiltered)
@@ -288,12 +279,13 @@
     const auto rest = [&]() -> int {
         {
             ProfScope ps("duplicate", L.stream);
-            if (int e = launch_duplicate(L, p->P, B, gridx, key16, t_land.mapped)) return e;
-        }
-        {
+            if (int e = launch_dup_count(L, p->P, B, gridx, T)) return e;
+            if (int e = launch_emit_rowscan(L, p->P, B, emit_digit_bits(T), t_land.mapped)) return e;
             g_d2h_count++;
-            const hipError_t e = hipEventRecord(t_land.ev, L.stream);
-            if (e != hipSuccess) return fail(GSR_ERR_HIP, "[gsr] num_rendered read-back: %s", hipGetErrorString(e));
+            const hipError_t ev = hipEventRecord(t_land.ev, L.stream);
+            if (ev != hipSuccess) return fail(GSR_ERR_HIP, "[gsr] num_rendered read-back: %s", hipGetErrorString(ev));
+            if (mode != 2)
+                if (int e = launch_duplicate(L, p->P, B, gridx, T, key16)) return e;
         }
         if (mode != 2) {
             const int res = sorted_buffer(T);
@@ -302,7 +294,7 @@
                 SortJob job{{B.b.key[0], B.b.key[1]}, {B.b.val[0], B.b.val[1]}, B.b.hist, B.b.totals, B.b_stride,
                             B.g.counters + CNT_NUM_RENDERED, B.g_stride, B.b.cap, V};
                 int r2 = 0;
-                if (int e = launch_radix_sort_pairs(L, job, false, tile_bits(T), &r2, key16)) return e;
+                if (int e = launch_radix_sort_pairs(L, job, false, tile_bits(T), &r2, key16, true)) return e;
             }
             {
                 ProfScope ps("tile_ranges", L.stream);
@@ -326,8 +318,6 @@
     t_list_pairs.assign((size_t)V, 0);
     for (int v = 0; v < V; v++) {
         const uint64_t R = t_land.pinned[4 * v + LAND_NUM_REFERENCE], Lp = t_land.pinned[4 * v + CNT_NUM_RENDERED];
-        if (t_land.pinned[4 * v + CNT_STALL])
-            return fail(GSR_ERR_HIP, "[gsr] pair emission: a workgroup's pair count never arrived (view %d)", v);
         if (p->prefiltered && t_land.pinned[4 * v + CNT_TRAP])
             return fail(GSR_ERR_TRAP, "Point is filtered although prefiltered is set. This shouldn't happen!");
         if (R > 0x7FFFFFFFull)
@@ -847,6 +837,14 @@
     for (auto& kv : g_prof) { kv.second.rec.clear(); kv.second.used = 0; }
 }
 
+int gsr_tile_sort_split(int T, int* widths)
+{
+    const int end_bit = tile_bits(T > 0 ? T : 1), npass = radix_pass_count(end_bit);
+    for (int i = 0; i < npass && i < 4; i++) widths[i] = radix_pass_bits(end_bit, i);
+    return npass;
+}
+int gsr_emit_digit_bits(int T) { return emit_digit_bits(T > 0 ? T : 1); }
+
 int gsr_get_profile(const char** names, float* ms, int cap)
 {
     std::lock_guard<std::mutex> lk(g_prof_mu);
@@ -875,7 +873,6 @@
 __attribute__((visibility("default"))) int gsr_debug_fwd_records(unsigned* out, int n) { return gsr::debug_fwd_records(out, n); }
 __attribute__((visibility("default"))) int gsr_debug_bwd_times(unsigned long long* out8, int reset) { return gsr::debug_bwd_times(out8, reset); }
 __attribute__((visibility("default"))) int gsr_debug_bwd_records(unsigned* out, int n) { return gsr::debug_bwd_records(out, n); }
-__attribute__((visibility("default"))) int gsr_debug_dup_times(unsigned long long* out8, int reset) { return gsr::debug_dup_times(out8, reset); }
 #endif
 
 long long gsr_d2h_count(void) { return gsr::g_d2h_count.load(); }
diff --git a/gaussian-pcloud-render_amd/csrc/binning.hip b/gaussian-pcloud-render_amd/csrc/binning.hip
--- a/gaussian-pcloud-render_amd/csrc/binning.hip
+++ b/gaussian-pcloud-render_amd/csrc/binning.hip
@@ -1,89 +1,88 @@
 #include "common.hpp"
+#include "radix_scatter.hpp"
 #include "tile_cull.hpp"
 
 namespace gsr {
 
-__device__ __forceinline__ uint64_t agent_load(const uint64_t* p)
-{
-    return __hip_atomic_load(p, __ATOMIC_RELAXED, __HIP_MEMORY_SCOPE_AGENT);
-}
-__device__ __forceinline__ void agent_store(uint64_t* p, uint64_t v)
-{
-    __hip_atomic_store(p, v, __ATOMIC_RELAXED, __HIP_MEMORY_SCOPE_AGENT);
-}
-
-#ifdef GSR_STATS
-constexpr int DUP_REC = 65536;
-__device__ unsigned g_dup_rec[DUP_REC][4];
-#define DUP_T(var) const unsigned long long var = wall_clock64()
-#define DUP_ADD(i, v) do { if (threadIdx.x == 0) { const unsigned r_ = blockIdx.y * gridDim.x + s_ticket; if (r_ < DUP_REC) g_dup_rec[r_][i] = (unsigned)(v); } } while (0)
-int debug_dup_times(unsigned long long* out8, int reset)
-{
-    static unsigned host[DUP_REC][4];
-    if (hipMemcpyFromSymbol(host, HIP_SYMBOL(g_dup_rec), sizeof(host)) != hipSuccess) return -1;
-    for (int i = 0; i < 8; i++) out8[i] = 0;
-    for (int r = 0; r < DUP_REC; r++) {
-        if (host[r][0] == 0 && host[r][1] == 0) continue;
-        for (int i = 0; i < 4; i++) out8[i] += host[r][i];
-        out8[4]++;
-    }
-    if (reset) {
-        for (int r = 0; r < DUP_REC; r++) for (int i = 0; i < 4; i++) host[r][i] = 0;
-        if (hipMemcpyToSymbol(HIP_SYMBOL(g_dup_rec), host, sizeof(host)) != hipSuccess) return -1;
-    }
-    return 0;
-}
-#else
-#define DUP_T(var) do { } while (0)
-#define DUP_ADD(i, v) do { } while (0)
-#endif
-
-struct DupArgs {
+struct EmitRow {
+    uint32_t t0, n;
+};
+__device__ __forceinline__ uint32_t emit_rows(uint32_t idf, uint32_t r0, uint32_t r1, uint32_t pairs)
+{
+    if (idf & SPANS_FLAG) return SPAN_ROWS;
+    return pairs ? (r1 >> 16) - (r0 >> 16) : 0u;
+}
+__device__ __forceinline__ EmitRow emit_row(uint32_t idf, uint32_t r0, uint32_t r1, uint32_t r2, uint32_t gridx, uint32_t row)
+{
+    const uint32_t minx = r0 & 0xFFFFu, miny = r0 >> 16;
+    EmitRow e;
+    if (idf & SPANS_FLAG) {
+        const uint32_t byte = ((row < 4u ? r1 : r2) >> (8u * (row & 3u))) & 0xFFu;
+        e.t0 = (miny + row) * gridx + minx + (byte & 15u);
+        e.n = byte >> 4;
+    } else {
+        e.t0 = (miny + row) * gridx + minx;
+        e.n = (r1 & 0xFFFFu) - minx;
+    }
+    return e;
+}
+__device__ __forceinline__ uint32_t emit_pairs(uint32_t w3, uint32_t r1, uint32_t r2)
+{
+    if (!(w3 & SPANS_FLAG)) return r2;
+    const uint32_t a4 = (r1 >> 4) & 0x0F0F0F0Fu, b4 = (r2 >> 4) & 0x0F0F0F0Fu;
+    return (a4 * 0x01010101u + b4 * 0x01010101u) >> 24;
+}
+
+struct DupCountArgs {
     int P;
     uint32_t gridx;
     const uint32_t* order[2];
     const uint32_t* sortctl;
     const Splat* splat;
-    uint64_t* dup_status;
-    uint64_t* counters;
+    uint64_t* wg;
+    uint32_t* hist;
     size_t g_stride;
-    void* keys;
-    uint32_t* vals;
-    size_t b_stride;
-    int64_t cap;
-    uint64_t* host_land;
-    int tickets;
+    int nblk;
+    uint32_t bits;
 };
 
-template <typename KeyT>
-__global__ __launch_bounds__(DUP_THREADS) void k_duplicate(DupArgs a)
-{
-    __shared__ uint32_t s_off[4][64];
-    __shared__ uint32_t s_id[4][64];
-    __shared__ uint2 s_rect[4][64];
-    __shared__ uint32_t s_sp2[4][64];
-    __shared__ uint2 s_pre[4][64];
-    __shared__ uint32_t s_flag[4][64];
+constexpr uint32_t DUP_LANE_ROWS = 8;
+
+__device__ __forceinline__ void count_row(int* diff, uint32_t* all, uint32_t t0, uint32_t n, uint32_t bits, uint32_t mask)
+{
+    const uint32_t turns = n >> bits, m = n & mask;
+    if (turns) atomicAdd(all, turns);
+    if (m) {
+        const uint32_t d0 = t0 & mask, e = d0 + m;
+        atomicAdd(&diff[d0], 1);
+        if (e <= mask + 1u) {
+            atomicSub(&diff[e], 1);
+        } else {
+            atomicAdd(&diff[0], 1);
+            atomicSub(&diff[e - (mask + 1u)], 1);
+        }
+    }
+}
+
+__global__ __launch_bounds__(DUP_THREADS) void k_dup_count(DupCountArgs a)
+{
+    __shared__ int s_diff[4][RADIX + 1];
+    __shared__ uint32_t s_all[4];
     __shared__ uint64_t s_wave[4];
     __shared__ uint64_t s_ref[4];
-    __shared__ uint64_t s_base;
-    __shared__ uint32_t s_ticket;
-    const uint32_t view = blockIdx.y;
+    __shared__ uint32_t s_tmp[4];
+    const uint32_t view = blockIdx.y, blk = blockIdx.x;
     const uint32_t lane = threadIdx.x & 63, w = threadIdx.x >> 6;
-    uint64_t* status = at_view(a.dup_status, a.g_stride, view);
-    const uint32_t nblk = gridDim.x;
-    DUP_T(t0);
-    if (threadIdx.x == 0) s_ticket = a.tickets ? (uint32_t)atomicAdd((unsigned long long*)&status[DUP_COPIES * nblk], 1ull) : blockIdx.x;
-    __syncthreads();
-    DUP_T(t1);
-    DUP_ADD(0, t1 - t0);
-    const uint32_t blk = s_ticket;
+    const uint32_t mask = (1u << a.bits) - 1u;
+    uint32_t* hist = at_view(a.hist, a.g_stride, view);
+    uint64_t* wg = at_view(a.wg, a.g_stride, view);
+    for (int i = threadIdx.x; i < 4 * (RADIX + 1); i += DUP_THREADS) (&s_diff[0][0])[i] = 0;
+    if (threadIdx.x < 4) s_all[threadIdx.x] = 0u;
     const uint32_t npass = depth_sort_passes(at_view(a.sortctl, a.g_stride, view)[SORTCTL_BITS]);
     const uint32_t* order = at_view((npass & 1u) ? a.order[1] : a.order[0], a.g_stride, view);
     const Splat* splat = at_view(a.splat, a.g_stride, view);
 
-    uint32_t cnt[DUP_G], id[DUP_G], sp2[DUP_G];
-    uint2 rc[DUP_G];
+    uint32_t cnt[DUP_G], id[DUP_G], r0[DUP_G], r1[DUP_G], r2[DUP_G];
     uint64_t ref_cnt = 0;
     const int slot0 = (int)(blk * DUP_BLOCK + w * (64 * DUP_G) + lane);
 #pragma unroll
@@ -93,208 +92,257 @@
     }
 #pragma unroll
     for (int g = 0; g < DUP_G; g++) {
-        cnt[g] = 0;
-        rc[g] = make_uint2(0, 0);
-        sp2[g] = 0;
+        cnt[g] = r0[g] = r1[g] = r2[g] = 0u;
         if (slot0 + g * 64 < a.P) {
             const float4 q3 = splat[id[g]].q3;
             const uint32_t w3 = __float_as_uint(q3.w);
-            rc[g] = make_uint2(__float_as_uint(q3.x), __float_as_uint(q3.y));
-            sp2[g] = __float_as_uint(q3.z);
-            if (w3 & SPANS_FLAG) {
-                const uint32_t a4 = (rc[g].y >> 4) & 0x0F0F0F0Fu, b4 = (sp2[g] >> 4) & 0x0F0F0F0Fu;
-                const uint32_t pa = a4 * 0x01010101u;
-                const uint32_t pb = b4 * 0x01010101u + (pa >> 24) * 0x01010101u;
-                cnt[g] = pb >> 24;
-                id[g] |= SPANS_FLAG;
-            } else {
-                cnt[g] = sp2[g];
-            }
+            r0[g] = __float_as_uint(q3.x);
+            r1[g] = __float_as_uint(q3.y);
+            r2[g] = __float_as_uint(q3.z);
+            cnt[g] = emit_pairs(w3, r1[g], r2[g]);
+            id[g] |= w3 & SPANS_FLAG;
             ref_cnt += w3 & ~SPANS_FLAG;
         }
     }
-    uint64_t excl[DUP_G];
     uint64_t run = 0;
 #pragma unroll
-    for (int g = 0; g < DUP_G; g++) {
-        uint64_t inc64 = cnt[g];
-#pragma unroll
-        for (int d = 1; d < 64; d <<= 1) {
-            const uint64_t n = (uint64_t)__shfl_up((unsigned long long)inc64, d, 64);
-            if (lane >= (uint32_t)d) inc64 += n;
-        }
-        excl[g] = run + inc64 - cnt[g];
-        run += (uint64_t)__shfl((unsigned long long)inc64, 63, 64);
-    }
-#pragma unroll
-    for (int d = 32; d >= 1; d >>= 1) ref_cnt += (uint64_t)__shfl_xor((unsigned long long)ref_cnt, d, 64);
+    for (int g = 0; g < DUP_G; g++) run += cnt[g];
+#pragma unroll
+    for (int d = 32; d >= 1; d >>= 1) {
+        ref_cnt += (uint64_t)__shfl_xor((unsigned long long)ref_cnt, d, 64);
+        run += (uint64_t)__shfl_xor((unsigned long long)run, d, 64);
+    }
     if (lane == 63) { s_wave[w] = run; s_ref[w] = ref_cnt; }
     __syncthreads();
-    uint64_t wave_base = 0;
-#pragma unroll
-    for (int i = 0; i < 4; i++)
-        if ((uint32_t)i < w) wave_base += s_wave[i];
-    const uint64_t block_total = s_wave[0] + s_wave[1] + s_wave[2] + s_wave[3];
-    const uint64_t block_ref = s_ref[0] + s_ref[1] + s_ref[2] + s_ref[3];
-    const uint64_t sat = 0xFFFFFFFEull;
-    const uint64_t word = ((block_total < sat ? block_total : sat) + 1ull) | ((block_ref < 0xFFFFFFFFull ? block_ref : 0xFFFFFFFFull) << 32);
-    if (threadIdx.x < DUP_COPIES) agent_store(&status[threadIdx.x * nblk + blk], word);
-    DUP_T(t2);
-    DUP_ADD(1, t2 - t1);
-    uint64_t part = 0, part_ref = 0;
-    constexpr uint32_t LB = 4;
-    const uint64_t* mine = status + (size_t)(blk % DUP_COPIES) * nblk;
-    for (uint32_t b0 = threadIdx.x; b0 < blk; b0 += DUP_THREADS * LB) {
-        uint64_t v[LB];
-#pragma unroll
-        for (uint32_t k = 0; k < LB; k++) {
-            const uint32_t b = b0 + k * DUP_THREADS;
-            v[k] = b < blk ? agent_load(&mine[b]) : 1ull;
-        }
-#pragma unroll
-        for (uint32_t k = 0; k < LB; k++) {
-            uint32_t spins = 0;
-            while ((uint32_t)v[k] == 0u) {
-                v[k] = agent_load(&mine[b0 + k * DUP_THREADS]);
-                if ((uint32_t)v[k] == 0u && ++spins > (1u << 24)) {
-                    at_view(a.counters, a.g_stride, view)[CNT_STALL] = 1;
-                    a.host_land[4 * view + CNT_STALL] = 1;
-                    v[k] = 1;
-                }
-            }
-            part += (v[k] & 0xFFFFFFFFull) - 1;
-            part_ref += v[k] >> 32;
-        }
-    }
-#pragma unroll
-    for (int d = 32; d >= 1; d >>= 1) {
-        part += (uint64_t)__shfl_xor((unsigned long long)part, d, 64);
-        part_ref += (uint64_t)__shfl_xor((unsigned long long)part_ref, d, 64);
+    if (threadIdx.x == 0) {
+        wg[blk] = s_wave[0] + s_wave[1] + s_wave[2] + s_wave[3];
+        wg[a.nblk + blk] = s_ref[0] + s_ref[1] + s_ref[2] + s_ref[3];
+    }
+    int* diff = s_diff[w];
+#pragma unroll
+    for (int g = 0; g < DUP_G; g++) {
+        const uint32_t rows = emit_rows(id[g], r0[g], r1[g], cnt[g]);
+        if (rows <= DUP_LANE_ROWS) {
+            for (uint32_t r = 0; r < rows; r++) {
+                const EmitRow e = emit_row(id[g], r0[g], r1[g], r2[g], a.gridx, r);
+                count_row(diff, &s_all[w], e.t0, e.n, a.bits, mask);
+            }
+        }
+        uint64_t tall = __ballot(rows > DUP_LANE_ROWS);
+        while (tall) {
+            const int src = (int)__builtin_ctzll(tall);
+            tall &= tall - 1;
+            const uint32_t tid_ = __shfl(id[g], src, 64), t0_ = __shfl(r0[g], src, 64), t1_ = __shfl(r1[g], src, 64),
+                           t2_ = __shfl(r2[g], src, 64), trows = __shfl(rows, src, 64);
+            for (uint32_t r = lane; r < trows; r += 64) {
+                const EmitRow e = emit_row(tid_, t0_, t1_, t2_, a.gridx, r);
+                count_row(diff, &s_all[w], e.t0, e.n, a.bits, mask);
+            }
+        }
     }
     __syncthreads();
-    if (lane == 0) { s_wave[w] = part; s_ref[w] = part_ref; }
-    __syncthreads();
-    if (threadIdx.x == 0) {
-        const uint64_t base = s_wave[0] + s_wave[1] + s_wave[2] + s_wave[3];
-        s_base = base;
-        if (blk == nblk - 1) {
-            uint64_t* cnt = at_view(a.counters, a.g_stride, view);
-            const uint64_t ref_total = s_ref[0] + s_ref[1] + s_ref[2] + s_ref[3] + block_ref;
-            cnt[CNT_NUM_RENDERED] = base + block_total;
-            cnt[CNT_NUM_REFERENCE] = ref_total;
-            a.host_land[4 * view + CNT_NUM_RENDERED] = base + block_total;
-            a.host_land[4 * view + CNT_TRAP] = cnt[CNT_TRAP];
-            a.host_land[4 * view + LAND_NUM_REFERENCE] = ref_total;
-            __threadfence_system();
-        }
-    }
-    __syncthreads();
-    DUP_T(t3);
-    DUP_ADD(2, t3 - t2);
-    if (a.keys == nullptr) return;
-    KeyT* keys = at_view((KeyT*)a.keys, a.b_stride, view);
-    uint32_t* vals = at_view(a.vals, a.b_stride, view);
-    const uint64_t wave_off = s_base + wave_base;
-
-#pragma unroll 1
-    for (int g = 0; g < DUP_G; g++) {
-        uint32_t cnt_g = cnt[0], id_g = id[0], sp2_g = sp2[0];
-        uint2 rc_g = rc[0];
-        uint64_t ex_g = excl[0];
-#pragma unroll
-        for (int k = 1; k < DUP_G; k++)
-            if (g == k) { cnt_g = cnt[k]; id_g = id[k]; rc_g = rc[k]; ex_g = excl[k]; sp2_g = sp2[k]; }
-        const uint64_t off64 = wave_off + ex_g;
-        const uint64_t grp_begin64 = (uint64_t)__shfl((unsigned long long)off64, 0, 64);
-        const uint64_t grp_end64 = (uint64_t)__shfl((unsigned long long)(off64 + cnt_g), 63, 64);
-        if (grp_begin64 >= (uint64_t)a.cap) break;
-        const uint32_t grp_begin = (uint32_t)grp_begin64;
-        const uint32_t grp_end = grp_end64 < (uint64_t)a.cap ? (uint32_t)grp_end64 : (uint32_t)a.cap;
-        const uint64_t nzb = __ballot(cnt_g != 0);
-        const uint32_t n_nz = (uint32_t)__popcll(nzb);
-        const uint32_t jslot = __builtin_amdgcn_mbcnt_hi((uint32_t)(nzb >> 32), __builtin_amdgcn_mbcnt_lo((uint32_t)nzb, 0u));
-        __builtin_amdgcn_wave_barrier();
-        if (cnt_g != 0) {
-            s_off[w][jslot] = (uint32_t)(off64 - grp_begin64);
-            s_id[w][jslot] = id_g;
-            s_rect[w][jslot] = rc_g;
-            s_sp2[w][jslot] = sp2_g;
-            if (id_g & SPANS_FLAG) {
-                const uint32_t a4 = (rc_g.y >> 4) & 0x0F0F0F0Fu, b4 = (sp2_g >> 4) & 0x0F0F0F0Fu;
-                const uint32_t pa = a4 * 0x01010101u;
-                s_pre[w][jslot] = make_uint2(pa, b4 * 0x01010101u + (pa >> 24) * 0x01010101u);
-            }
-        }
-        __builtin_amdgcn_wave_barrier();
-        const uint32_t my_start = lane < n_nz ? s_off[w][lane] : 0xFFFFFFFFu;
-        const uint32_t range = grp_end - grp_begin;
-        uint32_t before = 0;
-        for (uint32_t c = 0; c < range; c += 64) {
-            s_flag[w][lane] = 0u;
-            const uint32_t d = my_start - c;
-            if (d < 64u) s_flag[w][d] = 1u;
-            __builtin_amdgcn_wave_barrier();
-            const uint32_t mine = s_flag[w][lane];
-            const uint64_t starts = __ballot(mine != 0u);
-            const uint32_t owner = before + mine - 1u +
-                                   __builtin_amdgcn_mbcnt_hi((uint32_t)(starts >> 32), __builtin_amdgcn_mbcnt_lo((uint32_t)starts, 0u));
-            before += (uint32_t)__popcll(starts);
-            __builtin_amdgcn_wave_barrier();
-            const uint32_t rel = c + lane;
-            if (rel < range) {
-                const uint2 r = s_rect[w][owner];
-                const uint32_t oid = s_id[w][owner];
-                const uint32_t minx = r.x & 0xFFFFu, miny = r.x >> 16;
-                const uint32_t t = rel - s_off[w][owner];
-                uint32_t row, col;
-                if (oid & SPANS_FLAG) {
-                    const uint2 pre = s_pre[w][owner];
-                    const uint32_t tt = (127u - t) * 0x01010101u;
-                    const uint32_t xa = (pre.x + tt) & 0x80808080u, xb = (pre.y + tt) & 0x80808080u;
-                    row = 8u - (uint32_t)__popc(xa) - (uint32_t)__popc(xb);
-                    const uint32_t rp = row - 1u;
-                    const uint32_t before = row == 0u ? 0u : (((rp < 4u ? pre.x : pre.y) >> (8u * (rp & 3u))) & 0xFFu);
-                    const uint32_t byte = ((row < 4u ? r.y : s_sp2[w][owner]) >> (8u * (row & 3u))) & 0xFFu;
-                    col = (byte & 15u) + (t - before);
-                } else {
-                    const uint32_t width = (r.y & 0xFFFFu) - minx;
-                    row = t / width;
-                    col = t - row * width;
-                }
-                const uint32_t p = grp_begin + rel;
-                keys[p] = (KeyT)((miny + row) * a.gridx + (minx + col));
-                vals[p] = oid & ~SPANS_FLAG;
-            }
-        }
-    }
-#ifdef GSR_STATS
-    if (w == 0) { DUP_T(t4); DUP_ADD(3, t4 - t3); }
-#endif
-}
-
-int launch_duplicate(const Launch& L, int P, const Batch& B, int gridx, bool key16, uint64_t* host_land)
-{
-    DupArgs a;
+    {
+        const uint32_t d = threadIdx.x;
+        const uint32_t v = d <= mask ? (uint32_t)(s_diff[0][d] + s_diff[1][d] + s_diff[2][d] + s_diff[3][d]) : 0u;
+        const uint32_t inc = block_exclusive_scan_256(v, s_tmp, nullptr) + v;
+        if (d <= mask) hist[(size_t)d * a.nblk + blk] = inc + s_all[0] + s_all[1] + s_all[2] + s_all[3];
+    }
+}
+
+int launch_dup_count(const Launch& L, int P, const Batch& B, int gridx, int T)
+{
+    DupCountArgs a;
     a.P = P;
     a.gridx = (uint32_t)gridx;
     a.order[0] = B.g.dval[0];
     a.order[1] = B.g.dval[1];
     a.sortctl = B.g.sortctl;
     a.splat = B.g.splat;
-    a.dup_status = B.g.dup_status;
+    a.wg = B.g.emit_wg;
+    a.hist = B.g.emit_hist;
+    a.g_stride = B.g_stride;
+    a.nblk = emit_blocks(P);
+    a.bits = (uint32_t)emit_digit_bits(T);
+    hipLaunchKernelGGL(k_dup_count, dim3((unsigned)a.nblk, B.V), dim3(DUP_THREADS), 0, L.stream, a);
+    return check_launch(L, "dup_count");
+}
+
+struct EmitArgs {
+    int P;
+    uint32_t gridx;
+    const uint32_t* order[2];
+    const uint32_t* sortctl;
+    const Splat* splat;
+    const uint64_t* wg;
+    const uint32_t* hist;
+    const uint32_t* totals;
+    const uint64_t* counters;
+    size_t g_stride;
+    int nblk;
+    void* keys;
+    uint32_t* vals;
+    size_t b_stride;
+    uint32_t cap;
+};
+
+template <int BITS, typename KeyT>
+__global__ __launch_bounds__(RS_THREADS, sizeof(KeyT) == 2 ? 3 : 2) void k_duplicate(EmitArgs a)
+{
+    static_assert(RS_TILE / RS_WAVES == 64 * RS_ITEMS && DUP_BLOCK / 16 == 64 && DUP_BLOCK == RS_THREADS * DUP_G, "slot and search geometry");
+    __shared__ KeyT s_key[RS_TILE];
+    __shared__ uint32_t s_val[RS_TILE];
+    __shared__ uint32_t wave_cnt[RS_WAVES][RADIX];
+    __shared__ uint32_t local_base[RADIX];
+    __shared__ uint32_t global_base[RADIX];
+    __shared__ uint32_t tmp[4];
+    const ScatterLds<KeyT> s{s_key, s_val, wave_cnt, local_base, global_base, tmp};
+    __shared__ uint4 s_rec[DUP_BLOCK];
+    __shared__ uint32_t s_off[DUP_BLOCK + 64];
+    __shared__ uint32_t s_flag[RS_WAVES][64];
+    const uint32_t view = blockIdx.y, blk = blockIdx.x;
+    const uint32_t tid = threadIdx.x, lane = tid & 63, w = tid >> 6;
+    constexpr uint32_t mask = (1u << BITS) - 1u;
+    const uint64_t* wg = at_view(a.wg, a.g_stride, view);
+    const uint64_t total64 = wg[blk];
+    if (total64 == 0 || at_view(a.counters, a.g_stride, view)[CNT_NUM_RENDERED] == 0) return;
+    const uint32_t total = (uint32_t)total64;
+    {
+        const uint32_t npass = depth_sort_passes(at_view(a.sortctl, a.g_stride, view)[SORTCTL_BITS]);
+        const uint32_t* order = at_view((npass & 1u) ? a.order[1] : a.order[0], a.g_stride, view);
+        const Splat* splat = at_view(a.splat, a.g_stride, view);
+        for (uint32_t i = tid; i < DUP_BLOCK + 64; i += RS_THREADS) s_off[i] = 0xFFFFFFFFu;
+        uint4 r[DUP_G];
+        uint32_t c[DUP_G], id[DUP_G], sum = 0, nz = 0;
+#pragma unroll
+        for (int g = 0; g < DUP_G; g++) {
+            const int pos = (int)(blk * DUP_BLOCK + tid * DUP_G + g);
+            id[g] = pos < a.P ? order[pos] : 0u;
+        }
+#pragma unroll
+        for (int g = 0; g < DUP_G; g++) {
+            c[g] = 0u;
+            r[g] = make_uint4(0u, 0u, 0u, 0u);
+            if ((int)(blk * DUP_BLOCK + tid * DUP_G + g) < a.P) {
+                const float4 q3 = splat[id[g]].q3;
+                const uint32_t w3 = __float_as_uint(q3.w);
+                r[g] = make_uint4(id[g] | (w3 & SPANS_FLAG), __float_as_uint(q3.x), __float_as_uint(q3.y), __float_as_uint(q3.z));
+                c[g] = emit_pairs(w3, r[g].z, r[g].w);
+            }
+            sum += c[g];
+            nz += c[g] != 0u;
+        }
+        uint32_t o = block_exclusive_scan_256(sum, tmp, nullptr);
+        uint32_t j = block_exclusive_scan_256(nz, tmp, nullptr);
+#pragma unroll
+        for (int g = 0; g < DUP_G; g++) {
+            if (c[g] != 0u) {
+                s_rec[j] = r[g];
+                s_off[j] = o;
+                j++;
+            }
+            o += c[g];
+        }
+    }
+    const uint32_t* hist = at_view(a.hist, a.g_stride, view);
+    const uint32_t* totals = at_view(a.totals, a.g_stride, view);
+    const uint32_t tot_d = tid <= mask ? totals[tid] : 0u;
+    const uint32_t hist_d = tid <= mask ? hist[(size_t)tid * a.nblk + blk] : 0u;
+    uint32_t gbase_d = block_exclusive_scan_256(tot_d, tmp, nullptr) + hist_d;
+    KeyT* keys = at_view((KeyT*)a.keys, a.b_stride, view);
+    uint32_t* vals = at_view(a.vals, a.b_stride, view);
+
+    for (uint32_t chunk = 0; chunk < total; chunk += RS_TILE) {
+        for (int i = lane; i < RADIX; i += 64) s.wave_cnt[w][i] = 0;
+        const uint32_t left = total - chunk;
+        const uint32_t count = left < (uint32_t)RS_TILE ? left : (uint32_t)RS_TILE;
+        const bool full = count == (uint32_t)RS_TILE;
+        const uint32_t first = chunk + w * (RS_TILE / RS_WAVES);
+        uint32_t before;
+        {
+            const uint32_t c1 = (uint32_t)__popcll(__ballot(s_off[lane * 16] < first));
+            const uint32_t b16 = c1 ? (c1 - 1u) * 16u : 0u;
+            const uint32_t c2 = (uint32_t)__popcll(__ballot(lane < 16u && s_off[b16 + (lane & 15u)] < first));
+            before = b16 + c2;
+        }
+        uint32_t k[RS_ITEMS], v[RS_ITEMS];
+#pragma unroll
+        for (int j = 0; j < RS_ITEMS; j++) {
+            const uint32_t s0 = first + j * 64;
+            s_flag[w][lane] = 0u;
+            const uint32_t dist = s_off[before + lane] - s0;
+            if (dist < 64u) s_flag[w][dist] = 1u;
+            __builtin_amdgcn_wave_barrier();
+            const uint32_t mine = s_flag[w][lane];
+            const uint64_t starts = __ballot(mine != 0u);
+            const uint32_t owner = (before + mine - 1u +
+                                    __builtin_amdgcn_mbcnt_hi((uint32_t)(starts >> 32), __builtin_amdgcn_mbcnt_lo((uint32_t)starts, 0u))) &
+                                   (DUP_BLOCK - 1);
+            before += (uint32_t)__popcll(starts);
+            __builtin_amdgcn_wave_barrier();
+            const uint32_t slot = s0 + lane;
+            k[j] = 0xFFFFFFFFu;
+            v[j] = 0u;
+            if (full || slot < total) {
+                const uint4 r = s_rec[owner];
+                const uint32_t t = slot - s_off[owner];
+                uint32_t row, row_first;
+                if (r.x & SPANS_FLAG) {
+                    const uint32_t a4 = (r.z >> 4) & 0x0F0F0F0Fu, b4 = (r.w >> 4) & 0x0F0F0F0Fu;
+                    const uint32_t pa = a4 * 0x01010101u;
+                    const uint32_t pb = b4 * 0x01010101u + (pa >> 24) * 0x01010101u;
+                    const uint32_t tt = (127u - t) * 0x01010101u;
+                    const uint32_t xa = (pa + tt) & 0x80808080u, xb = (pb + tt) & 0x80808080u;
+                    row = 8u - (uint32_t)__popc(xa) - (uint32_t)__popc(xb);
+                    const uint32_t rp = row - 1u;
+                    row_first = row == 0u ? 0u : (((rp < 4u ? pa : pb) >> (8u * (rp & 3u))) & 0xFFu);
+                } else {
+                    const uint32_t width = (r.z & 0xFFFFu) - (r.y & 0xFFFFu);
+                    row = t / width;
+                    row_first = row * width;
+                }
+                k[j] = (uint32_t)(KeyT)(emit_row(r.x, r.y, r.z, r.w, a.gridx, row).t0 + (t - row_first));
+                v[j] = r.x & ~SPANS_FLAG;
+            }
+        }
+        radix_scatter_tile<BITS, KeyT, RS_ITEMS, true>(k, v, full, first, total, count, 0, mask, 0u, gbase_d, a.cap, keys, vals, s);
+        __syncthreads();
+    }
+}
+
+int launch_duplicate(const Launch& L, int P, const Batch& B, int gridx, int T, bool key16)
+{
+    EmitArgs a;
+    a.P = P;
+    a.gridx = (uint32_t)gridx;
+    a.order[0] = B.g.dval[0];
+    a.order[1] = B.g.dval[1];
+    a.sortctl = B.g.sortctl;
+    a.splat = B.g.splat;
+    a.wg = B.g.emit_wg;
+    a.hist = B.g.emit_hist;
+    a.totals = B.g.emit_totals;
     a.counters = B.g.counters;
     a.g_stride = B.g_stride;
-    a.keys = B.b.key[0];
-    a.vals = B.b.val[0];
+    a.nblk = emit_blocks(P);
+    a.keys = B.b.key[1];
+    a.vals = B.b.val[1];
     a.b_stride = B.b_stride;
-    a.cap = B.b.key[0] ? B.b.cap : 0;
-    a.host_land = host_land;
-    a.tickets = block_tickets(-1);
-    const dim3 grid((unsigned)div_up(P, DUP_BLOCK), B.V);
-    if (key16)
-        hipLaunchKernelGGL(k_duplicate<uint16_t>, grid, dim3(DUP_THREADS), 0, L.stream, a);
-    else
-        hipLaunchKernelGGL(k_duplicate<uint32_t>, grid, dim3(DUP_THREADS), 0, L.stream, a);
+    a.cap = (uint32_t)B.b.cap;
+    const dim3 grid((unsigned)emit_blocks(P), B.V);
+    const int bits = emit_digit_bits(T);
+#define GSR_EMIT(B_, K_)                                                                                  \
+    case B_:                                                                                              \
+        hipLaunchKernelGGL((k_duplicate<B_, K_>), grid, dim3(RS_THREADS), 0, L.stream, a);                \
+        break;
+    if (key16) switch (bits) {
+        GSR_EMIT(1, uint16_t) GSR_EMIT(2, uint16_t) GSR_EMIT(3, uint16_t) GSR_EMIT(4, uint16_t) GSR_EMIT(5, uint16_t)
+        GSR_EMIT(6, uint16_t) GSR_EMIT(7, uint16_t) GSR_EMIT(8, uint16_t)
+    }
+    else switch (bits) {
+        GSR_EMIT(6, uint32_t) GSR_EMIT(7, uint32_t) GSR_EMIT(8, uint32_t)
+        default: return GSR_ERR_INVALID;
+    }
+#undef GSR_EMIT
     return check_launch(L, "duplicate");
 }
 
diff --git a/gaussian-pcloud-render_amd/csrc/common.hpp b/gaussian-pcloud-render_amd/csrc/common.hpp
--- a/gaussian-pcloud-render_amd/csrc/common.hpp
+++ b/gaussian-pcloud-render_amd/csrc/common.hpp
@@ -31,15 +31,21 @@
 inline int sort_hist_stride(int64_t n, int tile = RS_TILE) { return (int)(((n + tile - 1) / tile + 15) / 16 * 16); }
 
 constexpr int DUP_THREADS = 256;
-#ifndef GSR_DUP_G
-#define GSR_DUP_G 4
-#endif
-constexpr int DUP_G = GSR_DUP_G;
+constexpr int DUP_G = 4;
 constexpr int DUP_BLOCK = DUP_THREADS * DUP_G;
-#ifndef GSR_DUP_COPIES
-#define GSR_DUP_COPIES 8
-#endif
-constexpr int DUP_COPIES = GSR_DUP_COPIES;
+inline int emit_blocks(int P) { return (P > 0 ? P : 1) / DUP_BLOCK + ((P > 0 ? P : 1) % DUP_BLOCK != 0); }
+
+inline int radix_pass_count(int end_bit) { return (end_bit + RADIX_BITS - 1) / RADIX_BITS; }
+inline int radix_pass_bits(int end_bit, int pass)
+{
+    const int npass = radix_pass_count(end_bit);
+    int shift = 0, bits = 0;
+    for (int i = 0; i <= pass && i < npass; i++) {
+        bits = (end_bit - shift + (npass - i) - 1) / (npass - i);
+        shift += bits;
+    }
+    return pass < npass ? bits : 0;
+}
 
 inline size_t align_up(size_t v, size_t a) { return (v + a - 1) / a * a; }
 inline int64_t div_up(int64_t a, int64_t b) { return (a + b - 1) / b; }
@@ -75,10 +81,10 @@
     uint32_t* totals;
     uint32_t* blk_minmax;
     uint32_t* sortctl;
-    uint64_t* dup_status;
+    uint64_t* emit_wg;
+    uint32_t* emit_hist;
+    uint32_t* emit_totals;
     uint64_t* counters;
-    char* zero_begin;
-    size_t zero_bytes;
     size_t bytes;
 };
 
@@ -139,9 +145,14 @@
     carve(cur, g.totals, (size_t)RADIX);
     carve(cur, g.blk_minmax, 2 * nblk);
     carve(cur, g.sortctl, (size_t)4);
-    g.zero_begin = cur;
-    carve(cur, g.dup_status, (size_t)DUP_COPIES * (size_t)div_up((int64_t)p, DUP_BLOCK) + 1);
-    g.zero_bytes = (size_t)(cur - g.zero_begin);
+    const size_t eblk = (size_t)emit_blocks(P);
+    carve(cur, g.emit_wg, 8 * eblk + 1);
+    {
+        const size_t need = (RADIX * eblk + RADIX) * sizeof(uint32_t);
+        const size_t keys = 2 * align_up(p * sizeof(uint32_t), 256);
+        g.emit_hist = keys >= need ? g.dkey[0] : g.hist;
+        g.emit_totals = g.emit_hist + RADIX * eblk;
+    }
     carve(cur, g.counters, (size_t)8);
     g.bytes = (size_t)(cur - reinterpret_cast<char*>(base));
     return g;
@@ -303,12 +314,17 @@
 };
 constexpr int SORTCTL_BASE = 0;
 constexpr int SORTCTL_BITS = 1;
+constexpr uint64_t EMIT_MAX_PAIRS = 0x7FFFFFFFull;
 constexpr uint32_t CULLED_KEY = 0xFFFFFFFFu;
 __host__ __device__ inline uint32_t depth_sort_passes(uint32_t bits) { return (bits + RADIX_BITS - 1) / RADIX_BITS; }
-int launch_radix_sort_pairs(const Launch& L, const SortJob& job, bool iota_vals, int end_bit, int* result_buffer, bool key16 = false);
-int block_tickets(int set);
+int launch_radix_sort_pairs(const Launch& L, const SortJob& job, bool iota_vals, int end_bit, int* result_buffer, bool key16 = false,
+                            bool first_pass_done = false);
+int launch_emit_rowscan(const Launch& L, int P, const Batch& B, int bits, uint64_t* host_land);
 inline bool tile_keys16(int T) { return T <= 65536; }
-int launch_duplicate(const Launch& L, int P, const Batch& B, int gridx, bool key16, uint64_t* host_land);
+inline int tile_bits(int T) { return (int)higher_msb((uint32_t)T); }
+inline int emit_digit_bits(int T) { return radix_pass_bits(tile_bits(T), 0); }
+int launch_dup_count(const Launch& L, int P, const Batch& B, int gridx, int T);
+int launch_duplicate(const Launch& L, int P, const Batch& B, int gridx, int T, bool key16);
 int launch_tile_ranges(const Launch& L, const Batch& B, const uint32_t* sorted_keys, int T, bool key16);
 int launch_tile_order(const Launch& L, const Batch& B, int T);
 int launch_bwd_items(const Launch& L, const Batch& B, int T, int P);
@@ -342,7 +358,6 @@
 int selftest_det_reduce(hipStream_t stream);
 #ifdef GSR_STATS
 int debug_bwd_stats(unsigned long long* out8, int reset);
-int debug_dup_times(unsigned long long* out8, int reset);
 int debug_scatter_times(unsigned long long* out8, int reset);
 int debug_fwd_times(unsigned long long* out8, int reset);
 int debug_fwd_records(unsigned* out, int n);
diff --git a/gaussian-pcloud-render_amd/csrc/preprocess.hip b/gaussian-pcloud-render_amd/csrc/preprocess.hip
--- a/gaussian-pcloud-render_amd/csrc/preprocess.hip
+++ b/gaussian-pcloud-render_amd/csrc/preprocess.hip
@@ -74,8 +74,7 @@
     uint32_t* dkey;
     float* grad_rec;
     uint64_t* counters;
-    char* g_zero;
-    size_t g_zero_bytes, g_stride, gr_stride;
+    size_t g_stride, gr_stride;
     char* iv_zero;
     size_t iv_zero_bytes, iv_stride;
     int* radii;
@@ -93,7 +92,6 @@
                 at_view(a.counters, a.g_stride, vw)[CNT_STALL] = 0;
                 at_view(a.counters, a.g_stride, vw)[CNT_BWD_DIRTY] = 0;
             }
-            zero_region(a.g_zero + a.g_stride * vw, a.g_zero_bytes, gtid, nthr);
             zero_region(a.iv_zero + a.iv_stride * vw, a.iv_zero_bytes, gtid, nthr);
         }
     }
@@ -256,7 +254,7 @@
     a.view = p.viewmatrix; a.proj = p.projmatrix; a.campos = p.campos;
     a.splat = g.splat; a.tiles_touched = g.tiles_touched; a.clamped = g.clamped;
     a.dkey = g.dkey[0]; a.radii = radii; a.counters = g.counters; a.grad_rec = B.grad_rec; a.gr_stride = B.gr_stride;
-    a.g_zero = g.zero_begin; a.g_zero_bytes = g.zero_bytes; a.g_stride = B.g_stride;
+    a.g_stride = B.g_stride;
     a.iv_zero = B.iv.zero_begin; a.iv_zero_bytes = B.iv.zero_bytes; a.iv_stride = B.iv_stride;
     const int blocks = (p.P + 255) / 256;
     a.V = B.V;
diff --git a/gaussian-pcloud-render_amd/csrc/radix_scatter.hpp b/gaussian-pcloud-render_amd/csrc/radix_scatter.hpp
--- /dev/null
+++ b/gaussian-pcloud-render_amd/csrc/radix_scatter.hpp
@@ -0,0 +1,127 @@
+#pragma once
+#include "common.hpp"
+
+#ifndef SC_T
+#define SC_T(var) do { } while (0)
+#define SC_PUT(i, v) do { } while (0)
+#endif
+
+namespace gsr {
+
+__device__ __forceinline__ uint32_t wave_inclusive_scan(uint32_t v, uint32_t lane)
+{
+#pragma unroll
+    for (int d = 1; d < 64; d <<= 1) {
+        const uint32_t n = __shfl_up(v, d, 64);
+        if (lane >= (uint32_t)d) v += n;
+    }
+    return v;
+}
+
+__device__ __forceinline__ uint32_t block_exclusive_scan_256(uint32_t v, uint32_t* tmp, uint32_t* total)
+{
+    const uint32_t lane = threadIdx.x & 63, w = threadIdx.x >> 6;
+    const uint32_t inc = wave_inclusive_scan(v, lane);
+    if (lane == 63) tmp[w] = inc;
+    __syncthreads();
+    uint32_t base = 0;
+#pragma unroll
+    for (int i = 0; i < 4; i++)
+        if ((uint32_t)i < w) base += tmp[i];
+    if (total) *total = tmp[0] + tmp[1] + tmp[2] + tmp[3];
+    __syncthreads();
+    return base + inc - v;
+}
+
+template <typename SKeyT>
+struct ScatterLds {
+    SKeyT* key;
+    uint32_t* val;
+    uint32_t (*wave_cnt)[RADIX];
+    uint32_t* local_base;
+    uint32_t* global_base;
+    uint32_t* tmp;
+};
+
+template <int BITS, typename KeyT, int RS_ITEMS, bool CHECK_CAP, typename SKeyT, typename IdxT>
+__device__ __forceinline__ void radix_scatter_tile(const uint32_t (&k)[RS_ITEMS], const uint32_t (&v)[RS_ITEMS], bool full, IdxT seg_base, IdxT n, uint32_t count,
+                                                   int shift, uint32_t mask, uint32_t kbase, uint32_t& gbase_d, uint32_t cap,
+                                                   KeyT* __restrict__ keys_out, uint32_t* __restrict__ vals_out,
+                                                   const ScatterLds<SKeyT>& s, unsigned long long t1 = 0)
+{
+    const uint32_t tid = threadIdx.x, lane = tid & 63, w = tid >> 6;
+    uint32_t rank[RS_ITEMS];
+
+#pragma unroll
+    for (int j = 0; j < RS_ITEMS; j++) {
+        const bool ok = full || seg_base + j * 64 + lane < n;
+        const uint32_t d = (k[j] >> shift) & mask;
+        const uint64_t okb = full ? ~0ull : __ballot(ok);
+        uint32_t plo = (uint32_t)okb, phi = (uint32_t)(okb >> 32);
+#pragma unroll
+        for (int b = 0; b < BITS; b++) {
+            const uint32_t m = (uint32_t)__builtin_amdgcn_sbfe((int32_t)k[j], (uint32_t)(shift + b), 1u);
+            const uint64_t bal = __ballot(m != 0u);
+            plo = __builtin_amdgcn_bitop3_b32(plo, (uint32_t)bal, m, 0x90);
+            phi = __builtin_amdgcn_bitop3_b32(phi, (uint32_t)(bal >> 32), m, 0x90);
+        }
+        const uint32_t before = s.wave_cnt[w][d];
+        const uint32_t below = __builtin_amdgcn_mbcnt_hi(phi, __builtin_amdgcn_mbcnt_lo(plo, 0u));
+        rank[j] = before + below;
+        __builtin_amdgcn_wave_barrier();
+        if (ok && below == 0) s.wave_cnt[w][d] = before + (uint32_t)__popc(plo) + (uint32_t)__popc(phi);
+        __builtin_amdgcn_wave_barrier();
+    }
+    __syncthreads();
+    SC_T(t2);
+    SC_PUT(1, t2 - t1);
+
+    {
+        const uint32_t d = tid;
+        uint32_t c[RS_WAVES], run = 0;
+#pragma unroll
+        for (int i = 0; i < RS_WAVES; i++) {
+            c[i] = s.wave_cnt[i][d];
+            s.wave_cnt[i][d] = run;
+            run += c[i];
+        }
+        const uint32_t lbase = block_exclusive_scan_256(run, s.tmp, nullptr);
+        s.local_base[d] = lbase;
+        s.global_base[d] = gbase_d;
+        gbase_d += run;
+    }
+    __syncthreads();
+    SC_T(t3);
+    SC_PUT(2, t3 - t2);
+
+#pragma unroll
+    for (int j = 0; j < RS_ITEMS; j++) {
+        if (full || seg_base + j * 64 + lane < n) {
+            const uint32_t d = (k[j] >> shift) & mask;
+            const uint32_t pos = s.local_base[d] + s.wave_cnt[w][d] + rank[j];
+            s.key[pos] = (SKeyT)k[j];
+            s.val[pos] = v[j];
+        }
+    }
+    __syncthreads();
+    SC_T(t4);
+    SC_PUT(3, t4 - t3);
+
+#pragma unroll
+    for (int i = 0; i < RS_ITEMS; i++) {
+        const uint32_t p = i * RS_THREADS + tid;
+        if (p < count) {
+            const uint32_t key = s.key[p];
+            const uint32_t d = (key >> shift) & mask;
+            const size_t g = (size_t)s.global_base[d] + (p - s.local_base[d]);
+            if (!CHECK_CAP || g < (size_t)cap) {
+                keys_out[g] = (KeyT)(key + kbase);
+                vals_out[g] = s.val[p];
+            }
+        }
+    }
+    SC_T(t5);
+    SC_PUT(4, t5 - t4);
+}
+
+}
diff --git a/gaussian-pcloud-render_amd/csrc/sort.hip b/gaussian-pcloud-render_amd/csrc/sort.hip
--- a/gaussian-pcloud-render_amd/csrc/sort.hip
+++ b/gaussian-pcloud-render_amd/csrc/sort.hip
@@ -1,33 +1,34 @@
 #include "common.hpp"
 
+#ifdef GSR_STATS
 namespace gsr {
+constexpr int SC_REC = 65536;
+__device__ unsigned g_sc_rec[SC_REC][5];
+#define SC_T(var) const unsigned long long var = wall_clock64()
+#define SC_PUT(i, v) do { if (threadIdx.x == 0) { const unsigned r_ = blockIdx.y * gridDim.x + blockIdx.x; if (r_ < SC_REC) g_sc_rec[r_][i] = (unsigned)(v); } } while (0)
+int debug_scatter_times(unsigned long long* out8, int reset)
+{
+    static unsigned host[SC_REC][5];
+    if (hipMemcpyFromSymbol(host, HIP_SYMBOL(g_sc_rec), sizeof(host)) != hipSuccess) return -1;
+    for (int i = 0; i < 8; i++) out8[i] = 0;
+    for (int r = 0; r < SC_REC; r++) {
+        if (host[r][1] == 0) continue;
+        for (int i = 0; i < 5; i++) out8[i] += host[r][i];
+        out8[5]++;
+    }
+    if (reset) {
+        for (int r = 0; r < SC_REC; r++) for (int i = 0; i < 5; i++) host[r][i] = 0;
+        if (hipMemcpyToSymbol(HIP_SYMBOL(g_sc_rec), host, sizeof(host)) != hipSuccess) return -1;
+    }
+    return 0;
+}
+}
+#endif
+#include "radix_scatter.hpp"
+
+namespace gsr {
 
 __device__ __forceinline__ uint32_t lane_id() { return __builtin_amdgcn_mbcnt_hi(~0u, __builtin_amdgcn_mbcnt_lo(~0u, 0u)); }
-
-__device__ __forceinline__ uint32_t wave_inclusive_scan(uint32_t v, uint32_t lane)
-{
-#pragma unroll
-    for (int d = 1; d < 64; d <<= 1) {
-        const uint32_t n = __shfl_up(v, d, 64);
-        if (lane >= (uint32_t)d) v += n;
-    }
-    return v;
-}
-
-__device__ __forceinline__ uint32_t block_exclusive_scan_256(uint32_t v, uint32_t* tmp, uint32_t* total)
-{
-    const uint32_t lane = threadIdx.x & 63, w = threadIdx.x >> 6;
-    const uint32_t inc = wave_inclusive_scan(v, lane);
-    if (lane == 63) tmp[w] = inc;
-    __syncthreads();
-    uint32_t base = 0;
-#pragma unroll
-    for (int i = 0; i < 4; i++)
-        if ((uint32_t)i < w) base += tmp[i];
-    if (total) *total = tmp[0] + tmp[1] + tmp[2] + tmp[3];
-    __syncthreads();
-    return base + inc - v;
-}
 
 struct SortView {
     size_t stride;
@@ -123,12 +124,42 @@
     }
 }
 
+struct EmitTotals {
+    const uint64_t* wg;
+    uint64_t* counters;
+    uint64_t* host_land;
+};
 __global__ __launch_bounds__(256) void k_radix_rowscan(uint32_t* __restrict__ hist, uint32_t* __restrict__ totals, int nblk_pad,
                                                        size_t stride, const uint32_t* __restrict__ ctl, int shift,
                                                        const uint32_t* __restrict__ minmax, uint32_t* __restrict__ ctl_out,
-                                                       uint32_t nrows)
+                                                       uint32_t nrows, EmitTotals et)
 {
     __shared__ uint32_t tmp[4];
+    if (blockIdx.x == nrows && et.wg != nullptr) {
+        const uint64_t* wg = at_view(et.wg, stride, blockIdx.y);
+        uint64_t pairs = 0, ref = 0;
+        for (int b = threadIdx.x; b < nblk_pad; b += 256) { pairs += wg[b]; ref += wg[nblk_pad + b]; }
+#pragma unroll
+        for (int d = 32; d >= 1; d >>= 1) {
+            pairs += (uint64_t)__shfl_xor((unsigned long long)pairs, d, 64);
+            ref += (uint64_t)__shfl_xor((unsigned long long)ref, d, 64);
+        }
+        __shared__ uint64_t s_sum[2][4];
+        if ((threadIdx.x & 63) == 0) { s_sum[0][threadIdx.x >> 6] = pairs; s_sum[1][threadIdx.x >> 6] = ref; }
+        __syncthreads();
+        if (threadIdx.x == 0) {
+            pairs = s_sum[0][0] + s_sum[0][1] + s_sum[0][2] + s_sum[0][3];
+            ref = s_sum[1][0] + s_sum[1][1] + s_sum[1][2] + s_sum[1][3];
+            uint64_t* cnt = at_view(et.counters, stride, blockIdx.y);
+            cnt[CNT_NUM_RENDERED] = pairs <= EMIT_MAX_PAIRS ? pairs : 0ull;
+            cnt[CNT_NUM_REFERENCE] = ref;
+            et.host_land[4 * blockIdx.y + CNT_NUM_RENDERED] = pairs;
+            et.host_land[4 * blockIdx.y + CNT_TRAP] = cnt[CNT_TRAP];
+            et.host_land[4 * blockIdx.y + LAND_NUM_REFERENCE] = ref;
+            __threadfence_system();
+        }
+        return;
+    }
     if (blockIdx.x == nrows) {
         minmax = at_view(minmax, stride, blockIdx.y);
         uint32_t kmin = 0xFFFFFFFFu, kmax = 0u;
@@ -168,32 +199,6 @@
     }
     if (threadIdx.x == 0) totals[blockIdx.x] = carry;
 }
-
-#ifdef GSR_STATS
-constexpr int SC_REC = 65536;
-__device__ unsigned g_sc_rec[SC_REC][5];
-#define SC_T(var) const unsigned long long var = wall_clock64()
-#define SC_PUT(i, v) do { if (threadIdx.x == 0) { const unsigned r_ = blockIdx.y * gridDim.x + blockIdx.x; if (r_ < SC_REC) g_sc_rec[r_][i] = (unsigned)(v); } } while (0)
-int debug_scatter_times(unsigned long long* out8, int reset)
-{
-    static unsigned host[SC_REC][5];
-    if (hipMemcpyFromSymbol(host, HIP_SYMBOL(g_sc_rec), sizeof(host)) != hipSuccess) return -1;
-    for (int i = 0; i < 8; i++) out8[i] = 0;
-    for (int r = 0; r < SC_REC; r++) {
-        if (host[r][1] == 0) continue;
-        for (int i = 0; i < 5; i++) out8[i] += host[r][i];
-        out8[5]++;
-    }
-    if (reset) {
-        for (int r = 0; r < SC_REC; r++) for (int i = 0; i < 5; i++) host[r][i] = 0;
-        if (hipMemcpyToSymbol(HIP_SYMBOL(g_sc_rec), host, sizeof(host)) != hipSuccess) return -1;
-    }
-    return 0;
-}
-#else
-#define SC_T(var) do { } while (0)
-#define SC_PUT(i, v) do { } while (0)
-#endif
 
 template <int BITS, typename KeyT, int RS_ITEMS>
 __global__ __launch_bounds__(RS_THREADS) void k_radix_scatter(const KeyT* __restrict__ keys_in,
@@ -223,6 +228,7 @@
     __shared__ uint32_t local_base[RADIX];
     __shared__ uint32_t global_base[RADIX];
     __shared__ uint32_t tmp[4];
+    const ScatterLds<uint32_t> s{s_key, s_val, wave_cnt, local_base, global_base, tmp};
 
     const uint32_t tid = threadIdx.x, lane = tid & 63, w = tid >> 6;
     const int64_t blk_base = (int64_t)blk * RS_TILE;
@@ -234,7 +240,7 @@
     const uint32_t tot_d = tid <= mask ? totals[tid] : 0u;
     const uint32_t hist_d = tid <= mask ? hist[(size_t)tid * nblk_pad + blk] : 0u;
 
-    uint32_t k[RS_ITEMS], v[RS_ITEMS], rank[RS_ITEMS];
+    uint32_t k[RS_ITEMS], v[RS_ITEMS];
     const bool full = blk_base + RS_TILE <= n;
     {
         const KeyT* kp = keys_in + seg_base + lane;
@@ -267,79 +273,17 @@
     SC_T(t1);
     SC_PUT(0, t1 - t0);
 
-#pragma unroll
-    for (int j = 0; j < RS_ITEMS; j++) {
-        const bool ok = full || seg_base + j * 64 + lane < n;
-        const uint32_t d = (k[j] >> shift) & mask;
-        const uint64_t okb = full ? ~0ull : __ballot(ok);
-        uint32_t plo = (uint32_t)okb, phi = (uint32_t)(okb >> 32);
-#pragma unroll
-        for (int b = 0; b < BITS; b++) {
-            const uint32_t m = (uint32_t)__builtin_amdgcn_sbfe((int32_t)k[j], (uint32_t)(shift + b), 1u);
-            const uint64_t bal = __ballot(m != 0u);
-            plo = __builtin_amdgcn_bitop3_b32(plo, (uint32_t)bal, m, 0x90);
-            phi = __builtin_amdgcn_bitop3_b32(phi, (uint32_t)(bal >> 32), m, 0x90);
-        }
-        const uint32_t before = wave_cnt[w][d];
-        const uint32_t below = __builtin_amdgcn_mbcnt_hi(phi, __builtin_amdgcn_mbcnt_lo(plo, 0u));
-        rank[j] = before + below;
-        __builtin_amdgcn_wave_barrier();
-        if (ok && below == 0) wave_cnt[w][d] = before + (uint32_t)__popc(plo) + (uint32_t)__popc(phi);
-        __builtin_amdgcn_wave_barrier();
-    }
-    __syncthreads();
-    SC_T(t2);
-    SC_PUT(1, t2 - t1);
-
-    {
-        const uint32_t d = tid;
-        uint32_t c[RS_WAVES], run = 0;
-#pragma unroll
-        for (int i = 0; i < RS_WAVES; i++) {
-            c[i] = wave_cnt[i][d];
-            wave_cnt[i][d] = run;
-            run += c[i];
-        }
-        const uint32_t lbase = block_exclusive_scan_256(run, tmp, nullptr);
-        local_base[d] = lbase;
-        global_base[d] = gbase_d;
-    }
-    __syncthreads();
-    SC_T(t3);
-    SC_PUT(2, t3 - t2);
-
-#pragma unroll
-    for (int j = 0; j < RS_ITEMS; j++) {
-        if (full || seg_base + j * 64 + lane < n) {
-            const uint32_t d = (k[j] >> shift) & mask;
-            const uint32_t pos = local_base[d] + wave_cnt[w][d] + rank[j];
-            s_key[pos] = k[j];
-            s_val[pos] = v[j];
-        }
-    }
-    __syncthreads();
-    SC_T(t4);
-    SC_PUT(3, t4 - t3);
-
     const int64_t rem = n - blk_base;
     const uint32_t count = rem < RS_TILE ? (uint32_t)rem : (uint32_t)RS_TILE;
-#pragma unroll
-    for (int i = 0; i < RS_ITEMS; i++) {
-        const uint32_t p = i * RS_THREADS + tid;
-        if (p < count) {
-            const uint32_t key = s_key[p];
-            const uint32_t d = (key >> shift) & mask;
-            const size_t g = (size_t)global_base[d] + (p - local_base[d]);
-            keys_out[g] = (KeyT)(key + kbase);
-            vals_out[g] = s_val[p];
-        }
-    }
 #ifdef GSR_STATS
-    { SC_T(t5); SC_PUT(4, t5 - t4); }
+    radix_scatter_tile<BITS, KeyT, RS_ITEMS, false>(k, v, full, seg_base, n, count, shift, mask, kbase, gbase_d, 0u, keys_out, vals_out, s, t1);
+#else
+    radix_scatter_tile<BITS, KeyT, RS_ITEMS, false>(k, v, full, seg_base, n, count, shift, mask, kbase, gbase_d, 0u, keys_out, vals_out, s);
 #endif
 }
 
-int launch_radix_sort_pairs(const Launch& L, const SortJob& job, bool iota_vals, int end_bit, int* result_buffer, bool key16)
+int launch_radix_sort_pairs(const Launch& L, const SortJob& job, bool iota_vals, int end_bit, int* result_buffer, bool key16,
+                            bool first_pass_done)
 {
     int cur = 0;
     if (job.cap > 0 && job.V > 0) {
@@ -351,10 +295,16 @@
         const dim3 grid_hist(nblk_pad, job.V);
         const dim3 grid((unsigned)div_up(nblk, 8 * HIST_GROUP) * 8 * HIST_GROUP, job.V);
         bool first = true;
-        const int npass = (end_bit + RADIX_BITS - 1) / RADIX_BITS;
+        const int npass = radix_pass_count(end_bit);
         int shift = 0;
         for (int pass = 0; pass < npass; pass++) {
-            const int bits = (end_bit - shift + (npass - pass) - 1) / (npass - pass);
+            const int bits = radix_pass_bits(end_bit, pass);
+            if (pass == 0 && first_pass_done) {
+                cur ^= 1;
+                first = false;
+                shift += bits;
+                continue;
+            }
             const uint32_t mask = (1u << bits) - 1u;
             const bool make_ctl = job.sortctl != nullptr && pass == 0;
             sv.ctl = (job.sortctl != nullptr && pass > 0) ? job.sortctl : nullptr;
@@ -370,7 +320,8 @@
                                    shift, mask, job.hist, nblk_pad, minmax);
             if (int e = check_launch(L, "radix_hist")) return e;
             hipLaunchKernelGGL(k_radix_rowscan, dim3(mask + 1u + (make_ctl ? 1u : 0u), job.V), dim3(256), 0, L.stream, job.hist,
-                               job.totals, nblk_pad, job.stride, sv.ctl, shift, (const uint32_t*)minmax, job.sortctl, mask + 1u);
+                               job.totals, nblk_pad, job.stride, sv.ctl, shift, (const uint32_t*)minmax, job.sortctl, mask + 1u,
+                               EmitTotals{nullptr, nullptr, nullptr});
             if (int e = check_launch(L, "radix_rowscan")) return e;
             const uint32_t* vin = (first && iota_vals) ? (const uint32_t*)nullptr : (const uint32_t*)job.val[cur];
 #define GSR_SCATTER(B)                                                                                                        \
@@ -399,10 +350,19 @@
             shift += bits;
         }
     } else {
-        cur = ((end_bit + RADIX_BITS - 1) / RADIX_BITS) & 1;
+        cur = radix_pass_count(end_bit) & 1;
     }
     *result_buffer = cur;
     return GSR_OK;
 }
 
-}
+int launch_emit_rowscan(const Launch& L, int P, const Batch& B, int bits, uint64_t* host_land)
+{
+    const uint32_t nrows = 1u << bits;
+    hipLaunchKernelGGL(k_radix_rowscan, dim3(nrows + 1u, B.V), dim3(256), 0, L.stream, B.g.emit_hist, B.g.emit_totals, emit_blocks(P),
+                       B.g_stride, (const uint32_t*)nullptr, 0, (const uint32_t*)nullptr, (uint32_t*)nullptr, nrows,
+                       EmitTotals{B.g.emit_wg, B.g.counters, host_land});
+    return check_launch(L, "emit_rowscan");
+}
+
+}
diff --git a/gaussian-pcloud-render_amd/diff_gaussian_rasterization/_native.py b/gaussian-pcloud-render_amd/diff_gaussian_rasterization/_native.py
--- a/gaussian-pcloud-render_amd/diff_gaussian_rasterization/_native.py
+++ b/gaussian-pcloud-render_amd/diff_gaussian_rasterization/_native.py
@@ -55,6 +55,8 @@
     "gsr_set_forward_half_views": (_int, [_int]),
     "gsr_set_backward_moments": (_int, [_int]),
     "gsr_get_profile": (_int, [C.POINTER(C.c_char_p), C.POINTER(C.c_float), _int]),
+    "gsr_tile_sort_split": (_int, [_int, C.POINTER(_int)]),
+    "gsr_emit_digit_bits": (_int, [_int]),
     "gsr_selftest": (_int, [_fp]),
     "gsr_d2h_count": (C.c_longlong, []),
     "gsr_clock_probe_launch": (_int, [_fp, _int, _fp]),
diff --git a/include/gsr.h b/include/gsr.h
--- a/include/gsr.h
+++ b/include/gsr.h
@@ -120,6 +120,9 @@
 void gsr_set_profiling(int on);
 int gsr_get_profile(const char** names, float* ms, int cap);
 
+int gsr_tile_sort_split(int T, int* widths);
+int gsr_emit_digit_bits(int T);
+
 int gsr_clock_probe_launch(void* dst16, int iters, gsr_stream_t stream);
 int gsr_wall_clock_khz(void);
 
```

New measurement: 2077. 0.974x the previous value.
